# ubuntuslave/vo_single_camera_sos

Hardware: AMD Instinct MI355X
Metric: frame-pairs/sec (detect+match+triangulate+RANSAC) on 640x480 omni, 2000 kpts (higher is better)
Workload: dtype u8/f32/f64

## Files before the change

include/sosvo.h:

```cpp
#ifndef SOSVO_H
#define SOSVO_H

#include <stdint.h>

#ifdef __cplusplus
extern "C" {
#endif

typedef struct sosvo_ctx sosvo_ctx;

typedef enum {
  SOSVO_OK = 0,
  SOSVO_ERR_ARG = -1,
  SOSVO_ERR_HIP = -2,
  SOSVO_ERR_NODEVICE = -3,
  SOSVO_ERR_CAPACITY = -4
} sosvo_status;

#define SOSVO_DESC_BYTES 32
#define SOSVO_KEY_SHIFT 20
#define SOSVO_KEY_IDX_MASK 0xFFFFFu
#define SOSVO_KEY_NONE 0xFFFFFFFFu


int32_t sosvo_abi_version(void);

int32_t sosvo_orb_bit_pattern_31(int8_t* pattern_host);

int32_t sosvo_create(sosvo_ctx** out, int32_t device, void* stream);
int32_t sosvo_destroy(sosvo_ctx* ctx);
int32_t sosvo_set_stream(sosvo_ctx* ctx, void* stream);
#define SOSVO_HINT_SHARED_DEVICE 1
#define SOSVO_HINT_SCORE_FP64_ONLY 2
#define SOSVO_HINT_MATCH_UNSPLIT 3
int32_t sosvo_set_hint(sosvo_ctx* ctx, int32_t hint, int32_t value);
int32_t sosvo_synchronize(sosvo_ctx* ctx);
const char* sosvo_last_error(const sosvo_ctx* ctx);

int32_t sosvo_timer_start(sosvo_ctx* ctx);
int32_t sosvo_timer_stop(sosvo_ctx* ctx);
int32_t sosvo_timer_elapsed_ms(sosvo_ctx* ctx, float* ms);

int32_t sosvo_profile_enable(sosvo_ctx* ctx, int32_t on);
int32_t sosvo_profile_count(sosvo_ctx* ctx);
int32_t sosvo_profile_get(sosvo_ctx* ctx, int32_t i, char* name_out, int32_t name_cap, float* ms);

int32_t sosvo_debug_fill_scratch(sosvo_ctx* ctx, int32_t byte);

int32_t sosvo_unwrap(sosvo_ctx* ctx, const uint8_t* omni, const uint8_t* masks, const float* map_x,
                     const float* map_y, int32_t nframes, int32_t H, int32_t W, int32_t rows,
                     int32_t cols, uint8_t* pano);

int32_t sosvo_unwrap_prepare(sosvo_ctx* ctx, const uint8_t* masks, const float* map_x, const float* map_y,
                             int32_t H, int32_t W, int32_t rows, int32_t cols, uint32_t* table);
int32_t sosvo_unwrap_table(sosvo_ctx* ctx, const uint8_t* omni, const uint32_t* table, int32_t nframes,
                           int32_t H, int32_t W, int32_t rows, int32_t cols, uint8_t* pano);

int32_t sosvo_median_gray(sosvo_ctx* ctx, const uint8_t* img, int32_t nimg, int32_t rows,
                          int32_t cols, int32_t ksize, uint8_t* gray);
int32_t sosvo_unwrap_median_gray(sosvo_ctx* ctx, const uint8_t* omni, const uint32_t* table, int32_t nframes,
                                 int32_t H, int32_t W, int32_t rows, int32_t cols, int32_t ksize, uint8_t* gray);

int32_t sosvo_unwrap_median_gray_rows(sosvo_ctx* ctx, const uint8_t* omni, const uint32_t* table, int32_t nframes,
                                      int32_t H, int32_t W, int32_t rows, int32_t cols, int32_t ksize,
                                      const int32_t* row_range, uint8_t* gray);

int32_t sosvo_gray_rows_needed(sosvo_ctx* ctx, const uint32_t* mask_bits, int32_t nsets, int32_t rows, int32_t cols,
                               int32_t nmask, int32_t edge, const int8_t* pattern, float cos_a, float sin_a,
                               int32_t* row_range);

int32_t sosvo_detect_gft(sosvo_ctx* ctx, const uint8_t* gray, const uint32_t* mask_bits, int32_t nimg,
                         int32_t images_per_maskset, int32_t rows, int32_t cols, int32_t nmask,
                         double quality, double min_distance, int32_t max_corners, int32_t cap,
                         float* kp, int32_t* n, int32_t* status);

int32_t sosvo_describe_orb(sosvo_ctx* ctx, const uint8_t* gray, int32_t nimg, int32_t rows, int32_t cols,
                           int32_t nmask, int32_t cap, float* kp, int32_t* n, float cos_a, float sin_a,
                           const int8_t* pattern, int32_t edge, uint8_t* desc);

int32_t sosvo_describe_orb_rows(sosvo_ctx* ctx, const uint8_t* gray, int32_t nimg, int32_t rows, int32_t cols,
                                int32_t nmask, int32_t cap, float* kp, int32_t* n, float cos_a, float sin_a,
                                const int8_t* pattern, int32_t edge, const int32_t* row_range, uint8_t* desc);

int32_t sosvo_subpix_weights(sosvo_ctx* ctx, int32_t half, int32_t* w_host);
int32_t sosvo_refine_subpix(sosvo_ctx* ctx, const uint8_t* gray, int32_t nimg, int32_t rows, int32_t cols, int32_t nmask,
                            int32_t cap, float* kp, const int32_t* n, int32_t half, int32_t max_iter, double eps,
                            const int32_t* row_range);

#define SOSVO_LK_INITIAL_FLOW 1
int32_t sosvo_gray_pyramid_bytes(sosvo_ctx* ctx, int32_t nimg, int32_t rows, int32_t cols, int32_t levels, int64_t* bytes);
int32_t sosvo_gray_pyramid(sosvo_ctx* ctx, const uint8_t* gray, int32_t nimg, int32_t rows, int32_t cols, int32_t levels,
                           const int32_t* row_range, uint8_t* pyr);
int32_t sosvo_track_lk(sosvo_ctx* ctx, const uint8_t* gray, const uint8_t* pyr, int32_t nimg, int32_t rows, int32_t cols,
                       int32_t levels, const int32_t* row_range, const int32_t* prev_img, const int32_t* next_img, int32_t nprob,
                       int32_t cap, const float* prev_pts, const int32_t* n, int32_t half, int32_t max_iter, double eps,
                       double min_eig, int32_t flags, float* next_pts, uint8_t* status, float* err, float* back, double fb_max);

int64_t sosvo_orb_pyramid_pixels(int32_t rows, int32_t cols);
int32_t sosvo_orb_mask_pyramid(sosvo_ctx* ctx, const uint32_t* mask_bits, int32_t nsets, int32_t rows,
                               int32_t cols, int32_t nmask, uint32_t* mask_pyr);
int32_t sosvo_detect_orb(sosvo_ctx* ctx, const uint8_t* gray, const uint32_t* mask_pyr, int32_t nimg,
                         int32_t images_per_maskset, int32_t rows, int32_t cols, int32_t nmask,
                         int32_t nfeatures, int32_t cap, float* kp4, float* resp, int32_t* n);
int32_t sosvo_describe_orb_levels(sosvo_ctx* ctx, const uint8_t* gray, int32_t nimg, int32_t rows,
                                  int32_t cols, int32_t nmask, int32_t cap, float* kp4, int32_t* n,
                                  const int8_t* pattern, uint8_t* desc, float* kp_xy);
int32_t sosvo_detect_describe_orb(sosvo_ctx* ctx, const uint8_t* gray, const uint32_t* mask_pyr, int32_t nimg,
                                  int32_t images_per_maskset, int32_t rows, int32_t cols, int32_t nmask,
                                  int32_t nfeatures, int32_t cap, float* kp4, float* resp, int32_t* n,
                                  const int8_t* pattern, uint8_t* desc, float* kp_xy);

int32_t sosvo_detect_fast(sosvo_ctx* ctx, const uint8_t* gray, const uint32_t* mask_bits, int32_t nimg,
                          int32_t images_per_maskset, int32_t rows, int32_t cols, int32_t nmask,
                          int32_t threshold, int32_t cap, float* kp, int32_t* n, int32_t* status);

int32_t sosvo_detect_agast(sosvo_ctx* ctx, const uint8_t* gray, const uint32_t* mask_bits, int32_t nimg,
                           int32_t images_per_maskset, int32_t rows, int32_t cols, int32_t nmask,
                           int32_t threshold, int32_t cap, float* kp, int32_t* n, int32_t* status);

int32_t sosvo_match_hamming(sosvo_ctx* ctx, const uint8_t* q_desc, const uint8_t* t_desc,
                            const int32_t* nq, const int32_t* nt, const int32_t* q_slot,
                            const int32_t* t_slot, int32_t nprob, int32_t q_stride,
                            int32_t t_stride, int32_t k, uint32_t* keys);

int32_t sosvo_match_hamming_gated(sosvo_ctx* ctx, const uint8_t* q_desc, const uint8_t* t_desc, const float* q_pos,
                                  const float* t_pos, const int32_t* nq, const int32_t* nt, const int32_t* q_slot,
                                  const int32_t* t_slot, int32_t nprob, int32_t n_forward, int32_t q_stride, int32_t t_stride,
                                  double min_dv, double max_du, int32_t max_distance, uint32_t* keys);

int32_t sosvo_match_hamming_ratio(sosvo_ctx* ctx, const uint8_t* q_desc, const uint8_t* t_desc, const float* q_pos,
                                  const float* t_pos, const int32_t* nq, const int32_t* nt, const int32_t* q_slot,
                                  const int32_t* t_slot, int32_t nprob, int32_t n_forward, int32_t q_stride, int32_t t_stride,
                                  double min_dv, double max_du, int32_t max_distance, int32_t ratio_64ths,
                                  uint32_t* keys, uint32_t* rivals);

int32_t sosvo_match_l2(sosvo_ctx* ctx, const float* q_desc, const float* t_desc, const int32_t* nq, const int32_t* nt,
                       int32_t nprob, int32_t q_stride, int32_t t_stride, int32_t dim, int32_t k, uint64_t* keys);

int32_t sosvo_match_radius(sosvo_ctx* ctx, const uint8_t* q_desc, const uint8_t* t_desc, const int32_t* nq,
                           const int32_t* nt, const int32_t* q_slot, const int32_t* t_slot, int32_t nprob,
                           int32_t q_stride, int32_t t_stride, int32_t max_distance, int32_t cap,
                           uint32_t* keys, int32_t* counts);

int32_t sosvo_cross_check_matches(sosvo_ctx* ctx, const uint32_t* keys_fwd, const uint32_t* keys_rev, const int32_t* nq,
                                  const int32_t* nt, const int32_t* q_slot, const int32_t* t_slot, int32_t nprob,
                                  int32_t q_stride, int32_t t_stride, uint32_t* keys_out, int32_t* n_kept);

int32_t sosvo_sort_matches(sosvo_ctx* ctx, const uint32_t* keys, const int32_t* nq,
                           const int32_t* q_slot, int32_t nprob, int32_t q_stride, int32_t* order);

#define SOSVO_FLAG_CAM_ROT_IDENTITY 1
#define SOSVO_FLAG_EPNP 2
#define SOSVO_FLAG_GP3P 4
#define SOSVO_FLAG_TWOPT 8
int32_t sosvo_ransac_abs_pose(sosvo_ctx* ctx, const double* f, const double* p, const int32_t* cam,
                              const double* cam_off, const double* cam_rot, int32_t ncam, int32_t flags,
                              const int32_t* n, int32_t nprob, int32_t stride, double thr,
                              int32_t max_iter, int32_t adaptive, uint64_t seed, double* T_out,
                              uint8_t* inlier_mask, int32_t* inlier_idx, int32_t* n_inliers,
                              int32_t* info, int32_t* hyp_counts);
int32_t sosvo_ransac_abs_pose_seeds(sosvo_ctx* ctx, const double* f, const double* p, const int32_t* cam,
                                    const double* cam_off, const double* cam_rot, int32_t ncam, int32_t flags,
                                    const int32_t* n, int32_t nprob, int32_t stride, double thr,
                                    int32_t max_iter, int32_t adaptive, const uint64_t* seeds, double* T_out,
                                    uint8_t* inlier_mask, int32_t* inlier_idx, int32_t* n_inliers,
                                    int32_t* info, int32_t* hyp_counts);

int32_t sosvo_refine_abs_pose(sosvo_ctx* ctx, const double* f, const double* p, const int32_t* cam,
                              const double* cam_off, const double* cam_rot, int32_t ncam,
                              const int32_t* n, int32_t nprob, int32_t stride, const int32_t* idx,
                              const int32_t* m, int32_t max_lm_iter, double* T_io, double* cost_out,
                              int32_t* iters_out);

#define SOSVO_REL_FIVEPT 5
#define SOSVO_REL_SEVENPT 7
#define SOSVO_REL_EIGHTPT 8
int32_t sosvo_ransac_rel_pose(sosvo_ctx* ctx, const double* f1, const double* f2, const int32_t* n, int32_t nprob,
                              int32_t stride, int32_t algorithm, double thr, int32_t max_iter, int32_t adaptive,
                              uint64_t seed, double* T_out, uint8_t* inlier_mask, int32_t* inlier_idx,
                              int32_t* n_inliers, int32_t* info, int32_t* hyp_counts);

int32_t sosvo_pano_to_bearing(sosvo_ctx* ctx, const double* uv, int32_t n, double cols, double rows,
                              double pixel_size, double cyl_height_max, double* az, double* el,
                              double* bearing);
int32_t sosvo_triangulate_midpoint(sosvo_ctx* ctx, const double* az_top, const double* el_top,
                                   const double* az_bot, const double* el_bot, int32_t n,
                                   const double* F_top_host, const double* F_bot_host, double* X);
int32_t sosvo_triangulate2(sosvo_ctx* ctx, const double* b1, const double* b2, int32_t n, const double* t12_host,
                           const double* R12_host, double* X);
int32_t sosvo_range_filter(sosvo_ctx* ctx, const double* X, int32_t n, double min_range,
                           double max_range, uint8_t* ok);
int32_t sosvo_rgbd_backproject(sosvo_ctx* ctx, const float* depth, int32_t rows, int32_t cols,
                               const int32_t* u, const int32_t* v, int32_t n, double fx, double fy,
                               double cx, double cy, double focal_length_m, int32_t depth_is_Z,
                               double* xyz, double* bearing);

typedef struct sosvo_rig {
  double pano_top[4];
  double pano_bot[4];
  double F_top[3];
  double F_bot[3];
  double min_range;
  double max_range;
  double stereo_min_disp;
  double stereo_max_hdiff;
  double f2f_max_hdiff;
  double pct_good_matches;
} sosvo_rig;

int32_t sosvo_stereo_assemble(sosvo_ctx* ctx, const sosvo_rig* rig_host, const float* kp_top,
                              const float* kp_bot, const uint8_t* desc_top, const uint8_t* desc_bot,
                              const int32_t* n_top, const int32_t* n_bot, const uint32_t* keys,
                              const int32_t* order, int32_t nframes, int32_t nmask, int32_t cap,
                              int32_t out_cap, float* m_top, float* m_bot, uint8_t* d_top,
                              uint8_t* d_bot, double* X, double* b_top, double* b_bot, int32_t* M,
                              int32_t* n_cand);

int32_t sosvo_f2f_assemble(sosvo_ctx* ctx, const sosvo_rig* rig_host, const float* m_top,
                           const float* m_bot, const double* X, const double* b_top,
                           const double* b_bot, const int32_t* M, int32_t frame_cap,
                           const int32_t* ref_frame, const int32_t* cur_frame, const uint32_t* keys_top,
                           const int32_t* order_top, const uint32_t* keys_bot, const int32_t* order_bot,
                           int32_t npairs, int32_t corr_cap, double* f, double* p, int32_t* cam,
                           int32_t* corr_q, int32_t* corr_t, int32_t* n, int32_t* n_topview);

int32_t sosvo_f2f_assemble_tracked(sosvo_ctx* ctx, const sosvo_rig* rig_host, const float* m_top, const float* m_bot,
                                   const double* X, const int32_t* M, int32_t frame_cap, const int32_t* ref_frame,
// ... 193 lines not shown
```

vo_single_camera_sos_amd/_lib.py:

```python
import ctypes
import os
import re
from collections import namedtuple

_HERE = os.path.dirname(os.path.abspath(__file__))
LIB_PATH = os.path.join(_HERE, "libsosvo.so")
HEADER_PATH = os.path.join(os.path.dirname(_HERE), "include", "sosvo.h")

c_i32 = ctypes.c_int32
c_f64 = ctypes.c_double
c_f32 = ctypes.c_float
c_u64 = ctypes.c_uint64
c_p = ctypes.c_void_p

SOSVO_OK = 0
STATUS_NAMES = {0: "SOSVO_OK", -1: "SOSVO_ERR_ARG", -2: "SOSVO_ERR_HIP", -3: "SOSVO_ERR_NODEVICE",
                -4: "SOSVO_ERR_CAPACITY"}

KEY_SHIFT = 20
KEY_IDX_MASK = 0xFFFFF
KEY_NONE = 0xFFFFFFFF
DESC_BYTES = 32


class SosvoError(RuntimeError):
    pass


SIGNATURES = {
    "sosvo_abi_version": (c_i32, []),
    "sosvo_orb_bit_pattern_31": (c_i32, [c_p]),
    "sosvo_create": (c_i32, [ctypes.POINTER(c_p), c_i32, c_p]),
    "sosvo_destroy": (c_i32, [c_p]),
    "sosvo_set_stream": (c_i32, [c_p, c_p]),
    "sosvo_set_hint": (c_i32, [c_p, c_i32, c_i32]),
    "sosvo_set_lk_options": (c_i32, [c_p, c_p]),
    "sosvo_set_stereo_lk_options": (c_i32, [c_p, c_p]),
    "sosvo_synchronize": (c_i32, [c_p]),
    "sosvo_last_error": (ctypes.c_char_p, [c_p]),
    "sosvo_timer_start": (c_i32, [c_p]),
    "sosvo_timer_stop": (c_i32, [c_p]),
    "sosvo_timer_elapsed_ms": (c_i32, [c_p, ctypes.POINTER(c_f32)]),
    "sosvo_profile_enable": (c_i32, [c_p, c_i32]),
    "sosvo_profile_count": (c_i32, [c_p]),
    "sosvo_debug_fill_scratch": (c_i32, [c_p, c_i32]),
    "sosvo_profile_get": (c_i32, [c_p, c_i32, ctypes.c_char_p, c_i32, ctypes.POINTER(c_f32)]),
    "sosvo_unwrap": (c_i32, [c_p, c_p, c_p, c_p, c_p, c_i32, c_i32, c_i32, c_i32, c_i32, c_p]),
    "sosvo_unwrap_prepare": (c_i32, [c_p, c_p, c_p, c_p, c_i32, c_i32, c_i32, c_i32, c_p]),
    "sosvo_unwrap_table": (c_i32, [c_p, c_p, c_p, c_i32, c_i32, c_i32, c_i32, c_i32, c_p]),
    "sosvo_median_gray": (c_i32, [c_p, c_p, c_i32, c_i32, c_i32, c_i32, c_p]),
    "sosvo_unwrap_median_gray": (c_i32, [c_p, c_p, c_p, c_i32, c_i32, c_i32, c_i32, c_i32, c_i32, c_p]),
    "sosvo_unwrap_median_gray_rows": (c_i32, [c_p, c_p, c_p, c_i32, c_i32, c_i32, c_i32, c_i32, c_i32, c_p, c_p]),
    "sosvo_gray_rows_needed": (c_i32, [c_p, c_p, c_i32, c_i32, c_i32, c_i32, c_i32, c_p, c_f32, c_f32, c_p]),
    "sosvo_detect_gft": (c_i32, [c_p, c_p, c_p, c_i32, c_i32, c_i32, c_i32, c_i32, c_f64, c_f64, c_i32, c_i32, c_p,
                                 c_p, c_p]),
    "sosvo_describe_orb": (c_i32, [c_p, c_p, c_i32, c_i32, c_i32, c_i32, c_i32, c_p, c_p, c_f32, c_f32, c_p, c_i32,
                                   c_p]),
    "sosvo_describe_orb_rows": (c_i32, [c_p, c_p, c_i32, c_i32, c_i32, c_i32, c_i32, c_p, c_p, c_f32, c_f32, c_p, c_i32,
                                        c_p, c_p]),
    "sosvo_subpix_weights": (c_i32, [c_p, c_i32, c_p]),
    "sosvo_refine_subpix": (c_i32, [c_p, c_p, c_i32, c_i32, c_i32, c_i32, c_i32, c_p, c_p, c_i32, c_i32, c_f64, c_p]),
    "sosvo_gray_pyramid_bytes": (c_i32, [c_p, c_i32, c_i32, c_i32, c_i32, ctypes.POINTER(ctypes.c_int64)]),
    "sosvo_gray_pyramid": (c_i32, [c_p, c_p, c_i32, c_i32, c_i32, c_i32, c_p, c_p]),
    "sosvo_track_lk": (c_i32, [c_p, c_p, c_p, c_i32, c_i32, c_i32, c_i32, c_p, c_p, c_p, c_i32, c_i32, c_p, c_p, c_i32, c_i32,
                               c_f64, c_f64, c_i32, c_p, c_p, c_p, c_p, c_f64]),
    "sosvo_refine_stereo_lk": (c_i32, [c_p, c_p, c_i32, c_i32, c_i32, c_p, c_i32, c_i32, c_p, c_p, c_p, c_p, c_p, c_f64, c_f64,
                                       c_p, c_p]),
    "sosvo_orb_pyramid_pixels": (ctypes.c_int64, [c_i32, c_i32]),
    "sosvo_orb_mask_pyramid": (c_i32, [c_p, c_p, c_i32, c_i32, c_i32, c_i32, c_p]),
    "sosvo_detect_orb": (c_i32, [c_p, c_p, c_p, c_i32, c_i32, c_i32, c_i32, c_i32, c_i32, c_i32, c_p, c_p, c_p]),
    "sosvo_describe_orb_levels": (c_i32, [c_p, c_p, c_i32, c_i32, c_i32, c_i32, c_i32, c_p, c_p, c_p, c_p, c_p]),
    "sosvo_detect_describe_orb": (c_i32, [c_p, c_p, c_p, c_i32, c_i32, c_i32, c_i32, c_i32, c_i32, c_i32, c_p, c_p, c_p, c_p,
                                          c_p, c_p]),
    "sosvo_detect_fast": (c_i32, [c_p, c_p, c_p, c_i32, c_i32, c_i32, c_i32, c_i32, c_i32, c_i32, c_p, c_p, c_p]),
    "sosvo_detect_agast": (c_i32, [c_p, c_p, c_p, c_i32, c_i32, c_i32, c_i32, c_i32, c_i32, c_i32, c_p, c_p, c_p]),
    "sosvo_match_hamming": (c_i32, [c_p, c_p, c_p, c_p, c_p, c_p, c_p, c_i32, c_i32, c_i32, c_i32, c_p]),
    "sosvo_match_hamming_gated": (c_i32, [c_p, c_p, c_p, c_p, c_p, c_p, c_p, c_p, c_p, c_i32, c_i32, c_i32, c_i32, c_f64, c_f64,
                                          c_i32, c_p]),
    "sosvo_match_hamming_ratio": (c_i32, [c_p, c_p, c_p, c_p, c_p, c_p, c_p, c_p, c_p, c_i32, c_i32, c_i32, c_i32, c_f64, c_f64,
                                          c_i32, c_i32, c_p, c_p]),
    "sosvo_match_radius": (c_i32, [c_p, c_p, c_p, c_p, c_p, c_p, c_p, c_i32, c_i32, c_i32, c_i32, c_i32, c_p, c_p]),
    "sosvo_cross_check_matches": (c_i32, [c_p, c_p, c_p, c_p, c_p, c_p, c_p, c_i32, c_i32, c_i32, c_p, c_p]),
    "sosvo_sort_matches": (c_i32, [c_p, c_p, c_p, c_p, c_i32, c_i32, c_p]),
    "sosvo_pano_to_bearing": (c_i32, [c_p, c_p, c_i32, c_f64, c_f64, c_f64, c_f64, c_p, c_p, c_p]),
    "sosvo_triangulate_midpoint": (c_i32, [c_p, c_p, c_p, c_p, c_p, c_i32, c_p, c_p, c_p]),
    "sosvo_triangulate2": (c_i32, [c_p, c_p, c_p, c_i32, c_p, c_p, c_p]),
    "sosvo_range_filter": (c_i32, [c_p, c_p, c_i32, c_f64, c_f64, c_p]),
    "sosvo_rgbd_backproject": (c_i32, [c_p, c_p, c_i32, c_i32, c_p, c_p, c_i32, c_f64, c_f64, c_f64, c_f64, c_f64,
                                       c_i32, c_p, c_p]),
    "sosvo_stereo_assemble": (c_i32, [c_p] + [c_p] * 9 + [c_i32] * 4 + [c_p] * 9),
    "sosvo_f2f_assemble": (c_i32, [c_p] + [c_p] * 7 + [c_i32] + [c_p] * 6 + [c_i32, c_i32] + [c_p] * 7),
    "sosvo_f2f_assemble_tracked": (c_i32, [c_p] + [c_p] * 5 + [c_i32] + [c_p] * 5 + [c_i32, c_i32] + [c_p] * 7),
    "sosvo_ransac_abs_pose": (c_i32, [c_p, c_p, c_p, c_p, c_p, c_p, c_i32, c_i32, c_p, c_i32, c_i32, c_f64,
                                      c_i32, c_i32, c_u64, c_p, c_p, c_p, c_p, c_p, c_p]),
    "sosvo_ransac_abs_pose_seeds": (c_i32, [c_p, c_p, c_p, c_p, c_p, c_p, c_i32, c_i32, c_p, c_i32, c_i32, c_f64,
                                            c_i32, c_i32, c_p, c_p, c_p, c_p, c_p, c_p, c_p]),
    "sosvo_match_l2": (c_i32, [c_p, c_p, c_p, c_p, c_p, c_i32, c_i32, c_i32, c_i32, c_i32, c_p]),
    "sosvo_ransac_rel_pose": (c_i32, [c_p, c_p, c_p, c_p, c_i32, c_i32, c_i32, c_f64, c_i32, c_i32, c_u64, c_p, c_p, c_p, c_p,
                                      c_p, c_p]),
    "sosvo_refine_abs_pose": (c_i32, [c_p, c_p, c_p, c_p, c_p, c_p, c_i32, c_p, c_i32, c_i32, c_p, c_p, c_i32,
                                      c_p, c_p, c_p]),
    "sosvo_rgbd_assemble": (c_i32, [c_p, c_p, c_p, c_p, c_p, c_p, c_i32, c_i32, c_i32, c_i32, c_i32, c_p, c_p, c_p, c_p, c_p]),
    "sosvo_f2f_assemble_central": (c_i32, [c_p, c_f64, c_f64, c_p, c_p, c_p, c_p, c_i32, c_p, c_p, c_p, c_p, c_i32, c_i32,
                                           c_p, c_p, c_p, c_p, c_p]),
    "sosvo_frame_pair_batch_workspace": (ctypes.c_size_t, [c_p]),
    "sosvo_frame_pair_batch": (c_i32, [c_p, c_p, c_p, c_p, c_p, c_p, c_p, c_p, ctypes.c_size_t, c_p]),
    "sosvo_frame_pair_batch_streams_workspace": (ctypes.c_size_t, [c_p, c_i32]),
    "sosvo_frame_pair_batch_streams": (c_i32, [c_p, c_p, c_p, c_i32, c_p, c_p, c_p, c_p, c_p, ctypes.c_size_t, c_p]),
    "sosvo_frame_pair_batch_streams_enqueue": (c_i32, [c_p, c_p, c_p, c_i32, c_p, c_p, c_p, c_p, c_p, ctypes.c_size_t, c_p]),
    "sosvo_frame_pair_batch_streams_join": (c_i32, [c_p]),
    "sosvo_sequence_workspace": (ctypes.c_size_t, [c_p, c_i32, c_i32]),
    "sosvo_sequence_front_end": (c_i32, [c_p, c_p, c_p, c_i32, c_i32, c_p, c_i32, c_i32, c_p, c_p, c_p, c_p, ctypes.c_size_t]),
    "sosvo_sequence_track": (c_i32, [c_p, c_p, c_p, c_i32, c_i32, c_p, c_p, c_i32, c_u64, c_p, ctypes.c_size_t, c_p]),
    "sosvo_sequence_copy_slot": (c_i32, [c_p, c_p, c_i32, c_i32, c_i32, c_i32, c_p, ctypes.c_size_t]),
    "sosvo_sequence_frame_counts": (c_i32, [c_p, c_p, c_i32, c_i32, c_i32, c_i32, c_p, ctypes.c_size_t, c_p]),
    "sosvo_sequence_front_end_slots": (c_i32, [c_p, c_p, c_p, c_i32, c_i32, c_p, c_i32, c_p, c_p, c_p, c_p, c_p, ctypes.c_size_t]),
    "sosvo_sequence_track_seeds": (c_i32, [c_p, c_p, c_p, c_i32, c_i32, c_p, c_p, c_p, c_i32, c_p, ctypes.c_size_t, c_p]),
    "sosvo_sequence_copy_slots": (c_i32, [c_p, c_p, c_i32, c_i32, c_p, c_p, c_i32, c_p, ctypes.c_size_t]),
    "sosvo_rgbd_sequence_workspace": (ctypes.c_size_t, [c_p, c_i32, c_i32]),
    "sosvo_rgbd_sequence_front_end": (c_i32, [c_p, c_p, c_p, c_i32, c_i32, c_p, c_p, c_i32, c_i32, c_p, c_p, c_p, ctypes.c_size_t]),
    "sosvo_rgbd_sequence_track": (c_i32, [c_p, c_p, c_i32, c_i32, c_p, c_p, c_i32, c_u64, c_p, ctypes.c_size_t, c_p]),
    "sosvo_rgbd_sequence_copy_slot": (c_i32, [c_p, c_p, c_i32, c_i32, c_i32, c_i32, c_p, ctypes.c_size_t]),
    "sosvo_rgbd_sequence_frame_counts": (c_i32, [c_p, c_p, c_i32, c_i32, c_i32, c_i32, c_p, ctypes.c_size_t, c_p]),
    "sosvo_rgbd_sequence_front_end_slots": (c_i32, [c_p, c_p, c_p, c_i32, c_i32, c_p, c_p, c_i32, c_p, c_p, c_p, c_p,
                                                    ctypes.c_size_t]),
    "sosvo_rgbd_sequence_track_seeds": (c_i32, [c_p, c_p, c_i32, c_i32, c_p, c_p, c_p, c_i32, c_p, ctypes.c_size_t, c_p]),
    "sosvo_rgbd_sequence_copy_slots": (c_i32, [c_p, c_p, c_i32, c_i32, c_p, c_p, c_i32, c_p, ctypes.c_size_t]),
    "sosvo_rgbd_pair_batch_workspace": (ctypes.c_size_t, [c_p]),
    "sosvo_rgbd_pair_batch": (c_i32, [c_p, c_p, c_p, c_p, c_p, c_p, c_p, c_p, ctypes.c_size_t, c_p]),
}

HINT_SHARED_DEVICE = 1
HINT_SCORE_FP64_ONLY = 2
HINT_MATCH_UNSPLIT = 3
FLAG_CAM_ROT_IDENTITY = 1
FLAG_EPNP = 2
FLAG_GP3P = 4
FLAG_TWOPT = 8
FLAG_CROSS_CHECK_STEREO = 0x1000
FLAG_CROSS_CHECK_F2F = 0x2000
FLAG_GATED_STEREO = 0x4000
FLAG_GATED_F2F = 0x8000
GATED_MAX_DIST_SHIFT = 16
GATED_MAX_DIST_MASK = 0x1FF << GATED_MAX_DIST_SHIFT
FLAG_RATIO_STEREO = 0x10
FLAG_RATIO_F2F = 0x20
RATIO_64THS_SHIFT = 25
RATIO_64THS_MASK = 0x3F << RATIO_64THS_SHIFT
FLAG_SUBPIX = 0x40
SUBPIX_HALF_SHIFT = 10
SUBPIX_HALF_MASK = 3 << SUBPIX_HALF_SHIFT
SUBPIX_MAX_ITER = 10
SUBPIX_EPS = 0.01
FLAG_LK_F2F = 0x80
FLAG_LK_STEREO = 0x100
LK_INITIAL_FLOW = 1
LK_MAX_HALF, LK_MAX_LEVELS, LK_MAX_ITER, LK_MAX_CAP = 10, 4, 30, 4096
DETECTOR_GFT = 0
DETECTOR_ORB = 1
DETECTOR_FAST = 2
DETECTOR_AGAST = 3
DETECTORS = {"GFT": DETECTOR_GFT, "ORB": DETECTOR_ORB, "FAST": DETECTOR_FAST, "AGAST": DETECTOR_AGAST}
RGBD_DETECTOR_SHIFT = 8
RGBD_DETECTOR_MASK = 3 << RGBD_DETECTOR_SHIFT
REL_FIVEPT = 5
REL_SEVENPT = 7
REL_EIGHTPT = 8


class Rig(ctypes.Structure):
    _fields_ = [("pano_top", c_f64 * 4), ("pano_bot", c_f64 * 4), ("F_top", c_f64 * 3), ("F_bot", c_f64 * 3),
                ("min_range", c_f64), ("max_range", c_f64), ("stereo_min_disp", c_f64),
                ("stereo_max_hdiff", c_f64), ("f2f_max_hdiff", c_f64), ("pct_good_matches", c_f64)]



class RgbdCam(ctypes.Structure):
    _fields_ = [("fx", c_f64), ("fy", c_f64), ("cx", c_f64), ("cy", c_f64), ("focal_length_m", c_f64),
                ("depth_is_Z", c_i32), ("reserved", c_i32), ("min_range", c_f64), ("max_range", c_f64)]


class BatchCfg(ctypes.Structure):
    _fields_ = [("n_pairs", c_i32), ("H", c_i32), ("W", c_i32), ("rows", c_i32), ("cols", c_i32), ("nmask", c_i32),
                ("kp_cap", c_i32), ("frame_cap", c_i32), ("median_ksize", c_i32), ("max_corners", c_i32), ("edge", c_i32),
                ("ransac_max_iter", c_i32), ("ransac_adaptive", c_i32), ("lm_max_iter", c_i32), ("quality", c_f64),
                ("min_distance", c_f64), ("ransac_threshold", c_f64), ("seed", c_u64), ("cos_a", c_f32), ("sin_a", c_f32),
                ("ransac_flags", c_i32), ("detector", c_i32)]


class RgbdBatchCfg(ctypes.Structure):
    _fields_ = [("n_pairs", c_i32), ("rows", c_i32), ("cols", c_i32), ("kp_cap", c_i32), ("frame_cap", c_i32),
                ("median_ksize", c_i32), ("max_corners", c_i32), ("edge", c_i32), ("ransac_max_iter", c_i32),
                ("ransac_adaptive", c_i32), ("lm_max_iter", c_i32), ("flags", c_i32), ("quality", c_f64),
                ("min_distance", c_f64), ("ransac_threshold", c_f64), ("pct_good_matches", c_f64), ("f2f_max_hdiff", c_f64),
                ("seed", c_u64), ("cos_a", c_f32), ("sin_a", c_f32)]


def detector_code(method):
    name = str(method).upper()
    if name not in DETECTORS:
        raise NotImplementedError("detection method %r: the batched paths run %s" % (method, ", ".join(DETECTORS)))
    return DETECTORS[name]


def rgbd_detector_flags(method):
    return detector_code(method) << RGBD_DETECTOR_SHIFT


def cross_check_flags(stereo=False, f2f=False):
    return (FLAG_CROSS_CHECK_STEREO if stereo else 0) | (FLAG_CROSS_CHECK_F2F if f2f else 0)


def gated_flags(stereo=False, f2f=False, max_distance=None):
    if max_distance is not None and (int(max_distance) != max_distance or not 1 <= max_distance <= 256):
        raise ValueError("gated_max_distance must be None or an integer in 1 .. 256, got %r" % (max_distance,))
    flags = (FLAG_GATED_STEREO if stereo else 0) | (FLAG_GATED_F2F if f2f else 0)
    if flags and max_distance is not None:
        flags |= int(max_distance) << GATED_MAX_DIST_SHIFT
    return flags


def ratio_64ths(ratio):
    try:
        x = float(ratio) * 64.0
    except (TypeError, ValueError):
        raise ValueError("ratio must be a float in (0, 1) with ratio * 64 an integer, got %r" % (ratio,))
    if not (x == x and 1.0 <= x <= 63.0 and x == int(x)):
        if x != x:
            raise ValueError("ratio must be a float in (0, 1) with ratio * 64 an integer, got %r" % (ratio,))
        lo, hi = sorted(sorted(range(1, 64), key=lambda c: abs(c - x))[:2])
        raise ValueError("ratio must be a float in (0, 1) with ratio * 64 an integer, got %r; the nearest admissible values "
                         "are %r (%d/64) and %r (%d/64)" % (ratio, lo / 64.0, lo, hi / 64.0, hi))
    return int(x)


def ratio_flags(stereo=False, f2f=False, ratio=None):
    r = None if ratio is None else ratio_64ths(ratio)
    flags = (FLAG_RATIO_STEREO if stereo else 0) | (FLAG_RATIO_F2F if f2f else 0)
    if flags and r is None:
        raise ValueError("the ratio test needs a ratio (a float in (0, 1) with ratio * 64 an integer, e.g. 0.75)")
    if flags:
        flags |= r << RATIO_64THS_SHIFT
    return flags


def subpix_half(subpix):
    if subpix is None or subpix is False:
        return None
    if subpix is True:
        return 5
    if int(subpix) != subpix or not 2 <= subpix <= 5:
        raise ValueError("subpix must be None or a window half-size in 2 .. 5, got %r" % (subpix,))
    return int(subpix)


def subpix_flags(subpix=None):
    half = subpix_half(subpix)
    return 0 if half is None else FLAG_SUBPIX | ((half - 2) << SUBPIX_HALF_SHIFT)


def subpix_half_of(flags):
    flags = int(flags)
    return ((flags & SUBPIX_HALF_MASK) >> SUBPIX_HALF_SHIFT) + 2 if flags & FLAG_SUBPIX else None


def subpix_weights(half):
    w = (c_i32 * 11)()
    rc = load().sosvo_subpix_weights(None, int(half), w)
    if rc != 0:
        raise SosvoError("sosvo_subpix_weights(%r) -> %s" % (half, STATUS_NAMES.get(rc, rc)))
    return list(w)[:2 * int(half) + 1]


class LKOptions(namedtuple("LKOptions", "half levels max_iter eps min_eig fb_max")):
    __slots__ = ()

    def __new__(cls, half=10, levels=3, max_iter=30, eps=0.01, min_eig=1e-4, fb_max=None):
        for name, v, lo, hi in (("half", half, 2, LK_MAX_HALF), ("levels", levels, 1, LK_MAX_LEVELS),
                                ("max_iter", max_iter, 1, LK_MAX_ITER)):
            if isinstance(v, bool) or not isinstance(v, (int, float)) or int(v) != v or not lo <= v <= hi:
                raise ValueError("lk %s must be an integer in %d .. %d, got %r" % (name, lo, hi, v))
        for name, v in (("eps", eps), ("min_eig", min_eig)):
            if isinstance(v, bool) or not isinstance(v, (int, float)) or not 0.0 <= v < float("inf"):
                raise ValueError("lk %s must be a finite number >= 0, got %r" % (name, v))
        if fb_max is not None and (isinstance(fb_max, bool) or not isinstance(fb_max, (int, float))
                                   or not 0.0 < fb_max < float("inf")):
            raise ValueError("lk fb_max must be None or a finite number > 0 (pixels), got %r" % (fb_max,))
# ... 181 lines not shown
```

vo_single_camera_sos_amd/csrc/common.h:

```cpp
#pragma once
#include <hip/hip_runtime.h>
#include <stdint.h>
#include <stdio.h>
#include <string.h>

#include "sosvo.h"

struct sosvo_prof_entry {
  const char* name;
  hipEvent_t a, b;
};

constexpr int kSosvoProfMax = 16384;

constexpr int kSosvoMaxSubStreams = 4;

struct sosvo_ctx {
  int32_t device;
  hipStream_t stream;
  hipEvent_t ev_start, ev_stop;
  char err[512];
  void* ws;
  size_t ws_bytes;
  int32_t prof_on;
  int32_t prof_n;
  int32_t prof_created;
  sosvo_prof_entry* prof;
  sosvo_ctx* sub[kSosvoMaxSubStreams];
  hipEvent_t sub_done[kSosvoMaxSubStreams], sub_median[kSosvoMaxSubStreams], sub_begin;
  int32_t n_sub;
  int32_t hint_score_fp64_only;
  int32_t hint_shared_device;
  int32_t hint_match_unsplit;
  sosvo_lk_options lk;
  sosvo_stereo_lk_options stereo_lk;
  int32_t sub_last;
  int32_t sub_pending;
  const void* sub_last_ws;
  size_t sub_last_bytes[kSosvoMaxSubStreams];
};

struct SosvoProfScope {
  sosvo_ctx* ctx;
  bool active;
  SosvoProfScope(sosvo_ctx* c, const char* name) : ctx(c), active(false) {
    if (!c->prof_on || !c->prof || c->prof_n >= kSosvoProfMax) return;
    sosvo_prof_entry& e = c->prof[c->prof_n];
    if (c->prof_n >= c->prof_created) {
      if (hipEventCreate(&e.a) != hipSuccess || hipEventCreate(&e.b) != hipSuccess) return;
      c->prof_created = c->prof_n + 1;
    }
    e.name = name;
    if (hipEventRecord(e.a, c->stream) != hipSuccess) return;
    active = true;
  }
  ~SosvoProfScope() {
    if (!active) return;
    (void)hipEventRecord(ctx->prof[ctx->prof_n].b, ctx->stream);
    ctx->prof_n++;
  }
};
#define SOSVO_PROFILE(ctx, name) SosvoProfScope sosvo_prof_scope_(ctx, name)

#define SOSVO_LAUNCH(ctx, kernel, ...)            \
  do {                                            \
    SOSVO_PROFILE(ctx, #kernel);                  \
    hipLaunchKernelGGL(kernel, __VA_ARGS__);      \
  } while (0)

#define SOSVO_WAVE 64

static inline int32_t sosvo_fail(sosvo_ctx* ctx, int32_t code, const char* what, const char* detail) {
  if (ctx) snprintf(ctx->err, sizeof(ctx->err), "%s: %s", what, detail ? detail : "");
  return code;
}

#define SOSVO_REQUIRE(ctx, cond, msg)                                   \
  do {                                                                  \
    if (!(cond)) return sosvo_fail((ctx), SOSVO_ERR_ARG, __func__, msg); \
  } while (0)

static inline bool sosvo_table_frame_ok(int64_t H, int64_t W) {
  return H > 0 && W > 0 && H <= 16384 && W <= 16384 && 3 * W * (H - 1) >= 8;
}
#define SOSVO_TABLE_FRAME_MSG \
  "frame size out of range for the unwrap table: 1 <= H, W <= 16384 and 3 * W * (H - 1) >= 8 (8 bytes must follow the start of the second row)"

#define SOSVO_HIP(ctx, call)                                                          \
  do {                                                                                \
    hipError_t e_ = (call);                                                           \
    if (e_ != hipSuccess) return sosvo_fail((ctx), SOSVO_ERR_HIP, #call, hipGetErrorString(e_)); \
  } while (0)

#define SOSVO_ENTER(ctx)                                   \
  do {                                                     \
    if (!(ctx)) return SOSVO_ERR_ARG;                      \
    SOSVO_HIP((ctx), hipSetDevice((ctx)->device));         \
  } while (0)

#define SOSVO_LATENCY_BOUND_PRIO() __builtin_amdgcn_s_setprio(3)
#define SOSVO_STREAMING_PRIO() __builtin_amdgcn_s_setprio(2)

#define SOSVO_LAUNCH_CHECK(ctx) SOSVO_HIP((ctx), hipGetLastError())

static inline int32_t sosvo_ws_reserve(sosvo_ctx* ctx, size_t bytes) {
  if (bytes <= ctx->ws_bytes) return SOSVO_OK;
  if (ctx->ws) {
    SOSVO_HIP(ctx, hipStreamSynchronize(ctx->stream));
    SOSVO_HIP(ctx, hipFree(ctx->ws));
    ctx->ws = nullptr;
    ctx->ws_bytes = 0;
  }
  SOSVO_HIP(ctx, hipMalloc(&ctx->ws, bytes));
  ctx->ws_bytes = bytes;
  return SOSVO_OK;
}

static inline int cdiv(int a, int b) { return (a + b - 1) / b; }

__host__ __device__ static inline uint32_t sosvo_float_ordered(float f) {
  uint32_t u;
  memcpy(&u, &f, 4);
  return (u & 0x80000000u) ? ~u : (u | 0x80000000u);
}
__host__ __device__ static inline float sosvo_ordered_float(uint32_t u) {
  u = (u & 0x80000000u) ? (u & 0x7FFFFFFFu) : ~u;
  float f;
  memcpy(&f, &u, 4);
  return f;
}

#ifdef __HIPCC__
__device__ __forceinline__ int refl101(int i, int n) {
  if (n == 1) return 0;
  while (i < 0 || i >= n) i = i < 0 ? -i : 2 * (n - 1) - i;
  return i;
}

__device__ __forceinline__ int clampi(int v, int lo, int hi) { return v < lo ? lo : (v > hi ? hi : v); }

__device__ __forceinline__ void sosvo_copy_bytes(uint8_t* __restrict__ d, const uint8_t* __restrict__ s, size_t nbytes, int i0, int stride) {
  size_t done = 0;
  if ((((uintptr_t)d | (uintptr_t)s) & 15) == 0) {
    const size_t nv = nbytes / 16;
    for (size_t i = i0; i < nv; i += stride) reinterpret_cast<uint4*>(d)[i] = reinterpret_cast<const uint4*>(s)[i];
    done = nv * 16;
  }
  for (size_t i = done + i0; i < nbytes; i += stride) d[i] = s[i];
}

__device__ __forceinline__ int lane_from_left(int v) { return __builtin_amdgcn_update_dpp(0, v, 0x138, 0xF, 0xF, true); }
__device__ __forceinline__ int lane_from_right(int v) { return __builtin_amdgcn_update_dpp(0, v, 0x130, 0xF, 0xF, true); }
__device__ __forceinline__ float lane_from_left(float v) { return __int_as_float(lane_from_left(__float_as_int(v))); }
__device__ __forceinline__ float lane_from_right(float v) { return __int_as_float(lane_from_right(__float_as_int(v))); }

__device__ __forceinline__ uint32_t vmad24(uint32_t k, uint32_t x, uint32_t acc) {
  uint32_t r;
  asm("v_mad_u32_u24 %0, %1, %2, %3" : "=v"(r) : "v"(x), "v"(k), "v"(acc));
  return r;
}

template <int NW = 4>
__device__ __forceinline__ int sosvo_block_compact_pos(bool valid, int* wave_off, int* s_running, int tid) {
  const int lane = tid & 63, wid = tid >> 6;
  const unsigned long long bal = __ballot(valid);
  __syncthreads();
  if (lane == 0) wave_off[wid + 1] = __popcll(bal);
  __syncthreads();
  if (tid == 0) {
    wave_off[0] = *s_running;
    for (int w = 0; w < NW; ++w) wave_off[w + 1] += wave_off[w];
    *s_running = wave_off[NW];
  }
  __syncthreads();
  return wave_off[wid] + __popcll(bal & ((1ULL << lane) - 1ULL));
}

__device__ __forceinline__ int xcd_problem(int nimg, int nmask) {
  const int xcd = (int)(blockIdx.x & 7), slot = (int)(blockIdx.x >> 3);
  const int img = (slot / nmask) * 8 + xcd, m = slot - (slot / nmask) * nmask;
  return img < nimg ? img * nmask + m : -1;
}
static inline unsigned xcd_grid(int nimg, int nmask) { return (unsigned)(8 * cdiv(nimg, 8) * nmask); }

__device__ __forceinline__ int sosvo_block_count_matches(const uint32_t* __restrict__ keys, int nq, int tid, int threads) {
  int kept = 0;
// ... 41 lines not shown
```

vo_single_camera_sos_amd/csrc/ctx.hip:

```cpp
#include "common.h"
#include "orb_bit_pattern_31.h"

#include <stdlib.h>

static const sosvo_lk_options kLkDefaults = SOSVO_LK_OPTIONS_DEFAULT;
static const sosvo_stereo_lk_options kStereoLkDefaults = SOSVO_STEREO_LK_OPTIONS_DEFAULT;

extern "C" {

int32_t sosvo_abi_version(void) { return 1; }

int32_t sosvo_orb_bit_pattern_31(int8_t* pattern_host) {
  if (!pattern_host) return SOSVO_ERR_ARG;
  memcpy(pattern_host, sosvo_orb_bit_pattern_31_table, 1024);
  return SOSVO_OK;
}

int32_t sosvo_create(sosvo_ctx** out, int32_t device, void* stream) {
  if (!out) return SOSVO_ERR_ARG;
  *out = nullptr;
  int n = 0;
  if (hipGetDeviceCount(&n) != hipSuccess || n <= 0) return SOSVO_ERR_NODEVICE;
  if (device < 0 || device >= n) return SOSVO_ERR_NODEVICE;
  hipDeviceProp_t prop;
  if (hipGetDeviceProperties(&prop, device) != hipSuccess) return SOSVO_ERR_HIP;
  if (strncmp(prop.gcnArchName, "gfx950", 6) != 0) return SOSVO_ERR_NODEVICE;
  sosvo_ctx* ctx = (sosvo_ctx*)calloc(1, sizeof(sosvo_ctx));
  if (!ctx) return SOSVO_ERR_HIP;
  ctx->device = device;
  ctx->stream = (hipStream_t)stream;
  if (hipSetDevice(device) != hipSuccess || hipEventCreate(&ctx->ev_start) != hipSuccess ||
      hipEventCreate(&ctx->ev_stop) != hipSuccess) {
    free(ctx);
    return SOSVO_ERR_HIP;
  }
  ctx->lk = kLkDefaults;
  ctx->stereo_lk = kStereoLkDefaults;
  *out = ctx;
  return SOSVO_OK;
}

int32_t sosvo_set_lk_options(sosvo_ctx* ctx, const sosvo_lk_options* options) {
  if (!ctx) return SOSVO_ERR_ARG;
  if (!options) return sosvo_fail(ctx, SOSVO_ERR_ARG, __func__, "null pointer (SOSVO_LK_OPTIONS_DEFAULT gives the defaults)");
  const sosvo_lk_options o = *options;
  if (!sosvo_lk_options_ok(o))
    return sosvo_fail(ctx, SOSVO_ERR_ARG, __func__,
                      "out of range: half 2..10, levels 1..4, max_iter 1..30, eps and min_eig finite and >= 0, fb_max finite");
  ctx->lk = o;
  ctx->lk.reserved = 0;
  return SOSVO_OK;
}

int32_t sosvo_set_stereo_lk_options(sosvo_ctx* ctx, const sosvo_stereo_lk_options* options) {
  if (!ctx) return SOSVO_ERR_ARG;
  if (!options)
    return sosvo_fail(ctx, SOSVO_ERR_ARG, __func__, "null pointer (SOSVO_STEREO_LK_OPTIONS_DEFAULT gives the defaults)");
  const sosvo_stereo_lk_options o = *options;
  if (!sosvo_stereo_lk_options_ok(o))
    return sosvo_fail(ctx, SOSVO_ERR_ARG, __func__,
                      "out of range: half 2..10, max_iter 1..30, eps and min_eig finite and >= 0, max_shift finite and >= 0");
  ctx->stereo_lk = o;
  return SOSVO_OK;
}

int32_t sosvo_set_hint(sosvo_ctx* ctx, int32_t hint, int32_t value) {
  if (!ctx) return SOSVO_ERR_ARG;
  if (hint == SOSVO_HINT_SHARED_DEVICE) {
    ctx->hint_shared_device = value != 0;
  } else if (hint == SOSVO_HINT_SCORE_FP64_ONLY) {
    ctx->hint_score_fp64_only = value != 0;
    for (int i = 0; i < ctx->n_sub; ++i)
      if (ctx->sub[i]) ctx->sub[i]->hint_score_fp64_only = value != 0;
  } else if (hint == SOSVO_HINT_MATCH_UNSPLIT) {
    ctx->hint_match_unsplit = value != 0;
  } else {
    return sosvo_fail(ctx, SOSVO_ERR_ARG, __func__, "unknown hint");
  }
  return SOSVO_OK;
}

int32_t sosvo_destroy(sosvo_ctx* ctx) {
  if (!ctx) return SOSVO_OK;
  (void)hipSetDevice(ctx->device);
  for (int i = 0; i < ctx->n_sub; ++i) {
    if (ctx->sub[i]) {
      hipStream_t st = ctx->sub[i]->stream;
      (void)hipStreamSynchronize(st);
      (void)sosvo_destroy(ctx->sub[i]);
      (void)hipStreamDestroy(st);
    }
    (void)hipEventDestroy(ctx->sub_done[i]);
    (void)hipEventDestroy(ctx->sub_median[i]);
  }
  if (ctx->n_sub) (void)hipEventDestroy(ctx->sub_begin);
  if (ctx->ws) (void)hipFree(ctx->ws);
  if (ctx->prof) {
    for (int i = 0; i < ctx->prof_created; ++i) {
      (void)hipEventDestroy(ctx->prof[i].a);
      (void)hipEventDestroy(ctx->prof[i].b);
    }
    free(ctx->prof);
  }
  (void)hipEventDestroy(ctx->ev_start);
  (void)hipEventDestroy(ctx->ev_stop);
  free(ctx);
  return SOSVO_OK;
}

int32_t sosvo_set_stream(sosvo_ctx* ctx, void* stream) {
  SOSVO_ENTER(ctx);
  ctx->stream = (hipStream_t)stream;
  return SOSVO_OK;
}

int32_t sosvo_synchronize(sosvo_ctx* ctx) {
  SOSVO_ENTER(ctx);
  SOSVO_HIP(ctx, hipStreamSynchronize(ctx->stream));
  return SOSVO_OK;
}

const char* sosvo_last_error(const sosvo_ctx* ctx) { return ctx ? ctx->err : "null context"; }

int32_t sosvo_timer_start(sosvo_ctx* ctx) {
  SOSVO_ENTER(ctx);
  SOSVO_HIP(ctx, hipEventRecord(ctx->ev_start, ctx->stream));
  return SOSVO_OK;
}

int32_t sosvo_timer_stop(sosvo_ctx* ctx) {
  SOSVO_ENTER(ctx);
  SOSVO_HIP(ctx, hipEventRecord(ctx->ev_stop, ctx->stream));
  return SOSVO_OK;
}

int32_t sosvo_profile_enable(sosvo_ctx* ctx, int32_t on) {
  SOSVO_ENTER(ctx);
  if (on && !ctx->prof) {
    ctx->prof = (sosvo_prof_entry*)calloc(kSosvoProfMax, sizeof(sosvo_prof_entry));
    if (!ctx->prof) return sosvo_fail(ctx, SOSVO_ERR_HIP, __func__, "out of host memory");
  }
  ctx->prof_on = on ? 1 : 0;
  ctx->prof_n = 0;
  return SOSVO_OK;
}

int32_t sosvo_profile_count(sosvo_ctx* ctx) { return ctx ? ctx->prof_n : 0; }

int32_t sosvo_profile_get(sosvo_ctx* ctx, int32_t i, char* name_out, int32_t name_cap, float* ms) {
  SOSVO_ENTER(ctx);
  SOSVO_REQUIRE(ctx, ctx->prof && i >= 0 && i < ctx->prof_n && name_out && name_cap > 0 && ms, "bad arguments");
  const sosvo_prof_entry& e = ctx->prof[i];
  SOSVO_HIP(ctx, hipEventSynchronize(e.b));
  SOSVO_HIP(ctx, hipEventElapsedTime(ms, e.a, e.b));
  snprintf(name_out, (size_t)name_cap, "%s", e.name ? e.name : "");
  return SOSVO_OK;
}

int32_t sosvo_debug_fill_scratch(sosvo_ctx* ctx, int32_t byte) {
  SOSVO_ENTER(ctx);
  if (ctx->ws && ctx->ws_bytes) SOSVO_HIP(ctx, hipMemsetAsync(ctx->ws, byte & 0xFF, ctx->ws_bytes, ctx->stream));
  for (int i = 0; i < ctx->n_sub; ++i) {
    if (!ctx->sub[i]) continue;
    const int32_t rc = sosvo_debug_fill_scratch(ctx->sub[i], byte);
    if (rc != SOSVO_OK) return sosvo_fail(ctx, rc, __func__, ctx->sub[i]->err);
  }
  return SOSVO_OK;
}

int32_t sosvo_timer_elapsed_ms(sosvo_ctx* ctx, float* ms) {
  SOSVO_ENTER(ctx);
  SOSVO_REQUIRE(ctx, ms != nullptr, "ms is null");
  SOSVO_HIP(ctx, hipEventSynchronize(ctx->ev_stop));
  SOSVO_HIP(ctx, hipEventElapsedTime(ms, ctx->ev_start, ctx->ev_stop));
  return SOSVO_OK;
}

}
```

vo_single_camera_sos_amd/csrc/detect.hip:

```cpp
#include "common.h"

#include <type_traits>

namespace {

constexpr int kThreads = 256;
constexpr int kCandCap = 4096;
constexpr int kCandCapSmall = 2048;
constexpr int kCandCapLarge = 16384;
constexpr int kMaxMasks = 32;

__device__ __forceinline__ float sqrt_rn_normal(float x) {
  const float s = __builtin_amdgcn_sqrtf(x);
  const float s_dn = __int_as_float(__float_as_int(s) - 1), s_up = __int_as_float(__float_as_int(s) + 1);
  const float r_dn = __builtin_fmaf(-s_dn, s, x), r_up = __builtin_fmaf(-s_up, s, x);
  float r = (r_dn <= 0.0f) ? s_dn : s;
  r = (r_up > 0.0f) ? s_up : r;
  return r;
}

constexpr int kEigHalo = 3;
constexpr int kEigStripW = 64 - 2 * kEigHalo;

__device__ __forceinline__ void eig_flush(uint32_t* __restrict__ mstat_img, uint32_t bits, uint32_t omax) {
  while (bits) {
    const int m = __ffs(bits) - 1;
    bits &= bits - 1;
    atomicMax(&mstat_img[m * 5], omax);
  }
}

__global__ __launch_bounds__(kThreads) void min_eigen_kernel(const uint8_t* __restrict__ gray,
                                                             const uint32_t* __restrict__ mask_bits, int nimg,
                                                             int images_per_maskset, int rows, int cols, int nmask,
                                                             int strips, int nchunks, int chunk_rows, int wcap,
                                                             uint2* __restrict__ cand, uint32_t* __restrict__ wcnt,
                                                             uint32_t* __restrict__ mstat) {
  SOSVO_STREAMING_PRIO();
  const int lane = threadIdx.x & 63;
  const int wave = __builtin_amdgcn_readfirstlane((int)((blockIdx.x * kThreads + threadIdx.x) >> 6));
  if (wave >= nimg * strips * nchunks) return;
  const int img = wave / (strips * nchunks);
  const int rem = wave - img * strips * nchunks;
  const int chunk = rem / strips, strip = rem - chunk * strips;
  const int xb = strip * kEigStripW - kEigHalo;
  const int xc = xb + lane;
  const int xs = clampi(xc, 0, cols - 1);
  const int ll = clampi(refl101(xs - 1, cols) - xb, 0, 63);
  const int lr = clampi(refl101(xs + 1, cols) - xb, 0, 63);
  const bool out_lane = lane >= kEigHalo && lane < 64 - kEigHalo && xc < cols;
  uint32_t* mstat_img = mstat + (size_t)img * nmask * 5;
  int r_lo = rows, r_hi = 0;
  {
    const uint32_t* sbb = mstat + (size_t)(img / images_per_maskset) * images_per_maskset * nmask * 5;
    for (int m = 0; m < nmask; ++m) {
      const uint32_t y1 = sbb[m * 5 + 4];
      if (y1) {
        r_lo = min(r_lo, (int)(0xFFFFFFFFu - sbb[m * 5 + 2]));
        r_hi = max(r_hi, (int)y1);
      }
    }
  }
  const int ys = max(chunk * chunk_rows, r_lo), ye = min(min(rows, chunk * chunk_rows + chunk_rows), r_hi);
  if (ys >= ye) {
    if (lane == 0) wcnt[wave] = 0u;
    return;
  }
  const int e_lo = max(ys - 1, 0), e_hi = min(ye, rows - 1);
  const int f_lo = max(ys, 1), f_hi = min(ye, rows - 1) - 1;
  const uint8_t* g = gray + (size_t)img * rows * cols;
  uint2* region = cand + (size_t)wave * wcap;
  int wpos = 0;
  uint32_t mb_prev = 0u;
  const uint32_t* mb = mask_bits + (size_t)(img / images_per_maskset) * rows * cols;
  const uint32_t mask_all = nmask < 32 ? (1u << nmask) - 1u : 0xFFFFFFFFu;
  const float scale = (float)(1.0 / 3060.0);

  int hd[3] = {0, 0, 0}, hs[3] = {0, 0, 0};
  float pxx[3] = {0.f, 0.f, 0.f}, pxy[3] = {0.f, 0.f, 0.f}, pyy[3] = {0.f, 0.f, 0.f};
  float hm[3] = {0.f, 0.f, 0.f}, ec[3] = {0.f, 0.f, 0.f};
  uint32_t cur_bits = 0u, cur_max = 0u;
  const int t_first = e_lo - 2, t_last = e_hi + 2;

  const bool edge_strip = xb < 1 || xb + 64 > cols - 1;
  int c_cur[3] = {0, 0, 0}, c_pre[3] = {0, 0, 0};
  auto request = [&](int t0) __attribute__((always_inline)) {
#pragma unroll
    for (int k = 0; k < 3; ++k) c_pre[k] = (int)g[(uint32_t)(refl101(min(t0 + k, t_last), rows) * cols) + (uint32_t)xs];
  };
  auto step = [&](auto phase_tag, auto edge_tag, const int t) __attribute__((always_inline)) {
    constexpr int P = decltype(phase_tag)::value;
    constexpr bool EDGE = decltype(edge_tag)::value;
    auto left = [&](auto v) { return EDGE ? __shfl(v, ll) : lane_from_left(v); };
    auto right = [&](auto v) { return EDGE ? __shfl(v, lr) : lane_from_right(v); };
    constexpr int i0 = (P + 1) % 3, i1 = (P + 2) % 3, i2 = P;
    if (t > t_last) return;
    const int y_pre = t - 2;
    const bool y_out = y_pre >= ys && y_pre < ye && y_pre >= e_lo && out_lane;
    const uint32_t o_pre = (uint32_t)(max(y_pre, 0) * cols) + (uint32_t)xc;
    const uint32_t mb_pre = y_out ? mb[o_pre] : 0u;
    {
      const int c = c_cur[P];
      const int l = left(c), r = right(c);
      hd[i2] = r - l;
      hs[i2] = (l + 2 * c) + r;
    }
    const int v = t - 1;
    if (v < e_lo - 1) return;
    {
      const int dxi = (hd[i0] + 2 * hd[i1]) + hd[i2], dyi = hs[i2] - hs[i0];
      const float dx = (float)dxi * scale, dy = (float)dyi * scale;
      const float xx = dx * dx, yy = dy * dy;
      float xy = dx * dy;
      if (v < 0 || v >= rows) xy = -xy;
      pxx[i2] = (left(xx) + xx) + right(xx);
      pxy[i2] = (left(xy) + xy) + right(xy);
      pyy[i2] = (left(yy) + yy) + right(yy);
    }
    const int y = v - 1;
    if (y < e_lo) return;
    {
      const float a = ((pxx[i0] + pxx[i1]) + pxx[i2]) * 0.5f, b = (pxy[i0] + pxy[i1]) + pxy[i2];
      const float c = ((pyy[i0] + pyy[i1]) + pyy[i2]) * 0.5f;
      const float e = (a + c) - sqrt_rn_normal(((a - c) * (a - c)) + (b * b));
      if (y_out) {
        const uint32_t bits = mb_pre & mask_all;
        if (bits != cur_bits) {
          eig_flush(mstat_img, cur_bits, cur_max);
          cur_bits = bits;
          cur_max = 0u;
        }
        cur_max = max(cur_max, sosvo_float_ordered(e));
      }
      const float el = left(e), er = right(e);
      hm[i2] = fmaxf(fmaxf(el, e), er);
      ec[i2] = e;
    }
    const int f = y - 1;
    const uint32_t mb_f = mb_prev & mask_all;
    mb_prev = mb_pre;
    if (f < f_lo || f > f_hi) return;
    {
      const float ev = ec[i1];
      const bool is_cand = out_lane && xc >= 1 && xc <= cols - 2 && ev == fmaxf(fmaxf(hm[i0], hm[i1]), hm[i2]) && ev > 0.0f &&
                           mb_f != 0u;
      const unsigned long long bal = __ballot(is_cand);
      if (bal) {
        const int pos = wpos + (int)__builtin_amdgcn_mbcnt_hi((uint32_t)(bal >> 32), __builtin_amdgcn_mbcnt_lo((uint32_t)bal, 0u));
        if (is_cand && pos < wcap) region[pos] = make_uint2(__float_as_uint(ev), ((uint32_t)f << 16) | (uint32_t)xc);
        wpos += __popcll(bal);
      }
    }
  };
  auto run = [&](auto edge_tag) __attribute__((always_inline)) {
    request(t_first);
    for (int t = t_first; t <= t_last; t += 3) {
#pragma unroll
      for (int k = 0; k < 3; ++k) c_cur[k] = c_pre[k];
      request(t + 3);
      step(std::integral_constant<int, 0>{}, edge_tag, t);
      step(std::integral_constant<int, 1>{}, edge_tag, t + 1);
      step(std::integral_constant<int, 2>{}, edge_tag, t + 2);
    }
  };
  if (edge_strip) run(std::true_type{}); else run(std::false_type{});
  if (lane == 0) wcnt[wave] = (uint32_t)wpos;
  const unsigned long long act = __ballot(out_lane && cur_bits != 0u);
  if (act) {
    const int first = __ffsll((long long)act) - 1;
    const uint32_t b0 = __shfl(cur_bits, first);
    if (__ballot(out_lane && cur_bits != 0u && cur_bits != b0) == 0ULL) {
      uint32_t om = (out_lane && cur_bits != 0u) ? cur_max : 0u;
      for (int s = 32; s > 0; s >>= 1) om = max(om, (uint32_t)__shfl_down((int)om, s));
      if (lane == 0) eig_flush(mstat_img, b0, om);
    } else {
      eig_flush(mstat_img, cur_bits, cur_max);
    }
  }
}

__global__ __launch_bounds__(kThreads) void mask_bbox_kernel(const uint32_t* __restrict__ mask_bits, int images_per_maskset,
                                                             int rows, int cols, int nmask, uint32_t* __restrict__ mstat) {
  __shared__ uint32_t sb[2][kMaxMasks];
  const int tid = threadIdx.x, y = blockIdx.x, set = blockIdx.y;
  if (tid < 2 * kMaxMasks) (&sb[0][0])[tid] = 0u;
  __syncthreads();
  const uint32_t* mb = mask_bits + ((size_t)set * rows + y) * cols;
  const uint32_t mask_all = nmask < 32 ? (1u << nmask) - 1u : 0xFFFFFFFFu;
  for (int x = tid; x < cols; x += kThreads) {
    uint32_t b = mb[x] & mask_all;
    while (b) {
      const int m = __ffs(b) - 1;
      b &= b - 1;
      atomicMax(&sb[0][m], 0xFFFFFFFFu - (uint32_t)x);
      atomicMax(&sb[1][m], (uint32_t)x + 1u);
    }
  }
  __syncthreads();
  if (tid < nmask && sb[1][tid]) {
    uint32_t* st = mstat + ((size_t)set * images_per_maskset * nmask + tid) * 5;
    atomicMax(&st[1], sb[0][tid]);
    atomicMax(&st[2], 0xFFFFFFFFu - (uint32_t)y);
    atomicMax(&st[3], sb[1][tid]);
    atomicMax(&st[4], (uint32_t)y + 1u);
  }
}

template <int LOGR, int NT>
__device__ __forceinline__ void bitonic_pass(unsigned long long* keys, int N, int k, int jtop, int tid) {
  constexpr int R = 1 << LOGR;
  const int jl = jtop >> (LOGR - 1);
  for (int t = tid; t < (N >> LOGR); t += NT) {
    const int i = ((t & ~(jl - 1)) << LOGR) | (t & (jl - 1));
    const bool desc = (i & k) == 0;
    unsigned long long v[R];
#pragma unroll
    for (int m = 0; m < R; ++m) v[m] = keys[i + m * jl];
#pragma unroll
    for (int sb = LOGR - 1; sb >= 0; --sb) {
#pragma unroll
      for (int m = 0; m < R; ++m) {
        if (m & (1 << sb)) continue;
        const unsigned long long a = v[m], b = v[m | (1 << sb)];
        const bool sw = (a < b) == desc;
        v[m] = sw ? b : a;
        v[m | (1 << sb)] = sw ? a : b;
      }
    }
#pragma unroll
    for (int m = 0; m < R; ++m) keys[i + m * jl] = v[m];
  }
}

__device__ __forceinline__ uint32_t dist2_packed(uint32_t a, uint32_t b) {
  typedef short short2v __attribute__((ext_vector_type(2)));
  const short2v d = __builtin_bit_cast(short2v, a) - __builtin_bit_cast(short2v, b);
  return (uint32_t)__builtin_amdgcn_sdot2(d, d, 0, false);
}

constexpr uint32_t kGridEmpty = 0xFFFFFFFFu;
struct gft_igrid {
  uint32_t thr_i;
  uint32_t magic;
  int cell, cx0, cy0, gwp;
  __device__ __forceinline__ gft_igrid(float md2, int cell_, int cx0_, int cy0_, int gwp_)
      : thr_i((uint32_t)__builtin_amdgcn_readfirstlane((int)(uint32_t)ceilf(md2))),
        magic((uint32_t)__builtin_amdgcn_readfirstlane((int)(cell_ > 1 ? 0xFFFFFFFFu / (uint32_t)cell_ + 1u : 0u))), cell(cell_),
        cx0(cx0_), cy0(cy0_), gwp(gwp_) {}
  __device__ __forceinline__ int cell_index(uint32_t xy, bool active) const {
    const uint32_t x = xy & 0xFFFFu, y = xy >> 16;
    const int xc = active ? (int)(cell > 1 ? __umulhi(x, magic) : x) - cx0 + 1 : 1;
    const int yc = active ? (int)(cell > 1 ? __umulhi(y, magic) : y) - cy0 + 1 : 1;
    return (yc * gwp + xc) * 2;
  }
  __device__ __forceinline__ uint32_t cell_hit(const uint32_t* grid, int cidx, int dxc, int dyc, uint32_t xy) const {
    const uint2 q2 = *reinterpret_cast<const uint2*>(&grid[cidx + dyc * gwp * 2 + dxc * 2]);
    return ((uint32_t)(q2.x != kGridEmpty) & (uint32_t)(dist2_packed(xy, q2.x) < thr_i)) |
           ((uint32_t)(q2.y != kGridEmpty) & (uint32_t)(dist2_packed(xy, q2.y) < thr_i));
  }
  __device__ __forceinline__ bool near(uint32_t a, uint32_t b) const { return dist2_packed(a, b) < thr_i; }
  __device__ __forceinline__ void insert(uint32_t* grid, int cidx, uint32_t xy, int* s_ovf, uint32_t* acc_list, int limit_list) const {
    if (atomicCAS(&grid[cidx], kGridEmpty, xy) != kGridEmpty && atomicCAS(&grid[cidx + 1], kGridEmpty, xy) != kGridEmpty) {
      const int o = atomicAdd(s_ovf, 1);
      if (o < limit_list) acc_list[o] = xy;
    }
  }
};

struct gft_regions {
  const uint2* cand;
  const uint32_t* wcnt;
  const uint32_t* mb;
  int img, m, cols, strips, nchunks, wcap, s0, c0, ns, R;
  float thr;
};

template <int NT, class F>
__device__ __forceinline__ void gft_walk_keys(const gft_regions& g, int* s_region, int tid, F&& f) {
  const int wave = __builtin_amdgcn_readfirstlane(tid >> 6), lane = tid & 63;
  for (int rb = 0; rb < g.R; rb += NT) {
    if (rb + tid < g.R) {
      const int rg = rb + tid, c = g.c0 + rg / g.ns, sidx = g.s0 + rg % g.ns;
      s_region[tid] = min((int)g.wcnt[(g.img * g.nchunks + c) * g.strips + sidx], g.wcap);
    }
    __syncthreads();
    const int rend = min(NT, g.R - rb);
    for (int rr = wave; rr < rend; rr += NT / 64) {
      const int have = s_region[rr];
      const int rg = rb + rr, c = g.c0 + rg / g.ns, sidx = g.s0 + rg % g.ns;
      const uint2* region = g.cand + (size_t)((g.img * g.nchunks + c) * g.strips + sidx) * g.wcap;
      for (int i = lane; i < have; i += 64) {
        const uint2 r = region[i];
        if (__uint_as_float(r.x) > g.thr && ((g.mb[(r.y >> 16) * (uint32_t)g.cols + (r.y & 0xFFFFu)] >> g.m) & 1u))
          f(((unsigned long long)sosvo_float_ordered(__uint_as_float(r.x)) << 32) | r.y);
      }
    }
    __syncthreads();
  }
}

template <int CAND, int NT>
__device__ __forceinline__ void gft_keep_largest(const gft_regions g, unsigned long long* keys, int* s_region, int* s_count,
                                              int* s_sel, int tid) {
  constexpr int kBits = 11, kBins = 1 << kBits, kPer = kBins / 64;
  static_assert(kBins * sizeof(uint32_t) <= CAND * sizeof(unsigned long long), "the histogram lives in the key LDS");
  uint32_t* hist = reinterpret_cast<uint32_t*>(keys);
  unsigned long long prefix = 0ULL;
  int want = CAND;
  for (int shift = 64; shift > 0;) {
    const int width = min(kBits, shift);
    const unsigned long long high = shift < 64 ? ~0ULL << shift : 0ULL;
    shift -= width;
    for (int i = tid; i < kBins; i += NT) hist[i] = 0u;
    __syncthreads();
    gft_walk_keys<NT>(g, s_region, tid, [&](unsigned long long key) {
      if ((key & high) == prefix) atomicAdd(&hist[(uint32_t)(key >> shift) & ((1u << width) - 1u)], 1u);
    });
    if (tid < 64) {
      uint32_t sum = 0u;
      for (int b = 0; b < kPer; ++b) sum += hist[tid * kPer + b];
      uint32_t incl = sum;
      for (int s = 1; s < 64; s <<= 1) {
        const uint32_t o = (uint32_t)__shfl_down((int)incl, s);
        if (tid + s < 64) incl += o;
      }
      uint32_t above = incl - sum;
      if (above < (uint32_t)want && (uint32_t)want <= incl) {
        for (int b = kPer - 1; b >= 0; --b) {
          const uint32_t c = hist[tid * kPer + b];
          if (above + c >= (uint32_t)want) {
            s_sel[0] = tid * kPer + b;
            s_sel[1] = want - (int)above;
            s_sel[2] = (int)c;
            break;
          }
          above += c;
        }
      }
    }
    __syncthreads();
    prefix |= (unsigned long long)(uint32_t)s_sel[0] << shift;
    want = s_sel[1];
    const bool whole_bin = want == s_sel[2];
    __syncthreads();
    if (whole_bin) break;
  }
  if (tid == 0) *s_count = 0;
  __syncthreads();
  gft_walk_keys<NT>(g, s_region, tid, [&](unsigned long long key) {
    if (key >= prefix) {
      const int slot = atomicAdd(s_count, 1);
      if (slot < CAND) keys[slot] = key;
    }
  });
}

template <int CAND, int NT>
__global__ __launch_bounds__(NT) void gft_select_kernel(const uint2* __restrict__ cand,
                                                              const uint32_t* __restrict__ wcnt, int strips, int nchunks,
                                                              int chunk_rows, int wcap, const uint32_t* __restrict__ mask_bits,
                                                              const uint32_t* __restrict__ mstat, int images_per_maskset,
                                                              int nmask, int rows, int cols, double quality,
                                                              float min_distance, int cell, int max_corners, int cap,
                                                              uint32_t* __restrict__ sorted_g, int sorted_stride,
                                                              float* __restrict__ kp, int32_t* __restrict__ n_out,
                                                              int32_t* __restrict__ status, int32_t* __restrict__ redo,
                                                              int redo_pass, int nimg_total) {
  SOSVO_LATENCY_BOUND_PRIO();
  constexpr int kSelGridCells = (CAND * 8 - 1024 * 4) / 8;
  const int p = xcd_problem(nimg_total, nmask);
  if (p < 0) return;
  if (redo && redo_pass == 1 && redo[p] == 0) return;
  __shared__ unsigned long long lds_u64[CAND];
  __shared__ int s_count, s_accepted, s_overflow;
  __shared__ int s_region[NT];
  __shared__ int s_sel[3];
  __shared__ unsigned long long s_conf[64];
  __shared__ unsigned long long s_prior;
  __shared__ int s_ovf;
  unsigned long long* keys = lds_u64;
  uint32_t* grid = reinterpret_cast<uint32_t*>(lds_u64);
  uint32_t* acc_list = grid + 2 * kSelGridCells;
  const int tid = threadIdx.x;
  const int img = p / nmask, m = p - img * nmask;
  const uint32_t* st = mstat + (size_t)p * 5;
  const uint32_t* sb = mstat + ((size_t)(img / images_per_maskset) * images_per_maskset * nmask + m) * 5;
  uint32_t* sorted = sorted_g + (size_t)p * sorted_stride;
  if (tid == 0) {
    s_count = 0;
    s_accepted = 0;
    s_overflow = 0;
    s_prior = 0ULL;
    s_ovf = 0;
  }
  __syncthreads();
  const bool any = st[0] != 0u;
  const int bx0 = any ? max(1, (int)(0xFFFFFFFFu - sb[1])) : 0, by0 = any ? max(1, (int)(0xFFFFFFFFu - sb[2])) : 0;
  const int bx1 = any ? min(cols - 2, (int)sb[3] - 1) : -1, by1 = any ? min(rows - 2, (int)sb[4] - 1) : -1;
  const int bw = bx1 - bx0 + 1, bh = by1 - by0 + 1;
  if (any && bw > 0 && bh > 0) {
    const float thr = (float)((double)sosvo_ordered_float(st[0]) * quality);
    const uint32_t* mb = mask_bits + (size_t)(img / images_per_maskset) * rows * cols;
    const int s0 = bx0 / kEigStripW, s1 = bx1 / kEigStripW;
    const int c0 = by0 / chunk_rows, c1 = by1 / chunk_rows;
    const int ns = s1 - s0 + 1, R = (c1 - c0 + 1) * ns;
    const int wave = __builtin_amdgcn_readfirstlane(tid >> 6), lane = tid & 63;
    for (int rb = 0; rb < R; rb += NT) {
      if (rb + tid < R) {
        const int rg = rb + tid, c = c0 + rg / ns, sidx = s0 + rg % ns;
        const int have = (int)wcnt[(img * nchunks + c) * strips + sidx];
        if (have > wcap) s_overflow = 1;
        s_region[tid] = min(have, wcap);
      }
      __syncthreads();
      const int rend = min(NT, R - rb);
      for (int rr = wave; rr < rend; rr += NT / 64) {
        const int have = s_region[rr];
        const int rg = rb + rr, c = c0 + rg / ns, sidx = s0 + rg % ns;
        const uint2* region = cand + (size_t)((img * nchunks + c) * strips + sidx) * wcap;
        for (int i0 = 0; i0 < have; i0 += 64) {
          const int i = i0 + lane;
          uint2 r = make_uint2(0u, 0u);
          bool keep = false;
          if (i < have) {
            r = region[i];
            keep = __uint_as_float(r.x) > thr && ((mb[(r.y >> 16) * (uint32_t)cols + (r.y & 0xFFFFu)] >> m) & 1u);
          }
          const unsigned long long km = __ballot(keep);
          if (km) {
            const int leader = __ffsll((long long)km) - 1;
            int slot0 = 0;
            if (lane == leader) slot0 = atomicAdd(&s_count, __popcll(km));
            slot0 = __shfl(slot0, leader);
            const int slot = slot0 + __popcll(km & ((1ULL << lane) - 1ULL));
            if (keep && slot < CAND) keys[slot] = ((unsigned long long)sosvo_float_ordered(__uint_as_float(r.x)) << 32) | r.y;
          }
        }
      }
      __syncthreads();
    }
  }
  __syncthreads();
  const int total = s_count;
  if (redo && redo_pass == 0) {
    const int cx0_ = bx0 / cell, cy0_ = by0 / cell;
    const int gw_ = bw > 0 ? bx1 / cell - cx0_ + 1 : 0, gh_ = bh > 0 ? by1 / cell - cy0_ + 1 : 0;
    const bool fits = total <= CAND && (gw_ + 2) * (gh_ + 2) <= kSelGridCells;
    if (tid == 0) redo[p] = fits ? 0 : 1;
    if (!fits) return;
  }
  if (__builtin_expect(total > CAND, 0)) {
    const gft_regions g = {cand, wcnt, mask_bits + (size_t)(img / images_per_maskset) * rows * cols, img, m, cols, strips, nchunks, wcap,
                           bx0 / kEigStripW, by0 / chunk_rows, bx1 / kEigStripW - bx0 / kEigStripW + 1,
                           (by1 / chunk_rows - by0 / chunk_rows + 1) * (bx1 / kEigStripW - bx0 / kEigStripW + 1),
                           (float)((double)sosvo_ordered_float(st[0]) * quality)};
    gft_keep_largest<CAND, NT>(g, keys, s_region, &s_count, s_sel, tid);
    __syncthreads();
  }
  const int n = min(total, CAND);
  int N = 64;
  while (N < n) N <<= 1;
  for (int i = n + tid; i < N; i += NT) keys[i] = 0ULL;
  __syncthreads();
  for (int k = 2, lk = 1; k <= N; k <<= 1, ++lk) {
    for (int left = lk, j = k >> 1; left > 0;) {
      const int take = left >= 3 ? 3 : left;
      if (take == 3) bitonic_pass<3, NT>(keys, N, k, j, tid);
      else if (take == 2) bitonic_pass<2, NT>(keys, N, k, j, tid);
      else bitonic_pass<1, NT>(keys, N, k, j, tid);
      j >>= take;
      left -= take;
      __syncthreads();
    }
  }
  for (int i = tid; i < n; i += NT) sorted[i] = (uint32_t)keys[i];
  int stt = (total > CAND || s_overflow) ? 1 : 0;
  const int cx0 = bx0 / cell, cy0 = by0 / cell;
  const int gw = bw > 0 ? bx1 / cell - cx0 + 1 : 0, gh = bh > 0 ? by1 / cell - cy0 + 1 : 0;
  const bool use_grid = gw * gh <= kSelGridCells;
  const int limit_list = 1024;
  const float md2 = min_distance * min_distance;
  const bool spaced = min_distance >= 1.0f;
  int limit = cap;
  if (max_corners > 0 && max_corners < limit) limit = max_corners;
  const int gwp = gw + 2;
  const bool igrid = spaced && n > 0 && cell <= 2048 && rows <= 32768 && cols <= 32768 && gwp * (gh + 2) <= kSelGridCells;
  const bool fast = NT > 256 && igrid;
  __syncthreads();
  if (igrid) {
    for (int i = tid; i < gwp * (gh + 2) * 2; i += NT) grid[i] = kGridEmpty;
  } else {
    for (int i = tid; i < (use_grid ? gw * gh * 2 : 0); i += NT) grid[i] = 0u;
  }
  __syncthreads();
  if (fast) {
    const int wave = __builtin_amdgcn_readfirstlane(tid >> 6), lane = tid & 63;
    const gft_igrid ig(md2, cell, cx0, cy0, gwp);
    int accepted = 0;
    uint32_t xy_next = lane < n ? sorted[lane] : 0u;
    for (int k0 = 0; k0 < n && accepted < limit; k0 += 64) {
      const int kend = min(64, n - k0);
      const bool active = lane < kend;
      const uint32_t xy = xy_next;
      xy_next = k0 + 64 + lane < n ? sorted[k0 + 64 + lane] : 0u;
      const int y = (int)(xy >> 16), x = (int)(xy & 0xFFFFu);
      const int cidx = ig.cell_index(xy, active);
      constexpr int NWV = NT / 64;
      for (int c9 = wave; c9 < 9; c9 += NWV) {
        const unsigned long long hb = __ballot(active && ig.cell_hit(grid, cidx, c9 % 3 - 1, c9 / 3 - 1, xy) != 0u);
        if (hb && lane == 0) atomicOr(&s_prior, hb);
      }
      for (int a = wave, novf = min(s_ovf, limit_list); a < novf; a += NWV) {
        const unsigned long long hb = __ballot(active && ig.near(xy, acc_list[a]));
        if (hb && lane == 0) atomicOr(&s_prior, hb);
      }
      {
        const int first = (wave + NWV - 9 % NWV) % NWV;
        uint32_t glo = 0u, ghi = 0u;
        int t = 0;
        for (int jb = first; jb < kend; jb += 4 * NWV, t += 4) {
#pragma unroll
          for (int u = 0; u < 4; ++u) {
            const int j = min(jb + u * NWV, 63);
            const unsigned long long row = __ballot(active && ig.near(xy, (uint32_t)__builtin_amdgcn_readlane((int)xy, j)));
            const bool here = lane == t + u;
            glo = here ? (uint32_t)row : glo;
            ghi = here ? (uint32_t)(row >> 32) : ghi;
          }
        }
        const int jmine = first + lane * NWV;
        if (jmine < kend) s_conf[jmine] = ((unsigned long long)ghi << 32) | glo;
      }
      __syncthreads();
      if (wave == 0) {
        const unsigned long long alive0 = __ballot(active) & ~s_prior;
        const unsigned long long mine = active ? s_conf[lane] : 0ULL;
        const unsigned long long lt = (1ULL << lane) - 1ULL;
        const bool surv = (alive0 >> lane) & 1ULL;
        const unsigned long long fr = __ballot(surv && (mine & alive0 & lt) == 0ULL);
        unsigned long long pending = alive0 & ~fr, acc = fr;
        const int rlo = (int)(uint32_t)mine, rhi = (int)(uint32_t)(mine >> 32);
        while (pending) {
          const int j = __ffsll((long long)pending) - 1;
          pending &= pending - 1ULL;
          const unsigned long long row = ((unsigned long long)(uint32_t)__builtin_amdgcn_readlane(rhi, j) << 32) |
                                         (uint32_t)__builtin_amdgcn_readlane(rlo, j);
          if ((row & acc & ((1ULL << j) - 1ULL)) == 0ULL) acc |= 1ULL << j;
        }
        const int room = limit - accepted;
        acc = __ballot(((acc >> lane) & 1ULL) && __popcll(acc & lt) < room);
        if ((acc >> lane) & 1ULL) {
          const int pos = accepted + __popcll(acc & ((1ULL << lane) - 1ULL));
          kp[((size_t)p * cap + pos) * 2] = (float)x;
          kp[((size_t)p * cap + pos) * 2 + 1] = (float)y;
          ig.insert(grid, cidx, xy, &s_ovf, acc_list, limit_list);
        }
        if (lane == 0) {
          s_accepted = accepted + __popcll(acc);
          s_prior = 0ULL;
        }
      }
      __syncthreads();
      accepted = s_accepted;
    }
    if (s_ovf > limit_list) stt |= 2;
  } else if (NT <= 256 && igrid) {
    if (tid < 64) {
      const int lane = tid;
      const gft_igrid ig(md2, cell, cx0, cy0, gwp);
      int accepted = 0;
      uint32_t xy_next = lane < n ? sorted[lane] : 0u;
      for (int k0 = 0; k0 < n && accepted < limit; k0 += 64) {
        const int kend = min(64, n - k0);
        const bool active = lane < kend;
        const uint32_t xy = xy_next;
        xy_next = k0 + 64 + lane < n ? sorted[k0 + 64 + lane] : 0u;
        const int cidx = ig.cell_index(xy, active);
        uint32_t prior = 0u;
#pragma unroll 1
        for (int dyc = -1; dyc <= 1; ++dyc)
#pragma unroll
          for (int dxc = -1; dxc <= 1; ++dxc) prior |= ig.cell_hit(grid, cidx, dxc, dyc, xy);
        for (int a = 0, novf = min(s_ovf, limit_list); a < novf; ++a) prior |= (uint32_t)ig.near(xy, acc_list[a]);
        unsigned long long alive = __ballot(active && prior == 0u);
        unsigned long long acc = 0ULL;
        int room = limit - accepted;
        while (alive && room > 0) {
          const int j = __ffsll((long long)alive) - 1;
          alive &= alive - 1ULL;
          acc |= 1ULL << j;
          room--;
          alive &= ~__ballot(ig.near(xy, (uint32_t)__builtin_amdgcn_readlane((int)xy, j)));
        }
        if ((acc >> lane) & 1ULL) {
          const int pos = accepted + __popcll(acc & ((1ULL << lane) - 1ULL));
          kp[((size_t)p * cap + pos) * 2] = (float)(xy & 0xFFFFu);
          kp[((size_t)p * cap + pos) * 2 + 1] = (float)(xy >> 16);
          ig.insert(grid, cidx, xy, &s_ovf, acc_list, limit_list);
        }
        accepted += __popcll(acc);
      }
      if (lane == 0) s_accepted = accepted;
    }
  } else
  if (tid < 64) {
    const int lane = tid;
    if (!use_grid && limit_list < limit) {
// ... 4 lines not shown
    uint32_t xy_next = lane < n ? sorted[lane] : 0u;
    for (int k0 = 0; k0 < n && accepted < limit; k0 += 64) {
      const int kend = min(64, n - k0);
      const bool active = lane < kend;
      const uint32_t xy = xy_next;
      xy_next = k0 + 64 + lane < n ? sorted[k0 + 64 + lane] : 0u;
      const int y = (int)(xy >> 16), x = (int)(xy & 0xFFFFu);
      bool prior = false;
      if (active && spaced) {
        if (use_grid) {
          const int xc = x / cell - cx0, yc = y / cell - cy0;
#pragma unroll
          for (int c9 = 0; c9 < 9; ++c9) {
            const int xx = xc + (c9 % 3) - 1, yy = yc + (c9 / 3) - 1;
            if (xx < 0 || xx >= gw || yy < 0 || yy >= gh) continue;
            const uint2 q2 = *reinterpret_cast<const uint2*>(&grid[(yy * gw + xx) * 2]);
#pragma unroll
            for (int slot = 0; slot < 2; ++slot) {
              const uint32_t q = slot ? q2.y : q2.x;
              if (q) {
                const float dx = (float)(x - (int)((q - 1u) & 0xFFFFu)), dy = (float)(y - (int)((q - 1u) >> 16));
                prior = prior || (dx * dx + dy * dy < md2);
              }
            }
          }
          for (int a = 0, novf = min(s_ovf, limit_list); a < novf; ++a) {
            const uint32_t q = acc_list[a];
            const float dx = (float)(x - (int)(q & 0xFFFFu)), dy = (float)(y - (int)(q >> 16));
            prior = prior || (dx * dx + dy * dy < md2);
          }
        } else {
          for (int a = 0; a < accepted; ++a) {
            const uint32_t q = acc_list[a];
            const float dx = (float)(x - (int)(q & 0xFFFFu)), dy = (float)(y - (int)(q >> 16));
            prior = prior || (dx * dx + dy * dy < md2);
          }
        }
      }
      unsigned long long alive = __ballot(active && !prior);
      unsigned long long acc = 0ULL;
      int room = limit - accepted;
      while (alive && room > 0) {
        const int j = __ffsll((long long)alive) - 1;
        alive &= alive - 1ULL;
        acc |= 1ULL << j;
        room--;
        if (spaced) {
          const int xj = __builtin_amdgcn_readlane(x, j), yj = __builtin_amdgcn_readlane(y, j);
          const float dx = (float)(x - xj), dy = (float)(y - yj);
          alive &= ~__ballot(dx * dx + dy * dy < md2);
        }
      }
      if ((acc >> lane) & 1ULL) {
        const int pos = accepted + __popcll(acc & ((1ULL << lane) - 1ULL));
        kp[((size_t)p * cap + pos) * 2] = (float)x;
        kp[((size_t)p * cap + pos) * 2 + 1] = (float)y;
        if (spaced) {
          if (use_grid) {
            uint32_t* c = &grid[((y / cell - cy0) * gw + (x / cell - cx0)) * 2];
            if (atomicCAS(&c[0], 0u, xy + 1u) != 0u && atomicCAS(&c[1], 0u, xy + 1u) != 0u) {
              const int o = atomicAdd(&s_ovf, 1);
              if (o < limit_list) acc_list[o] = xy;
            }
          } else {
            acc_list[pos] = xy;
          }
        }
      }
      accepted += __popcll(acc);
    }
    if (lane == 0) s_accepted = accepted;
  }
  __syncthreads();
  if (tid == 0) {
    if (s_ovf > limit_list) stt |= 2;
    n_out[p] = min(s_accepted, cap);
    if (status) status[p] = stt;
  }
}

__global__ __launch_bounds__(kThreads) void gauss7_kernel(const uint8_t* __restrict__ gray, long long img_stride, int nimg,
                                                          int rows, int cols, int strips, int nchunks, int chunk_rows,
                                                          uint8_t* __restrict__ out, long long out_stride,
                                                          const int32_t* __restrict__ row_range, int imgs_per_range) {
  SOSVO_STREAMING_PRIO();
  const int lane = threadIdx.x & 63;
  const int wave = __builtin_amdgcn_readfirstlane((int)((blockIdx.x * kThreads + threadIdx.x) >> 6));
  if (wave >= nimg * strips * nchunks) return;
  const int img = wave / (strips * nchunks);
  const int rem = wave - img * strips * nchunks;
  const int chunk = rem / strips, strip = rem - chunk * strips;
  const int xb = strip * kEigStripW - kEigHalo;
  const int xc = xb + lane;
  const int xs = clampi(xc, 0, cols - 1);
  int src[7];
#pragma unroll
  for (int k = 0; k < 7; ++k) src[k] = clampi(refl101(xs + k - 3, cols) - xb, 0, 63);
  const bool out_lane = lane >= kEigHalo && lane < 64 - kEigHalo && xc < cols;
  int ys = chunk * chunk_rows, ye = min(rows, ys + chunk_rows);
  if (row_range) {
    const int v = img / imgs_per_range;
    ys = max(ys, row_range[2 * v]);
    ye = min(ye, row_range[2 * v + 1]);
    if (ys >= ye) return;
  }
  const uint8_t* g = gray + (size_t)img * img_stride;
  uint8_t* o = out + (size_t)img * out_stride;
  uint32_t h[7] = {0, 0, 0, 0, 0, 0, 0};
  const bool edge_strip = xb < 3 || xb + 64 > cols - 3;
  const int t_first = ys - 3, t_last = ye + 2;
  int c_pre[7];
  auto request = [&](int t0, int k0, int k1) __attribute__((always_inline)) {
#pragma unroll
    for (int k = 0; k < 7; ++k)
      if (k >= k0 && k < k1) c_pre[k] = (int)g[(uint32_t)(refl101(min(t0 + k, t_last), rows) * cols) + (uint32_t)xs];
  };
  request(t_first, 0, 7);
  auto step = [&](auto phase_tag, auto edge_tag, const int t) __attribute__((always_inline)) {
    constexpr int P = decltype(phase_tag)::value;
    constexpr bool EDGE = decltype(edge_tag)::value;
    if (t > t_last) return;
    const int c = c_pre[P];
    int l1, l2, l3, r1, r2, r3;
    if (EDGE) {
      l3 = __shfl(c, src[0]); l2 = __shfl(c, src[1]); l1 = __shfl(c, src[2]);
      r1 = __shfl(c, src[4]); r2 = __shfl(c, src[5]); r3 = __shfl(c, src[6]);
    } else {
      l1 = lane_from_left(c); l2 = lane_from_left(l1); l3 = lane_from_left(l2);
      r1 = lane_from_right(c); r2 = lane_from_right(r1); r3 = lane_from_right(r2);
    }
    h[P] = vmad24(18u, (uint32_t)(l3 + r3), vmad24(34u, (uint32_t)(l2 + r2), vmad24(49u, (uint32_t)(l1 + r1), 54u * (uint32_t)c)));
    const int y = t - 3;
    if (y < ys) return;
    const uint32_t vsum = vmad24(18u, h[(P + 1) % 7] + h[P], vmad24(34u, h[(P + 2) % 7] + h[(P + 6) % 7],
                                vmad24(49u, h[(P + 3) % 7] + h[(P + 5) % 7], 54u * h[(P + 4) % 7])));
    if (out_lane) o[(uint32_t)(y * cols) + (uint32_t)xc] = (uint8_t)((vsum + 32768u) >> 16);
  };
  auto run = [&](auto edge_tag) __attribute__((always_inline)) {
    for (int t = t_first; t <= t_last; t += 7) {
      step(std::integral_constant<int, 0>{}, edge_tag, t);
      step(std::integral_constant<int, 1>{}, edge_tag, t + 1);
      step(std::integral_constant<int, 2>{}, edge_tag, t + 2);
      step(std::integral_constant<int, 3>{}, edge_tag, t + 3);
      request(t + 7, 0, 4);
      step(std::integral_constant<int, 4>{}, edge_tag, t + 4);
      step(std::integral_constant<int, 5>{}, edge_tag, t + 5);
      step(std::integral_constant<int, 6>{}, edge_tag, t + 6);
      request(t + 7, 4, 7);
    }
  };
  if (edge_strip) run(std::true_type{}); else run(std::false_type{});
}

constexpr int kPatchMaxR = 23, kPatchRows = 48, kPatchStride = 64;
constexpr int kDescRegionBytesGft = 24 * 1024;
typedef uint32_t __attribute__((aligned(1))) u32_unaligned;

__host__ __device__ __forceinline__ int orb_patch_stride_dw(int R) { return ((2 * R + 1 + 3) >> 2) | 1; }
struct orb_pattern_table {
  int2 pt[256];
  int R, pad;
  uint16_t poff[512];
};
__global__ __launch_bounds__(256) void orb_pattern_table_kernel(const int8_t* __restrict__ pattern, float cos_a, float sin_a,
                                                                orb_pattern_table* __restrict__ tab) {
  __shared__ int s_R;
  const int t = threadIdx.x;
  if (t == 0) s_R = 0;
  __syncthreads();
  int d[4];
#pragma unroll
  for (int e = 0; e < 2; ++e) {
    const float px = (float)pattern[4 * t + 2 * e], py = (float)pattern[4 * t + 2 * e + 1];
    const float xr = (px * cos_a) - (py * sin_a), yr = (px * sin_a) + (py * cos_a);
    d[2 * e] = __float2int_rn(xr);
    d[2 * e + 1] = __float2int_rn(yr);
  }
  tab->pt[t] = make_int2((int)(((uint32_t)d[1] << 16) | ((uint32_t)d[0] & 0xFFFFu)), (int)(((uint32_t)d[3] << 16) | ((uint32_t)d[2] & 0xFFFFu)));
  atomicMax(&s_R, max(max(abs(d[0]), abs(d[1])), max(abs(d[2]), abs(d[3]))));
  __syncthreads();
  const int R = s_R;
  if (t == 0) tab->R = R;
  const int pitch = R <= kPatchMaxR ? 4 * orb_patch_stride_dw(R) : 0;
  tab->poff[2 * t] = (uint16_t)(R <= kPatchMaxR ? (d[1] + R) * pitch + (d[0] + R) : 0);
  tab->poff[2 * t + 1] = (uint16_t)(R <= kPatchMaxR ? (d[3] + R) * pitch + (d[2] + R) : 0);
}

template <int NT>
__global__ __launch_bounds__(NT) void orb_describe_kernel(const uint8_t* __restrict__ blurred, int rows, int cols,
                                                                int nmask, int cap, float* __restrict__ kp,
                                                                int32_t* __restrict__ n_io, const orb_pattern_table* __restrict__ ptab, int edge,
                                                                uint8_t* __restrict__ desc, int nimg_total,
                                                                const int32_t* __restrict__ row_range, int imgs_per_range) {
  SOSVO_LATENCY_BOUND_PRIO();
  extern __shared__ float lds_kp[];
  constexpr int kPatchWords = (NT / 64) * (kPatchRows * kPatchStride / 4);
  constexpr int kRegionWords = NT == 256 ? kDescRegionBytesGft / 4 : 0;
  __shared__ uint32_t patch_area[kPatchWords > kRegionWords ? kPatchWords : kRegionWords];
  __shared__ int wave_off[NT / 64 + 1];
  __shared__ int s_running;
  __shared__ int s_bb[4];
  const int tid = threadIdx.x, lane = tid & 63, wid = tid >> 6;
  const int p = xcd_problem(nimg_total, nmask);
  if (p < 0) return;
  const int img = p / nmask;
  const int n = min(n_io[p], cap);
  if (tid == 0) s_running = 0;
  __syncthreads();
  const int R = ptab->R;
  auto lane_offsets = [&](int pitch, int* a, int* b) __attribute__((always_inline)) {
    const int2* tp = ptab->pt;
    asm volatile("" : "+s"(tp));
#pragma unroll
    for (int r = 0; r < 4; ++r) {
      const int2 d = tp[64 * r + lane];
      a[r] = (d.x >> 16) * pitch + (int)(short)d.x;
      b[r] = (d.y >> 16) * pitch + (int)(short)d.y;
    }
  };
  const bool patch_ok = R <= kPatchMaxR && edge >= R + 1;
  const int PR = 2 * R + 1;
  int y_first = 0, y_last = rows - 1;
  if (row_range) {
    const int v = img / imgs_per_range;
    const int rr_lo = row_range[2 * v], rr_hi = row_range[2 * v + 1];
    y_first = (rr_lo <= 0 ? 0 : rr_lo + 3) + R;
    y_last = (rr_hi >= rows ? rows : rr_hi - 3) - 1 - R;
  }
  const int pdw = (PR + 3) >> 2;
  const int pstride = orb_patch_stride_dw(R);
  for (int i0 = 0; i0 < n; i0 += NT) {
    const int i = i0 + tid;
    float x = 0.f, y = 0.f;
    bool keep = false;
    if (i < n) {
      x = kp[((size_t)p * cap + i) * 2];
      y = kp[((size_t)p * cap + i) * 2 + 1];
      keep = x >= (float)edge && x < (float)(cols - edge) && y >= (float)edge && y < (float)(rows - edge);
      const int yi = __float2int_rn(y);
      keep = keep && yi >= y_first && yi <= y_last;
    }
    const int pos = sosvo_block_compact_pos<NT / 64>(keep, wave_off, &s_running, tid);
    if (keep) {
      lds_kp[2 * pos] = x;
      lds_kp[2 * pos + 1] = y;
    }
  }
  __syncthreads();
  const int m = s_running;
  for (int i = tid; i < 2 * m; i += NT) kp[(size_t)p * cap * 2 + i] = lds_kp[i];
  if (tid == 0) n_io[p] = m;
  const uint8_t* im = blurred + (size_t)img * rows * cols;
  if constexpr (NT == 256) {
    if (patch_ok && m > 0) {
      if (tid < 4) s_bb[tid] = tid < 2 ? 0x7FFFFFFF : -1;
      __syncthreads();
      for (int i = tid; i < m; i += NT) {
        const int cx = __float2int_rn(lds_kp[2 * i]), cy = __float2int_rn(lds_kp[2 * i + 1]);
        atomicMin(&s_bb[0], cx);
        atomicMin(&s_bb[1], cy);
        atomicMax(&s_bb[2], cx);
        atomicMax(&s_bb[3], cy);
      }
      __syncthreads();
      const int rx0 = s_bb[0] - R, ry0 = s_bb[1] - R, rw = s_bb[2] - s_bb[0] + PR, rh = s_bb[3] - s_bb[1] + PR;
      const int ldw = (rw + 3) >> 2, pitch_dw = ldw | 1, pitch_b = 4 * pitch_dw;
      if (pitch_b * rh <= kDescRegionBytesGft) {
        {
          const int step_r = NT / ldw, step_k = NT - step_r * ldw;
          int ry = tid / ldw, k = tid - ry * ldw;
          const uint8_t* org = im + (size_t)ry0 * cols + rx0;
          while (__any(ry < rh)) {
            uint32_t v[8];
            int dst[8];
#pragma unroll
            for (int u = 0; u < 8; ++u) {
              dst[u] = ry < rh ? ry * pitch_dw + k : -1;
              v[u] = *reinterpret_cast<const u32_unaligned*>(org + (uint32_t)(min(ry, rh - 1) * cols + 4 * k));
              k += step_k;
              ry += step_r;
              if (k >= ldw) {
                k -= ldw;
                ++ry;
              }
            }
#pragma unroll
            for (int u = 0; u < 8; ++u)
              if (dst[u] >= 0) patch_area[dst[u]] = v[u];
          }
        }
        int ra[4], rb[4];
        lane_offsets(pitch_b, ra, rb);
        __syncthreads();
        const uint8_t* region8 = reinterpret_cast<const uint8_t*>(patch_area);
        const int wid_s = __builtin_amdgcn_readfirstlane(wid);
        for (int j = wid_s; j < m; j += NT / 64) {
          const int cx = __builtin_amdgcn_readfirstlane(__float2int_rn(lds_kp[2 * j]));
          const int cy = __builtin_amdgcn_readfirstlane(__float2int_rn(lds_kp[2 * j + 1]));
          const int org = (cy - ry0) * pitch_b + (cx - rx0);
          unsigned long long* d = reinterpret_cast<unsigned long long*>(desc + ((size_t)p * cap + j) * 32);
          unsigned long long mine = 0ULL;
#pragma unroll
          for (int r = 0; r < 4; ++r) {
            const unsigned long long bal = __ballot(region8[org + ra[r]] < region8[org + rb[r]]);
            if (lane == r) mine = bal;
          }
          if (lane < 4) d[lane] = mine;
        }
        return;
      }
      __syncthreads();
    }
  }
  if (patch_ok) {
    uint32_t* patch32 = patch_area + wid * (kPatchRows * kPatchStride / 4);
    const uint8_t* patch = reinterpret_cast<const uint8_t*>(patch32);
    const int lsh = pdw <= 8 ? 3 : 4;
    const int prow = lane >> lsh, pk = min(lane & ((1 << lsh) - 1), pdw - 1);
    const int rpr = 64 >> lsh, nit = (PR + rpr - 1) / rpr;
    uint32_t reg[kPatchRows / 4];
    int goff[kPatchRows / 4], lidx[kPatchRows / 4];
#pragma unroll
    for (int it = 0; it < kPatchRows / 4; ++it) {
      const int r = min(rpr * it + prow, PR - 1);
      goff[it] = r * cols;
      lidx[it] = r * pstride + pk;
    }
    auto issue = [&](int j) {
      const uint8_t* base =
          im + ((size_t)__float2int_rn(lds_kp[2 * j + 1]) - R) * cols + (__float2int_rn(lds_kp[2 * j]) - R) + 4 * pk;
#pragma unroll
      for (int it = 0; it < kPatchRows / 4; ++it)
        if (it < nit) reg[it] = *reinterpret_cast<const u32_unaligned*>(base + goff[it]);
    };
    int pa[4], pb[4];
#pragma unroll
    for (int r = 0; r < 4; ++r) {
      pa[r] = ptab->poff[2 * (64 * r + lane)];
      pb[r] = ptab->poff[2 * (64 * r + lane) + 1];
    }
    int j = wid;
    if (j < m) issue(j);
    for (; j < m; j += NT / 64) {
#pragma unroll
      for (int it = 0; it < kPatchRows / 4; ++it)
        if (it < nit) patch32[lidx[it]] = reg[it];
      if (j + NT / 64 < m) issue(j + NT / 64);
      unsigned long long* d = reinterpret_cast<unsigned long long*>(desc + ((size_t)p * cap + j) * 32);
      unsigned long long mine = 0ULL;
#pragma unroll
      for (int r = 0; r < 4; ++r) {
        const unsigned long long bal = __ballot(patch[pa[r]] < patch[pb[r]]);
        if (lane == r) mine = bal;
      }
      if (lane < 4) d[lane] = mine;
    }
    return;
  }
  int ga[4], gb[4];
  lane_offsets(cols, ga, gb);
  for (int j = wid; j < m; j += NT / 64) {
    const uint8_t* c = im + (size_t)__float2int_rn(lds_kp[2 * j + 1]) * cols + __float2int_rn(lds_kp[2 * j]);
    unsigned long long* d = reinterpret_cast<unsigned long long*>(desc + ((size_t)p * cap + j) * 32);
#pragma unroll
    for (int r = 0; r < 4; ++r) {
      const unsigned long long bal = __ballot(c[ga[r]] < c[gb[r]]);
      if (lane == 0) d[r] = bal;
    }
  }
}

static void rolling_chunks(int nimg, int rows, int strips, int* nchunks, int* chunk_rows) {
  int nc = cdiv(16384, nimg * strips);
  if (nc > rows / 24) nc = rows / 24;
  if (nc < 1) nc = 1;
  *chunk_rows = cdiv(rows, nc);
  *nchunks = cdiv(rows, *chunk_rows);
}

}

static int32_t launch_gauss7_rows(sosvo_ctx* ctx, const uint8_t* in, long long in_stride, int nimg, int rows, int cols,
                                  uint8_t* out, long long out_stride, const int32_t* row_range, int imgs_per_range) {
  const int strips = cdiv(cols, kEigStripW);
  int nchunks, chunk_rows;
  rolling_chunks(nimg, rows, strips, &nchunks, &chunk_rows);
  SOSVO_LAUNCH(ctx, gauss7_kernel, dim3(cdiv(nimg * strips * nchunks, kThreads / 64)), dim3(kThreads), 0, ctx->stream, in,
               in_stride, nimg, rows, cols, strips, nchunks, chunk_rows, out, out_stride, row_range, imgs_per_range);
  SOSVO_LAUNCH_CHECK(ctx);
  return SOSVO_OK;
}
int32_t sosvo_launch_gauss7_rows(sosvo_ctx* ctx, const uint8_t* in, long long in_stride, int nimg, int rows, int cols,
                                 uint8_t* out, long long out_stride, const int32_t* row_range, int imgs_per_range) {
  return launch_gauss7_rows(ctx, in, in_stride, nimg, rows, cols, out, out_stride, row_range, imgs_per_range);
}
int32_t sosvo_launch_gauss7_to(sosvo_ctx* ctx, const uint8_t* in, long long in_stride, int nimg, int rows, int cols,
                               uint8_t* out, long long out_stride) {
  return launch_gauss7_rows(ctx, in, in_stride, nimg, rows, cols, out, out_stride, nullptr, 1);
}
int32_t sosvo_launch_gauss7(sosvo_ctx* ctx, const uint8_t* in, long long img_stride, int nimg, int rows, int cols,
                            uint8_t* out) {
  return sosvo_launch_gauss7_to(ctx, in, img_stride, nimg, rows, cols, out, img_stride);
}

extern "C" {

int32_t sosvo_detect_gft(sosvo_ctx* ctx, const uint8_t* gray, const uint32_t* mask_bits, int32_t nimg,
                         int32_t images_per_maskset, int32_t rows, int32_t cols, int32_t nmask, double quality,
                         double min_distance, int32_t max_corners, int32_t cap, float* kp, int32_t* n,
                         int32_t* status) {
  SOSVO_ENTER(ctx);
  SOSVO_REQUIRE(ctx, gray && mask_bits && kp && n, "null pointer");
  SOSVO_REQUIRE(ctx, nimg >= 0 && nimg <= 65535 && images_per_maskset > 0, "nimg out of range");
  SOSVO_REQUIRE(ctx, rows >= 3 && cols >= 3 && rows * (int64_t)cols < (1 << 28), "image sizes out of range");
  SOSVO_REQUIRE(ctx, rows <= 65535 && cols <= 65535, "image sizes out of range (the candidates are packed as y << 16 | x)");
  SOSVO_REQUIRE(ctx, nmask >= 1 && nmask <= kMaxMasks, "nmask out of range (1..32)");
  SOSVO_REQUIRE(ctx, cap > 0 && cap <= 4096 && quality > 0 && min_distance >= 0, "bad detector parameters (quality > 0)");
  if (nimg == 0) return SOSVO_OK;
  const size_t P = (size_t)nimg * nmask;
  size_t off = 0;
  auto carve = [&](size_t bytes) {
    size_t o = off;
    off += (bytes + 255) & ~(size_t)255;
    return o;
  };
  const int strips = cdiv(cols, kEigStripW);
  int nchunks, chunk_rows;
  rolling_chunks(nimg, rows, strips, &nchunks, &chunk_rows);
  const int wcap = (chunk_rows * kEigStripW + 63) & ~63;
  const size_t n_waves = (size_t)nimg * strips * nchunks;
  const size_t o_cand = carve(sizeof(uint2) * n_waves * wcap);
  const size_t o_wcnt = carve(sizeof(uint32_t) * n_waves);
  const size_t o_stat = carve(sizeof(uint32_t) * P * 5);
  const bool large = cap > 1024;
  const int sorted_stride = large ? kCandCapLarge : kCandCap;
  const size_t o_sorted = carve(sizeof(uint32_t) * P * sorted_stride);
  const size_t o_redo = carve(sizeof(int32_t) * P);
  int32_t rc = sosvo_ws_reserve(ctx, off);
  if (rc != SOSVO_OK) return rc;
  char* ws = (char*)ctx->ws;
  uint2* cand = (uint2*)(ws + o_cand);
  uint32_t* wcnt = (uint32_t*)(ws + o_wcnt);
  uint32_t* mstat = (uint32_t*)(ws + o_stat);
  uint32_t* sorted_g = (uint32_t*)(ws + o_sorted);
  SOSVO_HIP(ctx, hipMemsetAsync(mstat, 0, sizeof(uint32_t) * P * 5, ctx->stream));

  const int nsets = cdiv(nimg, images_per_maskset);
  SOSVO_LAUNCH(ctx, mask_bbox_kernel, dim3(rows, nsets), dim3(kThreads), 0, ctx->stream, mask_bits, images_per_maskset, rows,
               cols, nmask, mstat);
  SOSVO_LAUNCH_CHECK(ctx);
  const int waves = nimg * strips * nchunks;
  SOSVO_LAUNCH(ctx, min_eigen_kernel, dim3(cdiv(waves, kThreads / 64)), dim3(kThreads), 0, ctx->stream, gray, mask_bits, nimg,
               images_per_maskset, rows, cols, nmask, strips, nchunks, chunk_rows, wcap, cand, wcnt, mstat);
  SOSVO_LAUNCH_CHECK(ctx);
  const int cell = min_distance >= 1 ? (int)lrint(min_distance) : 1;
  int32_t* redo = (int32_t*)(ws + o_redo);
  if (large) {
    SOSVO_PROFILE(ctx, "gft_select_kernel");
    hipLaunchKernelGGL((gft_select_kernel<kCandCapLarge, 1024>), dim3(xcd_grid(nimg, nmask)), dim3(1024), 0, ctx->stream, cand, wcnt,
                       strips, nchunks, chunk_rows, wcap, mask_bits, mstat, images_per_maskset, nmask, rows, cols, quality, (float)min_distance, cell,
                       max_corners, cap, sorted_g, sorted_stride, kp, n, status, nullptr, 0, nimg);
  } else {
    SOSVO_PROFILE(ctx, "gft_select_kernel");
    auto launch = [&](auto small, auto full, int nt) {
      hipLaunchKernelGGL(small, dim3(xcd_grid(nimg, nmask)), dim3(nt), 0, ctx->stream, cand, wcnt, strips, nchunks, chunk_rows, wcap,
                         mask_bits, mstat, images_per_maskset, nmask, rows, cols, quality, (float)min_distance, cell, max_corners, cap,
                         sorted_g, sorted_stride, kp, n, status, redo, 0, nimg);
      hipLaunchKernelGGL(full, dim3(xcd_grid(nimg, nmask)), dim3(nt), 0, ctx->stream, cand, wcnt, strips, nchunks, chunk_rows, wcap,
                         mask_bits, mstat, images_per_maskset, nmask, rows, cols, quality, (float)min_distance, cell, max_corners, cap,
                         sorted_g, sorted_stride, kp, n, status, redo, 1, nimg);
    };
    if (P <= 1024)
      launch(gft_select_kernel<kCandCapSmall, 512>, gft_select_kernel<kCandCap, 512>, 512);
    else
      launch(gft_select_kernel<kCandCapSmall, kThreads>, gft_select_kernel<kCandCap, kThreads>, kThreads);
  }
  SOSVO_LAUNCH_CHECK(ctx);
  return SOSVO_OK;
}

int32_t sosvo_describe_orb(sosvo_ctx* ctx, const uint8_t* gray, int32_t nimg, int32_t rows, int32_t cols,
                           int32_t nmask, int32_t cap, float* kp, int32_t* n, float cos_a, float sin_a,
                           const int8_t* pattern, int32_t edge, uint8_t* desc) {
  return sosvo_describe_orb_rows(ctx, gray, nimg, rows, cols, nmask, cap, kp, n, cos_a, sin_a, pattern, edge, nullptr, desc);
}

int32_t sosvo_describe_orb_rows(sosvo_ctx* ctx, const uint8_t* gray, int32_t nimg, int32_t rows, int32_t cols,
                                int32_t nmask, int32_t cap, float* kp, int32_t* n, float cos_a, float sin_a,
                                const int8_t* pattern, int32_t edge, const int32_t* row_range, uint8_t* desc) {
  SOSVO_ENTER(ctx);
  SOSVO_REQUIRE(ctx, row_range == nullptr || nimg % 2 == 0, "row_range needs the two views' images (nimg even, view-major)");
  SOSVO_REQUIRE(ctx, gray && kp && n && pattern && desc, "null pointer");
  SOSVO_REQUIRE(ctx, nimg >= 0 && nimg <= 65535 && nmask >= 1, "nimg / nmask out of range");
  SOSVO_REQUIRE(ctx, rows >= 1 && cols >= 1 && rows * (int64_t)cols < (1 << 28), "image sizes out of range");
  SOSVO_REQUIRE(ctx, cap > 0 && cap <= 4096, "cap out of range");
  SOSVO_REQUIRE(ctx, edge >= 19, "edge must cover the rotated 31x31 patch (>= 19)");
  SOSVO_REQUIRE(ctx, ((uintptr_t)desc & 7) == 0, "desc must be 8-byte aligned");
  if (nimg == 0) return SOSVO_OK;
  const size_t bytes = (size_t)nimg * rows * cols;
  const size_t o_tab = (bytes + 255) & ~(size_t)255;
  int32_t rc = sosvo_ws_reserve(ctx, o_tab + sizeof(orb_pattern_table));
  if (rc != SOSVO_OK) return rc;
  uint8_t* blurred = (uint8_t*)ctx->ws;
  orb_pattern_table* ptab = (orb_pattern_table*)((char*)ctx->ws + o_tab);
  SOSVO_LAUNCH(ctx, orb_pattern_table_kernel, dim3(1), dim3(256), 0, ctx->stream, pattern, cos_a, sin_a, ptab);
  SOSVO_LAUNCH_CHECK(ctx);
  rc = launch_gauss7_rows(ctx, gray, (long long)rows * cols, nimg, rows, cols, blurred, (long long)rows * cols, row_range,
                          nimg > 1 ? nimg / 2 : 1);
  if (rc != SOSVO_OK) return rc;
  const size_t lds_kp_bytes = (size_t)cap * 2 * sizeof(float);
  const int irange = nimg > 1 ? nimg / 2 : 1;
  SOSVO_PROFILE(ctx, "orb_describe_kernel");
  auto launch = [&](auto kernel, int nt) {
    hipLaunchKernelGGL(kernel, dim3(xcd_grid(nimg, nmask)), dim3(nt), lds_kp_bytes, ctx->stream, blurred, rows, cols, nmask, cap, kp,
                       n, ptab, edge, desc, nimg, row_range, irange);
  };
  if (cap > 1024)
    launch(orb_describe_kernel<1024>, 1024);
  else if ((size_t)nimg * nmask <= 1024)
    launch(orb_describe_kernel<512>, 512);
  else
    launch(orb_describe_kernel<kThreads>, kThreads);
  SOSVO_LAUNCH_CHECK(ctx);
  return SOSVO_OK;
}

}
```

vo_single_camera_sos_amd/csrc/pipeline.hip:

```cpp
#include <vector>

#include "common.h"

namespace {

struct Carver {
  char* base;
  size_t off = 0;
  template <typename T>
  T* take(size_t count) {
    T* p = base ? reinterpret_cast<T*>(base + off) : nullptr;
    off += (count * sizeof(T) + 255) & ~(size_t)255;
    return p;
  }
};

struct OrbBufs {
  float *kp4 = nullptr, *resp = nullptr;
  uint32_t* mask_pyr = nullptr;
};
OrbBufs carve_orb(Carver& cv, int detector, size_t P, size_t cap, size_t nsets, int rows, int cols) {
  OrbBufs o;
  if (detector != SOSVO_DETECTOR_ORB) return o;
  o.kp4 = cv.take<float>(P * cap * 4);
// ... 644 lines not shown
                                 t.kp + (size_t)h * cap * 2, n_bot, t.s_keys, rig->stereo_min_disp, rig->stereo_max_hdiff, nullptr,
                                 t.lk_status));
  if (slot_of_frame)
    STAGE(sosvo_stereo_assemble_slots(ctx, rig, kp_top, kp_bot, desc_top, desc_bot, n_top, n_bot, t.s_keys, t.s_order, F,
                                      slot_of_frame, NM, cap, Fc, o.m_top, o.m_bot, o.d_top, o.d_bot, o.X, o.b_top, o.b_bot, o.M,
                                      t.n_cand));
  else
    STAGE(sosvo_stereo_assemble(ctx, rig, kp_top, kp_bot, desc_top, desc_bot, n_top, n_bot, t.s_keys, t.s_order, F, NM, cap,
                                Fc, o.m_top, o.m_bot, o.d_top, o.d_bot, o.X, o.b_top, o.b_bot, o.M, t.n_cand));
  return SOSVO_OK;
}

static int32_t correspondences_matched(sosvo_ctx* ctx, const sosvo_rig* rig, const sosvo_batch_cfg* cfg, int B, const FrameStore& s,
                                       const TrackTmp& b) {
  const int Fc = cfg->frame_cap, Cc = 2 * Fc;
  int32_t rc;
  const bool mutual = cross_f2f(*cfg);
  const Gate gate = gate_f2f(*cfg, *rig);
  if (mutual) {
    STAGE(mutual_tabs(ctx, b.cur_frame, b.ref_frame, B, b.mutual));
    STAGE(match_mutual(ctx, gate, b.ratio, s.d_top, s.m_top, s.M, B, Fc, b.mutual, b.k_top));
  } else
    STAGE(match_1nn(ctx, gate, b.ratio, s.d_top, s.d_top, s.m_top, s.m_top, s.M, s.M, b.cur_frame, b.ref_frame, B, B, Fc, b.k_top));
  STAGE(sosvo_sort_matches(ctx, b.k_top, s.M, b.cur_frame, B, Fc, b.o_top));
  if (mutual)
    STAGE(match_mutual(ctx, gate, b.ratio, s.d_bot, s.m_bot, s.M, B, Fc, b.mutual, b.k_bot));
  else
    STAGE(match_1nn(ctx, gate, b.ratio, s.d_bot, s.d_bot, s.m_bot, s.m_bot, s.M, s.M, b.cur_frame, b.ref_frame, B, B, Fc, b.k_bot));
  STAGE(sosvo_sort_matches(ctx, b.k_bot, s.M, b.cur_frame, B, Fc, b.o_bot));
  return sosvo_f2f_assemble(ctx, rig, s.m_top, s.m_bot, s.X, s.b_top, s.b_bot, s.M, Fc, b.ref_frame, b.cur_frame, b.k_top, b.o_top,
                            b.k_bot, b.o_bot, B, Cc, b.f, b.p, b.cam, b.cq, b.ct, b.cn, b.cn_top);
}

static int32_t correspondences_tracked(sosvo_ctx* ctx, const sosvo_rig* rig, const sosvo_batch_cfg* cfg, int B, const FrameStore& s,
                                       const TrackTmp& b, const sosvo_lk_images& im, const int32_t* img_rows) {
  const int Fc = cfg->frame_cap, Cc = 2 * Fc;
  int32_t rc;
  const LkTmp& k = b.lk;
  SOSVO_REQUIRE(ctx, im.level[0] && k.next, "SOSVO_FLAG_LK_F2F without the store's images");
  SOSVO_LAUNCH(ctx, lk_setup_kernel, dim3(cdiv(2 * B, 256)), dim3(256), 0, ctx->stream, B, im.slots, Fc, b.ref_frame, b.cur_frame, s.M,
               (int64_t)((s.m_bot - s.m_top) / 2), k.from, k.to, k.n, k.pt);
  SOSVO_LAUNCH_CHECK(ctx);
  STAGE(sosvo_lk_images_track(ctx, im, ctx->lk, img_rows, k.from, k.to, 2 * B, Fc, s.m_top, k.pt, k.n, k.next, k.status, k.err, k.back));
  return sosvo_f2f_assemble_tracked(ctx, rig, s.m_top, s.m_bot, s.X, s.M, Fc, b.ref_frame, k.next, k.next + (size_t)B * Fc * 2, k.status,
                                    k.status + (size_t)B * Fc, B, Cc, b.f, b.p, b.cam, b.cq, b.ct, b.cn, b.cn_top);
}

static int32_t run_tracking(sosvo_ctx* ctx, const sosvo_rig* rig, const sosvo_batch_cfg* cfg, int B, uint64_t seed,
                            const FrameStore& s, const TrackTmp& b, double* results, const uint64_t* seeds = nullptr,
                            const Workspace* images = nullptr) {
  const int Fc = cfg->frame_cap, Cc = 2 * Fc;
  int32_t rc;
  SOSVO_REQUIRE(ctx, !lk_f2f(*cfg) || images, "SOSVO_FLAG_LK_F2F without the store's images");
  if (lk_f2f(*cfg))
    STAGE(correspondences_tracked(ctx, rig, cfg, B, s, b, images->img, images->img_rows));
  else
    STAGE(correspondences_matched(ctx, rig, cfg, B, s, b));
  const int32_t rflags = SOSVO_FLAG_CAM_ROT_IDENTITY | (cfg->ransac_flags & SOSVO_FLAG_GP3P);
  if (seeds)
    STAGE(sosvo_ransac_abs_pose_seeds(ctx, b.f, b.p, b.cam, b.cam_off, b.cam_rot, 2, rflags, b.cn, B, Cc, cfg->ransac_threshold,
                                      cfg->ransac_max_iter, cfg->ransac_adaptive, seeds, b.T_ransac, b.mask, b.idx, b.n_inl,
                                      b.info, nullptr));
  else
    STAGE(sosvo_ransac_abs_pose(ctx, b.f, b.p, b.cam, b.cam_off, b.cam_rot, 2, rflags, b.cn, B, Cc, cfg->ransac_threshold,
                                cfg->ransac_max_iter, cfg->ransac_adaptive, seed, b.T_ransac, b.mask, b.idx, b.n_inl, b.info,
                                nullptr));
  SOSVO_HIP(ctx, hipMemcpyAsync(b.T, b.T_ransac, sizeof(double) * 12 * B, hipMemcpyDeviceToDevice, ctx->stream));
  STAGE(sosvo_refine_abs_pose(ctx, b.f, b.p, b.cam, b.cam_off, b.cam_rot, 2, b.cn, B, Cc, b.idx, b.n_inl, cfg->lm_max_iter,
                              b.T, b.lm_cost, b.lm_iters));
  SOSVO_LAUNCH(ctx, batch_results_kernel, dim3(cdiv(B, 256)), dim3(256), 0, ctx->stream, B, b.T, b.n_inl, b.cn, b.info,
               results);
  SOSVO_LAUNCH_CHECK(ctx);
  return SOSVO_OK;
}

static int32_t run_frame_pairs(sosvo_ctx* ctx, const sosvo_rig* rig, const sosvo_batch_cfg* cfg, const uint8_t* omni,
                               const uint32_t* unwrap_table, const uint32_t* mask_bits, const int8_t* pattern,
                               void* workspace, size_t workspace_bytes, double* results, hipEvent_t median_wait,
                               hipEvent_t median_done) {
  SOSVO_ENTER(ctx);
  SOSVO_REQUIRE(ctx, rig && cfg && omni && unwrap_table && mask_bits && pattern && workspace && results, "null pointer");
  SOSVO_REQUIRE(ctx, cfg->n_pairs > 0 && cfg->n_pairs <= 8192, "n_pairs out of range (1..8192)");
  SOSVO_REQUIRE(ctx, cfg->nmask >= 1 && cfg->nmask <= 32 && cfg->kp_cap > 0 && cfg->kp_cap <= 4096, "nmask / kp_cap out of range");
  SOSVO_REQUIRE(ctx, cfg->frame_cap > 0 && cfg->frame_cap <= 16384, "frame_cap out of range (max 16384)");
  SOSVO_REQUIRE(ctx, detector_ok(cfg->detector, cfg->kp_cap), "unknown detector, or ORB with kp_cap > 2048");
  if (omni_flags_msg(cfg->ransac_flags)) return sosvo_fail(ctx, SOSVO_ERR_ARG, __func__, omni_flags_msg(cfg->ransac_flags));
  SOSVO_REQUIRE(ctx, !lk_f2f(*cfg) || sosvo_lk_options_ok(ctx->lk), "LK settings out of range (sosvo_set_lk_options)");
  SOSVO_REQUIRE(ctx, ((uintptr_t)workspace & 255) == 0, "workspace must be 256-byte aligned");
  const int B = cfg->n_pairs, F = 2 * B;
  const Workspace ws = carve(*cfg, F, F, workspace, true);
  SOSVO_REQUIRE(ctx, workspace_bytes >= ws.bytes, "workspace too small (see sosvo_frame_pair_batch_workspace)");
  int32_t rc;
  SOSVO_LAUNCH(ctx, batch_setup_kernel, dim3(cdiv(B > 18 ? B : 18, 256)), dim3(256), 0, ctx->stream, B, foci_of(rig),
               ws.tt.ref_frame, ws.tt.cur_frame, ws.tt.cam_off, ws.tt.cam_rot);
  SOSVO_LAUNCH_CHECK(ctx);
  STAGE(run_front_end(ctx, rig, cfg, F, omni, unwrap_table, mask_bits, pattern, ws.fe, ws.store, median_wait, median_done, nullptr,
                      &ws));
  return run_tracking(ctx, rig, cfg, B, cfg->seed, ws.store, ws.tt, results, nullptr, &ws);
}

int32_t sosvo_frame_pair_batch(sosvo_ctx* ctx, const sosvo_rig* rig, const sosvo_batch_cfg* cfg, const uint8_t* omni,
                               const uint32_t* unwrap_table, const uint32_t* mask_bits, const int8_t* pattern,
                               void* workspace, size_t workspace_bytes, double* results) {
  SOSVO_ENTER(ctx);
  SOSVO_REQUIRE(ctx, rig && cfg && omni && unwrap_table && mask_bits && pattern && workspace && results, "null pointer");
  SOSVO_REQUIRE(ctx, sosvo_table_frame_ok(cfg->H, cfg->W), SOSVO_TABLE_FRAME_MSG);
  return run_frame_pairs(ctx, rig, cfg, omni, unwrap_table, mask_bits, pattern, workspace, workspace_bytes, results, nullptr,
                         nullptr);
}

static void part_range(int n, int part, int parts, int* lo, int* hi) {
  const int base = n / parts, extra = n % parts;
  *lo = part * base + (part < extra ? part : extra);
  *hi = *lo + base + (part < extra ? 1 : 0);
}

size_t sosvo_frame_pair_batch_streams_workspace(const sosvo_batch_cfg* cfg, int32_t n_streams) {
  if (!cfg || n_streams < 1 || n_streams > kSosvoMaxSubStreams || cfg->n_pairs < n_streams) return 0;
  size_t total = 0;
  for (int s = 0; s < n_streams; ++s) {
    int lo, hi;
    part_range(cfg->n_pairs, s, n_streams, &lo, &hi);
    sosvo_batch_cfg c = *cfg;
    c.n_pairs = hi - lo;
    const size_t bytes = sosvo_frame_pair_batch_workspace(&c);
    if (bytes == 0) return 0;
    total += (bytes + 255) & ~(size_t)255;
  }
  return total;
}

static int32_t sosvo_frame_pair_batch_streams_impl(sosvo_ctx* ctx, const sosvo_rig* rig, const sosvo_batch_cfg* cfg, int32_t n_streams,
                             const uint8_t* omni, const uint32_t* unwrap_table, const uint32_t* mask_bits,
                             const int8_t* pattern, void* workspace, size_t workspace_bytes, double* results, bool join) {
  SOSVO_REQUIRE(ctx, n_streams >= 1 && n_streams <= kSosvoMaxSubStreams, "n_streams out of range (1..4)");
  SOSVO_REQUIRE(ctx, cfg->n_pairs >= n_streams && cfg->n_pairs <= 8192, "n_pairs out of range (n_streams..8192)");
  SOSVO_REQUIRE(ctx, detector_ok(cfg->detector, cfg->kp_cap), "unknown detector, or ORB with kp_cap > 2048");
  if (omni_flags_msg(cfg->ransac_flags)) return sosvo_fail(ctx, SOSVO_ERR_ARG, __func__, omni_flags_msg(cfg->ransac_flags));
  SOSVO_REQUIRE(ctx, ((uintptr_t)workspace & 255) == 0, "workspace must be 256-byte aligned");
  const size_t need = sosvo_frame_pair_batch_streams_workspace(cfg, n_streams);
  SOSVO_REQUIRE(ctx, need > 0 && workspace_bytes >= need, "workspace too small (see sosvo_frame_pair_batch_streams_workspace)");
  while (ctx->n_sub < n_streams) {
    const int i = ctx->n_sub;
    if (i == 0) SOSVO_HIP(ctx, hipEventCreateWithFlags(&ctx->sub_begin, hipEventDisableTiming));
    hipStream_t st;
    SOSVO_HIP(ctx, hipStreamCreateWithFlags(&st, hipStreamNonBlocking));
    const int32_t rc = sosvo_create(&ctx->sub[i], ctx->device, st);
    if (rc != SOSVO_OK) {
      (void)hipStreamDestroy(st);
      return sosvo_fail(ctx, rc, __func__, "cannot create an internal stream context");
    }
    ctx->sub[i]->hint_shared_device = 1;
    ctx->sub[i]->hint_score_fp64_only = ctx->hint_score_fp64_only;
    SOSVO_HIP(ctx, hipEventCreateWithFlags(&ctx->sub_done[i], hipEventDisableTiming));
    SOSVO_HIP(ctx, hipEventCreateWithFlags(&ctx->sub_median[i], hipEventDisableTiming));
    ctx->n_sub = i + 1;
  }
  size_t bytes[kSosvoMaxSubStreams];
  for (int s = 0; s < n_streams; ++s) {
    int lo, hi;
    part_range(cfg->n_pairs, s, n_streams, &lo, &hi);
    sosvo_batch_cfg c = *cfg;
    c.n_pairs = hi - lo;
    bytes[s] = (sosvo_frame_pair_batch_workspace(&c) + 255) & ~(size_t)255;
  }
  if (ctx->sub_pending) {
    hipStreamCaptureStatus cap = hipStreamCaptureStatusNone;
    SOSVO_HIP(ctx, hipStreamIsCapturing(ctx->stream, &cap));
    SOSVO_REQUIRE(ctx, cap == hipStreamCaptureStatusNone,
                  "un-joined sosvo_frame_pair_batch_streams_enqueue work is pending: call ..._join before capturing");
    bool same = ctx->sub_last == n_streams && ctx->sub_last_ws == workspace;
    for (int s = 0; same && s < n_streams; ++s) same = ctx->sub_last_bytes[s] == bytes[s];
    if (!same) {
      for (int s = 0; s < ctx->sub_last; ++s) SOSVO_HIP(ctx, hipStreamWaitEvent(ctx->stream, ctx->sub_done[s], 0));
      ctx->sub_pending = 0;
    }
  }
  SOSVO_HIP(ctx, hipEventRecord(ctx->sub_begin, ctx->stream));
  char* ws = reinterpret_cast<char*>(workspace);
  hipEvent_t token = (ctx->sub_pending && ctx->sub_last > 0) ? ctx->sub_median[ctx->sub_last - 1] : nullptr;
  for (int s = 0; s < n_streams; ++s) {
    int lo, hi;
    part_range(cfg->n_pairs, s, n_streams, &lo, &hi);
    sosvo_batch_cfg c = *cfg;
    c.n_pairs = hi - lo;
    c.seed = cfg->seed + (uint64_t)lo;
    sosvo_ctx* sc = ctx->sub[s];
    sc->lk = ctx->lk;
    sc->stereo_lk = ctx->stereo_lk;
    SOSVO_HIP(ctx, hipStreamWaitEvent(sc->stream, ctx->sub_begin, 0));
    const int32_t rc = run_frame_pairs(sc, rig, &c, omni + (size_t)2 * lo * cfg->H * cfg->W * 3, unwrap_table, mask_bits, pattern,
                                       ws, bytes[s], results + (size_t)16 * lo, token, ctx->sub_median[s]);
    if (rc != SOSVO_OK) {
      (void)hipEventRecord(ctx->sub_done[s], sc->stream);
      for (int k = 0; k <= s; ++k) (void)hipStreamWaitEvent(ctx->stream, ctx->sub_done[k], 0);
      if (ctx->sub_pending)
        for (int k = s + 1; k < ctx->sub_last; ++k) (void)hipStreamWaitEvent(ctx->stream, ctx->sub_done[k], 0);
      ctx->sub_pending = 0;
      return sosvo_fail(ctx, rc, __func__, sc->err);
    }
    token = ctx->sub_median[s];
    SOSVO_HIP(ctx, hipEventRecord(ctx->sub_done[s], sc->stream));
    ws += bytes[s];
  }
  ctx->sub_last = n_streams;
  ctx->sub_last_ws = workspace;
  for (int s = 0; s < n_streams; ++s) ctx->sub_last_bytes[s] = bytes[s];
  ctx->sub_pending = join ? 0 : 1;
  if (join)
    for (int s = 0; s < n_streams; ++s) SOSVO_HIP(ctx, hipStreamWaitEvent(ctx->stream, ctx->sub_done[s], 0));
  return SOSVO_OK;
}

int32_t sosvo_frame_pair_batch_streams(sosvo_ctx* ctx, const sosvo_rig* rig, const sosvo_batch_cfg* cfg, int32_t n_streams,
                                       const uint8_t* omni, const uint32_t* unwrap_table, const uint32_t* mask_bits,
                                       const int8_t* pattern, void* workspace, size_t workspace_bytes, double* results) {
  SOSVO_ENTER(ctx);
  SOSVO_REQUIRE(ctx, rig && cfg && omni && unwrap_table && mask_bits && pattern && workspace && results, "null pointer");
  SOSVO_REQUIRE(ctx, sosvo_table_frame_ok(cfg->H, cfg->W), SOSVO_TABLE_FRAME_MSG);
  return sosvo_frame_pair_batch_streams_impl(ctx, rig, cfg, n_streams, omni, unwrap_table, mask_bits, pattern, workspace, workspace_bytes, results, true);
}

int32_t sosvo_frame_pair_batch_streams_enqueue(sosvo_ctx* ctx, const sosvo_rig* rig, const sosvo_batch_cfg* cfg,
                                               int32_t n_streams, const uint8_t* omni, const uint32_t* unwrap_table,
                                               const uint32_t* mask_bits, const int8_t* pattern, void* workspace,
                                               size_t workspace_bytes, double* results) {
  SOSVO_ENTER(ctx);
  SOSVO_REQUIRE(ctx, rig && cfg && omni && unwrap_table && mask_bits && pattern && workspace && results, "null pointer");
  SOSVO_REQUIRE(ctx, sosvo_table_frame_ok(cfg->H, cfg->W), SOSVO_TABLE_FRAME_MSG);
  return sosvo_frame_pair_batch_streams_impl(ctx, rig, cfg, n_streams, omni, unwrap_table, mask_bits, pattern, workspace, workspace_bytes, results, false);
}

int32_t sosvo_frame_pair_batch_streams_join(sosvo_ctx* ctx) {
  SOSVO_ENTER(ctx);
  for (int s = 0; s < ctx->sub_last; ++s) SOSVO_HIP(ctx, hipStreamWaitEvent(ctx->stream, ctx->sub_done[s], 0));
  ctx->sub_pending = 0;
  return SOSVO_OK;
}

size_t sosvo_rgbd_pair_batch_workspace(const sosvo_rgbd_batch_cfg* cfg) {
  if (!cfg || cfg->n_pairs <= 0 || cfg->rows <= 0 || cfg->cols <= 0 || cfg->kp_cap <= 0 || cfg->frame_cap <= 0 ||
      !detector_ok(rgbd_detector(*cfg), cfg->kp_cap) || !rgbd_flags_ok(*cfg))
    return 0;
  const size_t F = 2 * (size_t)cfg->n_pairs;
  return carve_rgbd(*cfg, F, F, nullptr).bytes;
}

static int32_t run_rgbd_front_end(sosvo_ctx* ctx, const sosvo_rgbd_cam* cam, const sosvo_rgbd_batch_cfg* cfg, int F,
                                  const uint8_t* bgr, const float* depth, const uint32_t* mask_bits, const int8_t* pattern,
                                  const RgbdFrontTmp& t, const RgbdStore& o, const int32_t* slot_of_frame = nullptr) {
  const int cap = cfg->kp_cap, Fc = cfg->frame_cap;
  int32_t rc;
  const int det = rgbd_detector(*cfg);
  STAGE(sosvo_median_gray(ctx, bgr, F, cfg->rows, cfg->cols, cfg->median_ksize, t.gray));
  if (det == SOSVO_DETECTOR_ORB) {
    STAGE(sosvo_orb_mask_pyramid(ctx, mask_bits, 1, cfg->rows, cfg->cols, 1, t.orb.mask_pyr));
    STAGE(sosvo_detect_describe_orb(ctx, t.gray, t.orb.mask_pyr, F, F, cfg->rows, cfg->cols, 1, cfg->max_corners, cap, t.orb.kp4,
                                    t.orb.resp, t.n, pattern, t.desc, t.kp));
  } else {
    if (det == SOSVO_DETECTOR_FAST || det == SOSVO_DETECTOR_AGAST)
      STAGE((det == SOSVO_DETECTOR_FAST ? sosvo_detect_fast : sosvo_detect_agast)(ctx, t.gray, mask_bits, F, F, cfg->rows, cfg->cols,
                                                                                  1, 10, cap, t.kp, t.n, t.status));
    else
      STAGE(sosvo_detect_gft(ctx, t.gray, mask_bits, F, F, cfg->rows, cfg->cols, 1, cfg->quality, cfg->min_distance,
                             cfg->max_corners, cap, t.kp, t.n, t.status));
    STAGE(sosvo_describe_orb(ctx, t.gray, F, cfg->rows, cfg->cols, 1, cap, t.kp, t.n, cfg->cos_a, cfg->sin_a, pattern, cfg->edge,
                             t.desc));
  }
  if (slot_of_frame)
    STAGE(sosvo_rgbd_assemble_slots(ctx, cam, t.kp, t.desc, t.n, depth, F, slot_of_frame, cfg->rows, cfg->cols, cap, Fc, o.m, o.d,
                                    o.X, o.b, o.M));
  else
    STAGE(sosvo_rgbd_assemble(ctx, cam, t.kp, t.desc, t.n, depth, F, cfg->rows, cfg->cols, cap, Fc, o.m, o.d, o.X, o.b, o.M));
  return SOSVO_OK;
}

static int32_t run_rgbd_tracking(sosvo_ctx* ctx, const sosvo_rgbd_batch_cfg* cfg, int B, uint64_t seed, const RgbdStore& s,
                                 const RgbdTrackTmp& b, double* results, const uint64_t* seeds = nullptr) {
  const int Fc = cfg->frame_cap;
  int32_t rc;
  const Gate gate = gate_f2f(*cfg);
  if (cross_f2f(*cfg)) {
    STAGE(mutual_tabs(ctx, b.cur_frame, b.ref_frame, B, b.mutual));
    STAGE(match_mutual(ctx, gate, b.ratio, s.d, s.m, s.M, B, Fc, b.mutual, b.keys));
  } else
    STAGE(match_1nn(ctx, gate, b.ratio, s.d, s.d, s.m, s.m, s.M, s.M, b.cur_frame, b.ref_frame, B, B, Fc, b.keys));
  STAGE(sosvo_sort_matches(ctx, b.keys, s.M, b.cur_frame, B, Fc, b.order));
  STAGE(sosvo_f2f_assemble_central(ctx, cfg->pct_good_matches, cfg->f2f_max_hdiff, s.m, s.X, s.b, s.M, Fc, b.ref_frame,
                                   b.cur_frame, b.keys, b.order, B, Fc, b.f, b.p, b.cq, b.ct, b.cn));
  const int32_t rflags = cfg->flags & (SOSVO_FLAG_EPNP | SOSVO_FLAG_GP3P | SOSVO_FLAG_TWOPT);
  if (seeds)
    STAGE(sosvo_ransac_abs_pose_seeds(ctx, b.f, b.p, nullptr, nullptr, nullptr, 1, rflags, b.cn, B, Fc, cfg->ransac_threshold,
                                      cfg->ransac_max_iter, cfg->ransac_adaptive, seeds, b.T_ransac, b.mask, b.idx, b.n_inl,
                                      b.info, nullptr));
  else
    STAGE(sosvo_ransac_abs_pose(ctx, b.f, b.p, nullptr, nullptr, nullptr, 1, rflags, b.cn, B, Fc, cfg->ransac_threshold,
                                cfg->ransac_max_iter, cfg->ransac_adaptive, seed, b.T_ransac, b.mask, b.idx, b.n_inl, b.info,
                                nullptr));
  SOSVO_HIP(ctx, hipMemcpyAsync(b.T, b.T_ransac, sizeof(double) * 12 * B, hipMemcpyDeviceToDevice, ctx->stream));
  STAGE(sosvo_refine_abs_pose(ctx, b.f, b.p, nullptr, nullptr, nullptr, 1, b.cn, B, Fc, b.idx, b.n_inl, cfg->lm_max_iter, b.T,
                              b.lm_cost, b.lm_iters));
  SOSVO_LAUNCH(ctx, batch_results_kernel, dim3(cdiv(B, 256)), dim3(256), 0, ctx->stream, B, b.T, b.n_inl, b.cn, b.info,
               results);
  SOSVO_LAUNCH_CHECK(ctx);
  return SOSVO_OK;
}
// ... 356 lines not shown
```

vo_single_camera_sos_amd/device.py:

```python
import ctypes

import torch

from . import _lib
from ._lib import SosvoError, c_f32, c_p

NULL = c_p(0)


def _ptr(t):
    return c_p(t.data_ptr()) if t is not None else NULL


def _check(t, dtype, name, shape=None, ndim=None):
    if not isinstance(t, torch.Tensor):
        raise SosvoError("%s: expected a torch tensor, got %r" % (name, type(t)))
    if not t.is_cuda:
        raise SosvoError("%s: must live on the GPU" % name)
    if t.dtype != dtype:
        raise SosvoError("%s: dtype %s, expected %s" % (name, t.dtype, dtype))
    if not t.is_contiguous():
        raise SosvoError("%s: must be contiguous" % name)
    if ndim is not None and t.dim() != ndim:
        raise SosvoError("%s: ndim %d, expected %d" % (name, t.dim(), ndim))
    if shape is not None:
        if len(shape) != t.dim() or any(s is not None and s != d for s, d in zip(shape, t.shape)):
            raise SosvoError("%s: shape %s, expected %s" % (name, tuple(t.shape), tuple(shape)))
    return t


def make_rig(pano_top, pano_bot, F_top, F_bot, min_range, max_range, stereo_min_disp=1.0, stereo_max_hdiff=2.5,
             f2f_max_hdiff=-1.0, pct_good_matches=1.0):
    r = _lib.Rig()
    for k in range(4):
        r.pano_top[k] = float(pano_top[k])
        r.pano_bot[k] = float(pano_bot[k])
    for k in range(3):
        r.F_top[k] = float(F_top[k])
        r.F_bot[k] = float(F_bot[k])
    r.min_range, r.max_range = float(min_range), float(max_range)
    r.stereo_min_disp, r.stereo_max_hdiff = float(stereo_min_disp), float(stereo_max_hdiff)
    r.f2f_max_hdiff, r.pct_good_matches = float(f2f_max_hdiff), float(pct_good_matches)
    return r


class GrayPyramid(object):

    def __init__(self, gray, upper, levels, row_range):
        self.gray, self.upper, self.levels, self.row_range = gray, upper, levels, row_range

    def level(self, l):
        NI, rows, cols = self.gray.shape
        if l == 0:
            return self.gray
        off = 0
        for k in range(1, l + 1):
            rows, cols = (rows + 1) // 2, (cols + 1) // 2
            if k < l:
                off += NI * rows * cols
        return self.upper[off:off + NI * rows * cols].view(NI, rows, cols)


class Context(object):

    def __init__(self, device=0, stream=None):
        self._lib = _lib.load()
        if not torch.cuda.is_available():
            raise SosvoError("no GPU visible: libsosvo needs an MI355X (gfx950); there is no CPU fallback")
        self.device = torch.device("cuda", device)
        torch.cuda.set_device(self.device)
        if stream is None:
            stream = torch.cuda.current_stream(self.device)
        self.stream = stream
        h = c_p()
        rc = self._lib.sosvo_create(ctypes.byref(h), int(device), c_p(stream.cuda_stream))
        if rc != 0:
            raise SosvoError("sosvo_create failed: %s" % _lib.STATUS_NAMES.get(rc, rc))
        self._h = h
        self.lk_options = _lib.LKOptions()
        self.stereo_lk_options = _lib.StereoLKOptions()

    def close(self):
        if getattr(self, "_h", None) is not None:
            self._lib.sosvo_destroy(self._h)
            self._h = None

    def __del__(self):
        try:
            self.close()
        except Exception:
            pass

    def _call(self, fn, *args):
        rc = fn(self._h, *args)
        if rc != 0:
            msg = self._lib.sosvo_last_error(self._h)
            raise SosvoError("%s -> %s: %s" % (fn.__name__, _lib.STATUS_NAMES.get(rc, rc),
                                               msg.decode() if msg else ""))

    def set_hint_shared_device(self, on=True):
        self._call(self._lib.sosvo_set_hint, _lib.HINT_SHARED_DEVICE, 1 if on else 0)

    def set_hint_match_unsplit(self, on=True):
        self._call(self._lib.sosvo_set_hint, _lib.HINT_MATCH_UNSPLIT, 1 if on else 0)

    def set_hint_score_fp64_only(self, on=True):
        self._call(self._lib.sosvo_set_hint, _lib.HINT_SCORE_FP64_ONLY, 1 if on else 0)

    def set_lk_options(self, lk=None):
        lk = _lib.LKOptions.of(lk)
        self._call(self._lib.sosvo_set_lk_options, ctypes.byref(_lib.LkOptionsStruct.of(lk)))
        self.lk_options = lk

    def set_stereo_lk_options(self, stereo_lk=None):
        o = _lib.StereoLKOptions.of(stereo_lk)
        self._call(self._lib.sosvo_set_stereo_lk_options, ctypes.byref(_lib.StereoLkOptionsStruct.of(o)))
        self.stereo_lk_options = o

    def set_stream(self, stream):
        self._call(self._lib.sosvo_set_stream, c_p(stream.cuda_stream))
        self.stream = stream

    def synchronize(self):
        self._call(self._lib.sosvo_synchronize)

    def timer_start(self):
        self._call(self._lib.sosvo_timer_start)

    def timer_stop(self):
        self._call(self._lib.sosvo_timer_stop)

    def timer_elapsed_ms(self):
        ms = c_f32()
        self._call(self._lib.sosvo_timer_elapsed_ms, ctypes.byref(ms))
        return float(ms.value)

    def debug_fill_scratch(self, byte=0xFF):
        self._call(self._lib.sosvo_debug_fill_scratch, int(byte))

    def profile_enable(self, on=True):
        self._call(self._lib.sosvo_profile_enable, 1 if on else 0)

    def profile_read(self):
        n = self._lib.sosvo_profile_count(self._h)
        buf = ctypes.create_string_buffer(128)
        ms = c_f32()
        out = []
        for i in range(n):
            self._call(self._lib.sosvo_profile_get, i, buf, 128, ctypes.byref(ms))
            out.append((buf.value.decode(), float(ms.value)))
        return out

    def unwrap(self, omni, masks, map_x, map_y, pano=None):
        _check(omni, torch.uint8, "omni", (None, None, None, 3))
        F, H, W = omni.shape[0], omni.shape[1], omni.shape[2]
        if masks is not None:
            _check(masks, torch.uint8, "masks", (2, H, W))
        _check(map_x, torch.float32, "map_x", (2, None, None))
        rows, cols = map_x.shape[1], map_x.shape[2]
        _check(map_y, torch.float32, "map_y", (2, rows, cols))
        if pano is None:
            pano = torch.empty((2, F, rows, cols, 3), dtype=torch.uint8, device=omni.device)
        _check(pano, torch.uint8, "pano", (2, F, rows, cols, 3))
        self._call(self._lib.sosvo_unwrap, _ptr(omni), _ptr(masks), _ptr(map_x), _ptr(map_y), F, H, W, rows, cols,
                   _ptr(pano))
        return pano

    def unwrap_prepare(self, masks, map_x, map_y, omni_shape):
        H, W = omni_shape
        if masks is not None:
            _check(masks, torch.uint8, "masks", (2, H, W))
        _check(map_x, torch.float32, "map_x", (2, None, None))
        rows, cols = map_x.shape[1], map_x.shape[2]
        _check(map_y, torch.float32, "map_y", (2, rows, cols))
        table = torch.empty((2, rows, cols, 2), dtype=torch.uint32, device=map_x.device)
        self._call(self._lib.sosvo_unwrap_prepare, _ptr(masks), _ptr(map_x), _ptr(map_y), H, W, rows, cols, _ptr(table))
        return table

    def unwrap_table(self, omni, table, pano=None):
        _check(omni, torch.uint8, "omni", (None, None, None, 3))
        F, H, W = omni.shape[0], omni.shape[1], omni.shape[2]
        _check(table, torch.uint32, "table", (2, None, None, 2))
        rows, cols = table.shape[1], table.shape[2]
        if pano is None:
            pano = torch.empty((2, F, rows, cols, 3), dtype=torch.uint8, device=omni.device)
        _check(pano, torch.uint8, "pano", (2, F, rows, cols, 3))
        self._call(self._lib.sosvo_unwrap_table, _ptr(omni), _ptr(table), F, H, W, rows, cols, _ptr(pano))
        return pano

    def median_gray(self, img, ksize, gray=None):
        _check(img, torch.uint8, "img")
        if img.dim() < 3 or img.shape[-1] != 3:
            raise SosvoError("img: expected [..., rows, cols, 3]")
        rows, cols = img.shape[-3], img.shape[-2]
        nimg = int(img.numel() // (rows * cols * 3))
        if gray is None:
            gray = torch.empty(tuple(img.shape[:-1]), dtype=torch.uint8, device=img.device)
        _check(gray, torch.uint8, "gray", tuple(img.shape[:-1]))
        self._call(self._lib.sosvo_median_gray, _ptr(img), nimg, rows, cols, int(ksize), _ptr(gray))
        return gray

    def gray_rows_needed(self, mask_bits, nmask, edge, pattern, cos_a, sin_a):
        _check(mask_bits, torch.uint32, "mask_bits", (None, None, None))
        _check(pattern, torch.int8, "pattern")
        nsets, rows, cols = mask_bits.shape
        out = torch.zeros((nsets, 2), dtype=torch.int32, device=mask_bits.device)
        self._call(self._lib.sosvo_gray_rows_needed, _ptr(mask_bits), nsets, rows, cols, int(nmask), int(edge), _ptr(pattern),
                   float(cos_a), float(sin_a), _ptr(out))
        return out

    def unwrap_median_gray(self, omni, table, ksize, gray=None, row_range=None):
        _check(omni, torch.uint8, "omni", (None, None, None, 3))
        F, H, W = omni.shape[0], omni.shape[1], omni.shape[2]
        _check(table, torch.uint32, "table", (2, None, None, 2))
        rows, cols = table.shape[1], table.shape[2]
        if gray is None:
            gray = torch.empty((2 * F, rows, cols), dtype=torch.uint8, device=omni.device)
        _check(gray, torch.uint8, "gray", (2 * F, rows, cols))
        if row_range is None:
            self._call(self._lib.sosvo_unwrap_median_gray, _ptr(omni), _ptr(table), F, H, W, rows, cols, int(ksize), _ptr(gray))
        else:
            _check(row_range, torch.int32, "row_range", (2, 2))
            self._call(self._lib.sosvo_unwrap_median_gray_rows, _ptr(omni), _ptr(table), F, H, W, rows, cols, int(ksize),
                       _ptr(row_range), _ptr(gray))
        return gray

    def detect_agast(self, gray, mask_bits, images_per_maskset, nmask, cap, threshold=10, kp=None, n=None, status=None):
        return self.detect_fast(gray, mask_bits, images_per_maskset, nmask, cap, threshold, kp, n, status, _agast=True)

    def detect_fast(self, gray, mask_bits, images_per_maskset, nmask, cap, threshold=10, kp=None, n=None, status=None,
                    _agast=False):
        _check(gray, torch.uint8, "gray", ndim=3)
        NI, rows, cols = gray.shape
        _check(mask_bits, torch.uint32, "mask_bits", (None, rows, cols))
        if mask_bits.shape[0] * images_per_maskset < NI:
            raise SosvoError("mask_bits has too few sets for %d images" % NI)
        P, dev = NI * nmask, gray.device
        if kp is None:
            kp = torch.zeros((P, cap, 2), dtype=torch.float32, device=dev)
        if n is None:
            n = torch.zeros((P,), dtype=torch.int32, device=dev)
        if status is None:
            status = torch.zeros((P,), dtype=torch.int32, device=dev)
        _check(kp, torch.float32, "kp", (P, cap, 2))
        _check(n, torch.int32, "n", (P,))
        _check(status, torch.int32, "status", (P,))
        self._call(self._lib.sosvo_detect_agast if _agast else self._lib.sosvo_detect_fast, _ptr(gray), _ptr(mask_bits), NI,
                   int(images_per_maskset), rows, cols, int(nmask), int(threshold), int(cap), _ptr(kp), _ptr(n), _ptr(status))
        return kp, n, status

    def detect_gft(self, gray, mask_bits, images_per_maskset, nmask, cap, quality=0.01, min_distance=5.0,
                   max_corners=1000, kp=None, n=None, status=None):
        _check(gray, torch.uint8, "gray", ndim=3)
        NI, rows, cols = gray.shape
        _check(mask_bits, torch.uint32, "mask_bits", (None, rows, cols))
        if mask_bits.shape[0] * images_per_maskset < NI:
            raise SosvoError("mask_bits has too few sets for %d images" % NI)
        P = NI * nmask
        dev = gray.device
        if kp is None:
            kp = torch.zeros((P, cap, 2), dtype=torch.float32, device=dev)
        if n is None:
            n = torch.zeros((P,), dtype=torch.int32, device=dev)
        if status is None:
            status = torch.zeros((P,), dtype=torch.int32, device=dev)
        _check(kp, torch.float32, "kp", (P, cap, 2))
        _check(n, torch.int32, "n", (P,))
        _check(status, torch.int32, "status", (P,))
        self._call(self._lib.sosvo_detect_gft, _ptr(gray), _ptr(mask_bits), NI, int(images_per_maskset), rows, cols,
                   int(nmask), float(quality), float(min_distance), int(max_corners), int(cap), _ptr(kp), _ptr(n),
                   _ptr(status))
        return kp, n, status

    def describe_orb(self, gray, kp, n, nmask, pattern, cos_a, sin_a, edge=31, desc=None, row_range=None):
        _check(gray, torch.uint8, "gray", ndim=3)
        NI, rows, cols = gray.shape
        P = NI * nmask
        _check(kp, torch.float32, "kp", (P, None, 2))
        cap = kp.shape[1]
        _check(n, torch.int32, "n", (P,))
        _check(pattern, torch.int8, "pattern", (512, 2))
        if desc is None:
            desc = torch.zeros((P, cap, 32), dtype=torch.uint8, device=gray.device)
        _check(desc, torch.uint8, "desc", (P, cap, 32))
        if row_range is not None:
            _check(row_range, torch.int32, "row_range", (2, 2))
        self._call(self._lib.sosvo_describe_orb_rows, _ptr(gray), NI, rows, cols, int(nmask), cap, _ptr(kp), _ptr(n),
                   float(cos_a), float(sin_a), _ptr(pattern), int(edge), _ptr(row_range), _ptr(desc))
        return desc

    def refine_subpix(self, gray, kp, n, nmask, half=5, max_iter=_lib.SUBPIX_MAX_ITER, eps=_lib.SUBPIX_EPS, row_range=None):
        _check(gray, torch.uint8, "gray", ndim=3)
        NI, rows, cols = gray.shape
        P = NI * nmask
        _check(kp, torch.float32, "kp", (P, None, 2))
        _check(n, torch.int32, "n", (P,))
        if row_range is not None:
            _check(row_range, torch.int32, "row_range", (2, 2))
        self._call(self._lib.sosvo_refine_subpix, _ptr(gray), NI, rows, cols, int(nmask), kp.shape[1], _ptr(kp), _ptr(n),
                   int(half), int(max_iter), float(eps), _ptr(row_range))
        return kp

    def gray_pyramid(self, gray, levels, row_range=None, out=None):
        _check(gray, torch.uint8, "gray", ndim=3)
        NI, rows, cols = gray.shape
        nbytes = _lib.gray_pyramid_bytes(NI, rows, cols, levels)
        if row_range is not None:
            _check(row_range, torch.int32, "row_range", (2, 2))
        upper = out.upper if out is not None else torch.zeros((nbytes,), dtype=torch.uint8, device=gray.device)
        _check(upper, torch.uint8, "out.upper", (nbytes,))
        self._call(self._lib.sosvo_gray_pyramid, _ptr(gray), NI, rows, cols, int(levels), _ptr(row_range),
                   _ptr(upper) if nbytes else NULL)
        return GrayPyramid(gray, upper, int(levels), row_range)

    def track_lk(self, pyr, prev_img, next_img, prev_pts, n, half=10, max_iter=30, eps=0.01, min_eig=1e-4, next_pts=None,
                 fb_max=None, out=None):
        if not isinstance(pyr, GrayPyramid):
            raise SosvoError("pyr: expected the result of gray_pyramid")
        NI, rows, cols = pyr.gray.shape
        _check(prev_pts, torch.float32, "prev_pts", (None, None, 2))
        NP, cap = prev_pts.shape[:2]
        _check(prev_img, torch.int32, "prev_img", (NP,))
        _check(next_img, torch.int32, "next_img", (NP,))
        _check(n, torch.int32, "n", (NP,))
        flags = 0
        if next_pts is not None:
            flags = _lib.LK_INITIAL_FLOW
        else:
            next_pts = out[0] if out is not None else torch.zeros_like(prev_pts)
        _check(next_pts, torch.float32, "next_pts", (NP, cap, 2))
        dev = prev_pts.device
        status = out[1] if out is not None else torch.zeros((NP, cap), dtype=torch.uint8, device=dev)
        err = out[2] if out is not None else torch.zeros((NP, cap), dtype=torch.float32, device=dev)
        _check(status, torch.uint8, "status", (NP, cap))
        _check(err, torch.float32, "err", (NP, cap))
        back = None
        if fb_max is not None:
            back = out[3] if out is not None and len(out) > 3 else torch.zeros_like(prev_pts)
            _check(back, torch.float32, "back", (NP, cap, 2))
        self._call(self._lib.sosvo_track_lk, _ptr(pyr.gray), _ptr(pyr.upper) if pyr.upper.numel() else NULL, NI, rows, cols,
                   pyr.levels, _ptr(pyr.row_range), _ptr(prev_img), _ptr(next_img), NP, cap, _ptr(prev_pts), _ptr(n), int(half),
                   int(max_iter), float(eps), float(min_eig), flags, _ptr(next_pts), _ptr(status), _ptr(err), _ptr(back),
                   0.0 if fb_max is None else float(fb_max))
        return (next_pts, status, err) if fb_max is None else (next_pts, status, err, back)

    def refine_stereo_lk(self, gray, kp_top, n_top, kp_bot, n_bot, keys, nmask, stereo_min_disp=-1.0, stereo_max_hdiff=0.0,
                         stereo_lk=None, row_range=None, status=None):
        o = _lib.StereoLKOptions.of(stereo_lk)
        _check(gray, torch.uint8, "gray", ndim=3)
        NI, rows, cols = gray.shape
        if NI % 2:
            raise SosvoError("gray: expected the top and bottom views' images, view-major (an even count)")
        P = (NI // 2) * int(nmask)
        _check(kp_bot, torch.float32, "kp_bot", (P, None, 2))
        cap = kp_bot.shape[1]
        _check(kp_top, torch.float32, "kp_top", (P, cap, 2))
        _check(n_top, torch.int32, "n_top", (P,))
        _check(n_bot, torch.int32, "n_bot", (P,))
        _check(keys, torch.uint32, "keys")
        if tuple(keys.shape) not in ((P, cap), (P, cap, 1)):
            raise SosvoError("keys: expected shape %r (k = 1), got %r" % ((P, cap), tuple(keys.shape)))
        if row_range is not None:
            _check(row_range, torch.int32, "row_range", (2, 2))
        if status is None:
            status = torch.zeros((P, cap), dtype=torch.uint8, device=gray.device)
        _check(status, torch.uint8, "status", (P, cap))
        opt = _lib.StereoLkOptionsStruct.of(o)
        self._call(self._lib.sosvo_refine_stereo_lk, _ptr(gray), NI, rows, cols, _ptr(row_range), int(nmask), cap, _ptr(kp_top),
                   _ptr(n_top), _ptr(kp_bot), _ptr(n_bot), _ptr(keys), float(stereo_min_disp), float(stereo_max_hdiff),
                   ctypes.cast(ctypes.pointer(opt), c_p), _ptr(status))
        return kp_bot, status

    def f2f_assemble_tracked(self, rig, frames, ref_frame, trk_top, trk_bot, st_top, st_bot, corr_cap, out=None):
        F, frame_cap = frames["m_top"].shape[0], frames["m_top"].shape[1]
        NP = ref_frame.shape[0]
        _check(ref_frame, torch.int32, "ref_frame", (NP,))
        _check(frames["m_top"], torch.float32, "m_top", (F, frame_cap, 2))
        _check(frames["m_bot"], torch.float32, "m_bot", (F, frame_cap, 2))
        _check(frames["X"], torch.float64, "X", (F, frame_cap, 3))
        _check(frames["M"], torch.int32, "M", (F,))
        for name, t in (("trk_top", trk_top), ("trk_bot", trk_bot)):
            _check(t, torch.float32, name, (NP, frame_cap, 2))
        for name, t in (("st_top", st_top), ("st_bot", st_bot)):
            _check(t, torch.uint8, name, (NP, frame_cap))
        dev = ref_frame.device
        if out is None:
            out = dict(f=torch.zeros((NP, corr_cap, 3), dtype=torch.float64, device=dev),
                       p=torch.zeros((NP, corr_cap, 3), dtype=torch.float64, device=dev),
                       cam=torch.zeros((NP, corr_cap), dtype=torch.int32, device=dev),
                       q=torch.zeros((NP, corr_cap), dtype=torch.int32, device=dev),
                       t=torch.zeros((NP, corr_cap), dtype=torch.int32, device=dev),
                       n=torch.zeros((NP,), dtype=torch.int32, device=dev),
                       n_top=torch.zeros((NP,), dtype=torch.int32, device=dev))
        _check(out["f"], torch.float64, "f", (NP, corr_cap, 3))
        _check(out["p"], torch.float64, "p", (NP, corr_cap, 3))
        for k in ("cam", "q", "t"):
            _check(out[k], torch.int32, k, (NP, corr_cap))
        _check(out["n"], torch.int32, "n", (NP,))
        _check(out["n_top"], torch.int32, "n_top", (NP,))
        self._call(self._lib.sosvo_f2f_assemble_tracked, ctypes.cast(ctypes.pointer(rig), c_p), _ptr(frames["m_top"]),
                   _ptr(frames["m_bot"]), _ptr(frames["X"]), _ptr(frames["M"]), frame_cap, _ptr(ref_frame), _ptr(trk_top),
                   _ptr(trk_bot), _ptr(st_top), _ptr(st_bot), NP, corr_cap, _ptr(out["f"]), _ptr(out["p"]), _ptr(out["cam"]),
                   _ptr(out["q"]), _ptr(out["t"]), _ptr(out["n"]), _ptr(out["n_top"]))
        return out

    def orb_pyramid_pixels(self, rows, cols):
        return int(self._lib.sosvo_orb_pyramid_pixels(int(rows), int(cols)))

    def orb_mask_pyramid(self, mask_bits, nmask):
        _check(mask_bits, torch.uint32, "mask_bits", ndim=3)
        nsets, rows, cols = mask_bits.shape
        out = torch.zeros((nsets, self.orb_pyramid_pixels(rows, cols)), dtype=torch.uint32, device=mask_bits.device)
        self._call(self._lib.sosvo_orb_mask_pyramid, _ptr(mask_bits), nsets, rows, cols, int(nmask), _ptr(out))
        return out

    def detect_orb(self, gray, mask_pyr, images_per_maskset, nmask, nfeatures, cap, kp4=None, resp=None, n=None):
        _check(gray, torch.uint8, "gray", ndim=3)
        NI, rows, cols = gray.shape
        _check(mask_pyr, torch.uint32, "mask_pyr", (None, self.orb_pyramid_pixels(rows, cols)))
        if mask_pyr.shape[0] * images_per_maskset < NI:
            raise SosvoError("mask_pyr has too few sets for %d images" % NI)
        P = NI * nmask
        dev = gray.device
        if kp4 is None:
            kp4 = torch.zeros((P, cap, 4), dtype=torch.float32, device=dev)
        if resp is None:
            resp = torch.zeros((P, cap), dtype=torch.float32, device=dev)
        if n is None:
            n = torch.zeros((P,), dtype=torch.int32, device=dev)
        _check(kp4, torch.float32, "kp4", (P, cap, 4))
        _check(resp, torch.float32, "resp", (P, cap))
        _check(n, torch.int32, "n", (P,))
        self._call(self._lib.sosvo_detect_orb, _ptr(gray), _ptr(mask_pyr), NI, int(images_per_maskset), rows, cols,
                   int(nmask), int(nfeatures), int(cap), _ptr(kp4), _ptr(resp), _ptr(n))
        return kp4, resp, n

    def describe_orb_levels(self, gray, kp4, n, nmask, pattern, desc=None, kp_xy=None):
        _check(gray, torch.uint8, "gray", ndim=3)
        NI, rows, cols = gray.shape
        P = NI * nmask
        _check(kp4, torch.float32, "kp4", (P, None, 4))
        cap = kp4.shape[1]
# ... 620 lines not shown
```

Baseline: 66780.

## Add wide two-columns-per-lane min-eigen and blur kernels with rolling narrow hint

Adds a wide min-eigenvalue detection kernel in which each lane handles two adjacent columns, so one wave covers two candidate strips. Rows are loaded as 4-byte unaligned words and the next row's loads are prefetched in a rotating three-slot pipeline. A matching wide blur layout (4 columns per lane) and a new gauss7 entry point are added, and the select kernel now takes a variable strip width. A new hint flag, default off, appears to choose the old narrow path, so the wide path likely becomes the default; this trades more registers and edge-case complexity for fewer waves and more work per load.

```diff
diff --git a/include/sosvo.h b/include/sosvo.h
--- a/include/sosvo.h
+++ b/include/sosvo.h
@@ -33,6 +33,7 @@
 #define SOSVO_HINT_SHARED_DEVICE 1
 #define SOSVO_HINT_SCORE_FP64_ONLY 2
 #define SOSVO_HINT_MATCH_UNSPLIT 3
+#define SOSVO_HINT_ROLLING_NARROW 4
 int32_t sosvo_set_hint(sosvo_ctx* ctx, int32_t hint, int32_t value);
 int32_t sosvo_synchronize(sosvo_ctx* ctx);
 const char* sosvo_last_error(const sosvo_ctx* ctx);
@@ -73,6 +74,13 @@
                          int32_t images_per_maskset, int32_t rows, int32_t cols, int32_t nmask,
                          double quality, double min_distance, int32_t max_corners, int32_t cap,
                          float* kp, int32_t* n, int32_t* status);
+
+int32_t sosvo_detect_gft_candidates(sosvo_ctx* ctx, const uint8_t* gray, const uint32_t* mask_bits, int32_t nimg,
+                                    int32_t images_per_maskset, int32_t rows, int32_t cols, int32_t nmask, int32_t* geometry,
+                                    uint32_t* cand_out, uint32_t* wcnt_out, uint32_t* mstat_out);
+
+int32_t sosvo_gauss7(sosvo_ctx* ctx, const uint8_t* gray, int32_t nimg, int32_t rows, int32_t cols, int64_t img_stride,
+                     uint8_t* out, int64_t out_stride, const int32_t* row_range);
 
 int32_t sosvo_describe_orb(sosvo_ctx* ctx, const uint8_t* gray, int32_t nimg, int32_t rows, int32_t cols,
                            int32_t nmask, int32_t cap, float* kp, int32_t* n, float cos_a, float sin_a,
diff --git a/vo_single_camera_sos_amd/_lib.py b/vo_single_camera_sos_amd/_lib.py
--- a/vo_single_camera_sos_amd/_lib.py
+++ b/vo_single_camera_sos_amd/_lib.py
@@ -54,6 +54,9 @@
     "sosvo_gray_rows_needed": (c_i32, [c_p, c_p, c_i32, c_i32, c_i32, c_i32, c_i32, c_p, c_f32, c_f32, c_p]),
     "sosvo_detect_gft": (c_i32, [c_p, c_p, c_p, c_i32, c_i32, c_i32, c_i32, c_i32, c_f64, c_f64, c_i32, c_i32, c_p,
                                  c_p, c_p]),
+    "sosvo_detect_gft_candidates": (c_i32, [c_p, c_p, c_p, c_i32, c_i32, c_i32, c_i32, c_i32, ctypes.POINTER(c_i32), c_p, c_p,
+                                            c_p]),
+    "sosvo_gauss7": (c_i32, [c_p, c_p, c_i32, c_i32, c_i32, ctypes.c_int64, c_p, ctypes.c_int64, c_p]),
     "sosvo_describe_orb": (c_i32, [c_p, c_p, c_i32, c_i32, c_i32, c_i32, c_i32, c_p, c_p, c_f32, c_f32, c_p, c_i32,
                                    c_p]),
     "sosvo_describe_orb_rows": (c_i32, [c_p, c_p, c_i32, c_i32, c_i32, c_i32, c_i32, c_p, c_p, c_f32, c_f32, c_p, c_i32,
@@ -133,6 +136,7 @@
 HINT_SHARED_DEVICE = 1
 HINT_SCORE_FP64_ONLY = 2
 HINT_MATCH_UNSPLIT = 3
+HINT_ROLLING_NARROW = 4
 FLAG_CAM_ROT_IDENTITY = 1
 FLAG_EPNP = 2
 FLAG_GP3P = 4
diff --git a/vo_single_camera_sos_amd/csrc/common.h b/vo_single_camera_sos_amd/csrc/common.h
--- a/vo_single_camera_sos_amd/csrc/common.h
+++ b/vo_single_camera_sos_amd/csrc/common.h
@@ -32,6 +32,7 @@
   int32_t hint_score_fp64_only;
   int32_t hint_shared_device;
   int32_t hint_match_unsplit;
+  int32_t hint_rolling_narrow;
   sosvo_lk_options lk;
   sosvo_stereo_lk_options stereo_lk;
   int32_t sub_last;
diff --git a/vo_single_camera_sos_amd/csrc/ctx.hip b/vo_single_camera_sos_amd/csrc/ctx.hip
--- a/vo_single_camera_sos_amd/csrc/ctx.hip
+++ b/vo_single_camera_sos_amd/csrc/ctx.hip
@@ -74,6 +74,10 @@
       if (ctx->sub[i]) ctx->sub[i]->hint_score_fp64_only = value != 0;
   } else if (hint == SOSVO_HINT_MATCH_UNSPLIT) {
     ctx->hint_match_unsplit = value != 0;
+  } else if (hint == SOSVO_HINT_ROLLING_NARROW) {
+    ctx->hint_rolling_narrow = value != 0;
+    for (int i = 0; i < ctx->n_sub; ++i)
+      if (ctx->sub[i]) ctx->sub[i]->hint_rolling_narrow = value != 0;
   } else {
     return sosvo_fail(ctx, SOSVO_ERR_ARG, __func__, "unknown hint");
   }
diff --git a/vo_single_camera_sos_amd/csrc/detect.hip b/vo_single_camera_sos_amd/csrc/detect.hip
--- a/vo_single_camera_sos_amd/csrc/detect.hip
+++ b/vo_single_camera_sos_amd/csrc/detect.hip
@@ -1,4 +1,5 @@
 #include "common.h"
+#include "rolling_layout.h"
 
 #include <type_traits>
 
@@ -9,6 +10,8 @@
 constexpr int kCandCapSmall = 2048;
 constexpr int kCandCapLarge = 16384;
 constexpr int kMaxMasks = 32;
+typedef uint32_t __attribute__((aligned(1))) u32_unaligned;
+typedef uint16_t __attribute__((aligned(1))) u16_unaligned;
 
 __device__ __forceinline__ float sqrt_rn_normal(float x) {
   const float s = __builtin_amdgcn_sqrtf(x);
@@ -179,6 +182,213 @@
   }
 }
 
+constexpr int kEigWideStripW = 61;
+constexpr int kEigWideMinCols = 8;
+
+__global__ __launch_bounds__(kThreads) void min_eigen_wide_kernel(const uint8_t* __restrict__ gray,
+                                                                  const uint32_t* __restrict__ mask_bits, int nimg,
+                                                                  int images_per_maskset, int rows, int cols, int nmask,
+                                                                  int strips, int nchunks, int chunk_rows, int wcap,
+                                                                  uint2* __restrict__ cand, uint32_t* __restrict__ wcnt,
+                                                                  uint32_t* __restrict__ mstat) {
+  SOSVO_STREAMING_PRIO();
+  const int lane = threadIdx.x & 63;
+  const int spairs = (strips + 1) >> 1;
+  const int wave = __builtin_amdgcn_readfirstlane((int)((blockIdx.x * kThreads + threadIdx.x) >> 6));
+  if (wave >= nimg * spairs * nchunks) return;
+  const int img = wave / (spairs * nchunks);
+  const int rem = wave - img * spairs * nchunks;
+  const int chunk = rem / spairs, sp = rem - chunk * spairs;
+  const int reg_a = (img * nchunks + chunk) * strips + 2 * sp;
+  const bool has_b = 2 * sp + 1 < strips;
+  const int xb = sp * (2 * kEigWideStripW) - kEigHalo;
+  const int x_lo = xb + 2 * lane, x_hi = x_lo + 1;
+  const bool own_lo = lane >= 2 && lane <= 62 && x_lo < cols, own_hi = lane >= 1 && lane <= 61 && x_hi < cols;
+  const bool cd_lo = own_lo && x_lo >= 1 && x_lo <= cols - 2, cd_hi = own_hi && x_hi >= 1 && x_hi <= cols - 2;
+  const uint32_t mask_all = nmask < 32 ? (1u << nmask) - 1u : 0xFFFFFFFFu;
+  const uint32_t am_lo = own_lo ? mask_all : 0u, am_hi = own_hi ? mask_all : 0u;
+  auto mirror = [&](int x) { return clampi(x < 0 ? -x : (x >= cols ? 2 * (cols - 1) - x : x), 0, cols - 1); };
+  const int m_lo = mirror(x_lo), m_hi = mirror(x_hi);
+  const int ld_col = clampi(min(m_lo, m_hi), 0, cols - 4);
+  const uint32_t src_col = (uint32_t)ld_col;
+  const uint32_t sh_lo = 8u * (uint32_t)clampi(m_lo - ld_col, 0, 3), sh_hi = 8u * (uint32_t)clampi(m_hi - ld_col, 0, 3);
+  const uint32_t neg_lo = (x_lo < 0 || x_lo >= cols) ? 0x80000000u : 0u, neg_hi = (x_hi < 0 || x_hi >= cols) ? 0x80000000u : 0u;
+  uint32_t* mstat_img = mstat + (size_t)img * nmask * 5;
+  int r_lo = rows, r_hi = 0;
+  {
+    const uint32_t* sbb = mstat + (size_t)(img / images_per_maskset) * images_per_maskset * nmask * 5;
+    for (int m = 0; m < nmask; ++m) {
+      const uint32_t y1 = sbb[m * 5 + 4];
+      if (y1) {
+        r_lo = min(r_lo, (int)(0xFFFFFFFFu - sbb[m * 5 + 2]));
+        r_hi = max(r_hi, (int)y1);
+      }
+    }
+  }
+  const int ys = max(chunk * chunk_rows, r_lo), ye = min(min(rows, chunk * chunk_rows + chunk_rows), r_hi);
+  if (ys >= ye) {
+    if (lane == 0) {
+      wcnt[reg_a] = 0u;
+      if (has_b) wcnt[reg_a + 1] = 0u;
+    }
+    return;
+  }
+  const int e_lo = max(ys - 1, 0), e_hi = min(ye, rows - 1);
+  const int f_lo = max(ys, 1), f_hi = min(ye, rows - 1) - 1;
+  const uint8_t* g = gray + (size_t)img * rows * cols;
+  uint2* region = cand + (size_t)(reg_a + (lane >> 5)) * wcap;
+  int wpos_a = 0, wpos_b = 0;
+  const uint32_t* mb = mask_bits + (size_t)(img / images_per_maskset) * rows * cols;
+  const float scale = (float)(1.0 / 3060.0);
+
+  int hd_l[3] = {0, 0, 0}, hs_l[3] = {0, 0, 0}, hd_h[3] = {0, 0, 0}, hs_h[3] = {0, 0, 0};
+  float pxx_l[3] = {0.f, 0.f, 0.f}, pxy_l[3] = {0.f, 0.f, 0.f}, pyy_l[3] = {0.f, 0.f, 0.f};
+  float pxx_h[3] = {0.f, 0.f, 0.f}, pxy_h[3] = {0.f, 0.f, 0.f}, pyy_h[3] = {0.f, 0.f, 0.f};
+  float hm_l[3] = {0.f, 0.f, 0.f}, ec_l[3] = {0.f, 0.f, 0.f}, hm_h[3] = {0.f, 0.f, 0.f}, ec_h[3] = {0.f, 0.f, 0.f};
+  uint32_t bits_l = 0u, max_l = 0u, bits_h = 0u, max_h = 0u;
+  uint32_t mprev_l = 0u, mprev_h = 0u;
+  const int t_first = e_lo - 2, t_last = e_hi + 2;
+  const bool edge_strip = xb < 0 || xb + 128 > cols;
+  uint32_t c_pre[3] = {0u, 0u, 0u}, mw_l[3] = {0u, 0u, 0u}, mw_h[3] = {0u, 0u, 0u};
+  auto request = [&](auto slot_tag, auto edge_tag, const int t) __attribute__((always_inline)) {
+    constexpr int P = decltype(slot_tag)::value;
+    constexpr bool EDGE = decltype(edge_tag)::value;
+    c_pre[P] = *reinterpret_cast<const u32_unaligned*>(g + ((uint32_t)(refl101(min(t, t_last), rows) * cols) + src_col));
+    const int y = t - 2;
+    mw_l[P] = 0u;
+    mw_h[P] = 0u;
+    if (y >= ys && y < ye) {
+      if (EDGE) {
+        if (own_lo) mw_l[P] = mb[(uint32_t)(y * cols) + (uint32_t)x_lo];
+        if (own_hi) mw_h[P] = mb[(uint32_t)(y * cols) + (uint32_t)x_hi];
+      } else {
+        uint32_t w[2];
+        __builtin_memcpy(w, mb + ((uint32_t)(y * cols) + (uint32_t)x_lo), 8);
+        mw_l[P] = w[0];
+        mw_h[P] = w[1];
+      }
+    }
+  };
+  auto eig = [&](float xx0, float xx1, float xx2, float xy0, float xy1, float xy2, float yy0, float yy1, float yy2) {
+    const float a = ((xx0 + xx1) + xx2) * 0.5f, b = (xy0 + xy1) + xy2;
+    const float c = ((yy0 + yy1) + yy2) * 0.5f;
+    return (a + c) - sqrt_rn_normal(((a - c) * (a - c)) + (b * b));
+  };
+  auto step = [&](auto phase_tag, auto edge_tag, const int t) __attribute__((always_inline)) {
+    constexpr int P = decltype(phase_tag)::value;
+    constexpr bool EDGE = decltype(edge_tag)::value;
+    constexpr int i0 = (P + 1) % 3, i1 = (P + 2) % 3, i2 = P;
+    if (t > t_last) return;
+    const uint32_t c = c_pre[P];
+    const uint32_t mb_l = mw_l[P] & am_lo, mb_h = mw_h[P] & am_hi;
+    request(phase_tag, edge_tag, t + 3);
+    {
+      const int cl = (int)((c >> sh_lo) & 0xFFu), ch = (int)((c >> sh_hi) & 0xFFu);
+      const int l = lane_from_left(ch), r = lane_from_right(cl);
+      hd_l[i2] = ch - l;
+      hs_l[i2] = (l + 2 * cl) + ch;
+      hd_h[i2] = r - cl;
+      hs_h[i2] = (cl + 2 * ch) + r;
+    }
+    const int v = t - 1;
+    if (v < e_lo - 1) return;
+    {
+      const float dx_l = (float)((hd_l[i0] + 2 * hd_l[i1]) + hd_l[i2]) * scale, dy_l = (float)(hs_l[i2] - hs_l[i0]) * scale;
+      const float dx_h = (float)((hd_h[i0] + 2 * hd_h[i1]) + hd_h[i2]) * scale, dy_h = (float)(hs_h[i2] - hs_h[i0]) * scale;
+      const float xx_l = dx_l * dx_l, yy_l = dy_l * dy_l, xx_h = dx_h * dx_h, yy_h = dy_h * dy_h;
+      float xy_l = dx_l * dy_l, xy_h = dx_h * dy_h;
+      if (v < 0 || v >= rows) {
+        xy_l = -xy_l;
+        xy_h = -xy_h;
+      }
+      if (EDGE) {
+        xy_l = __uint_as_float(__float_as_uint(xy_l) ^ neg_lo);
+        xy_h = __uint_as_float(__float_as_uint(xy_h) ^ neg_hi);
+      }
+      pxx_l[i2] = (lane_from_left(xx_h) + xx_l) + xx_h;
+      pxx_h[i2] = (xx_l + xx_h) + lane_from_right(xx_l);
+      pxy_l[i2] = (lane_from_left(xy_h) + xy_l) + xy_h;
+      pxy_h[i2] = (xy_l + xy_h) + lane_from_right(xy_l);
+      pyy_l[i2] = (lane_from_left(yy_h) + yy_l) + yy_h;
+      pyy_h[i2] = (yy_l + yy_h) + lane_from_right(yy_l);
+    }
+    const int y = v - 1;
+    if (y < e_lo) return;
+    {
+      const float e_l = eig(pxx_l[i0], pxx_l[i1], pxx_l[i2], pxy_l[i0], pxy_l[i1], pxy_l[i2], pyy_l[i0], pyy_l[i1], pyy_l[i2]);
+      const float e_h = eig(pxx_h[i0], pxx_h[i1], pxx_h[i2], pxy_h[i0], pxy_h[i1], pxy_h[i2], pyy_h[i0], pyy_h[i1], pyy_h[i2]);
+      if (mb_l != bits_l) {
+        eig_flush(mstat_img, bits_l, max_l);
+        bits_l = mb_l;
+        max_l = 0u;
+      }
+      max_l = max(max_l, sosvo_float_ordered(e_l));
+      if (mb_h != bits_h) {
+        eig_flush(mstat_img, bits_h, max_h);
+        bits_h = mb_h;
+        max_h = 0u;
+      }
+      max_h = max(max_h, sosvo_float_ordered(e_h));
+      hm_l[i2] = fmaxf(fmaxf(lane_from_left(e_h), e_l), e_h);
+      hm_h[i2] = fmaxf(fmaxf(e_l, e_h), lane_from_right(e_l));
+      ec_l[i2] = e_l;
+      ec_h[i2] = e_h;
+    }
+    const int f = y - 1;
+    const uint32_t mf_l = mprev_l, mf_h = mprev_h;
+    mprev_l = mb_l;
+    mprev_h = mb_h;
+    if (f < f_lo || f > f_hi) return;
+    {
+      const float ev_l = ec_l[i1], ev_h = ec_h[i1];
+      const bool is_l = cd_lo && ev_l == fmaxf(fmaxf(hm_l[i0], hm_l[i1]), hm_l[i2]) && ev_l > 0.0f && mf_l != 0u;
+      const bool is_h = cd_hi && ev_h == fmaxf(fmaxf(hm_h[i0], hm_h[i1]), hm_h[i2]) && ev_h > 0.0f && mf_h != 0u;
+      const unsigned long long bal_l = __ballot(is_l), bal_h = __ballot(is_h);
+      if (bal_l | bal_h) {
+        const uint32_t al = (uint32_t)bal_l, ah = (uint32_t)bal_h, bl = (uint32_t)(bal_l >> 32), bh = (uint32_t)(bal_h >> 32);
+        const int below_a = (int)__builtin_amdgcn_mbcnt_lo(al, __builtin_amdgcn_mbcnt_lo(ah, 0u));
+        const int below_b = (int)__builtin_amdgcn_mbcnt_hi(bl, __builtin_amdgcn_mbcnt_hi(bh, 0u));
+        const int pos_l = lane < 32 ? wpos_a + below_a : wpos_b + below_b, pos_h = pos_l + (is_l ? 1 : 0);
+        if (is_l && pos_l < wcap) region[pos_l] = make_uint2(__float_as_uint(ev_l), ((uint32_t)f << 16) | (uint32_t)x_lo);
+        if (is_h && pos_h < wcap) region[pos_h] = make_uint2(__float_as_uint(ev_h), ((uint32_t)f << 16) | (uint32_t)x_hi);
+        wpos_a += __popc(al) + __popc(ah);
+        wpos_b += __popc(bl) + __popc(bh);
+      }
+    }
+  };
+  auto run = [&](auto edge_tag) __attribute__((always_inline)) {
+    request(std::integral_constant<int, 0>{}, edge_tag, t_first);
+    request(std::integral_constant<int, 1>{}, edge_tag, t_first + 1);
+    request(std::integral_constant<int, 2>{}, edge_tag, t_first + 2);
+    for (int t = t_first; t <= t_last; t += 3) {
+      step(std::integral_constant<int, 0>{}, edge_tag, t);
+      step(std::integral_constant<int, 1>{}, edge_tag, t + 1);
+      step(std::integral_constant<int, 2>{}, edge_tag, t + 2);
+    }
+  };
+  if (edge_strip) run(std::true_type{}); else run(std::false_type{});
+  if (lane == 0) {
+    wcnt[reg_a] = (uint32_t)wpos_a;
+    if (has_b) wcnt[reg_a + 1] = (uint32_t)wpos_b;
+  }
+  auto finish = [&](uint32_t cur_bits, uint32_t cur_max) __attribute__((always_inline)) {
+    const unsigned long long act = __ballot(cur_bits != 0u);
+    if (act) {
+      const int first = __ffsll((long long)act) - 1;
+      const uint32_t b0 = __shfl(cur_bits, first);
+      if (__ballot(cur_bits != 0u && cur_bits != b0) == 0ULL) {
+        uint32_t om = cur_bits != 0u ? cur_max : 0u;
+        for (int s = 32; s > 0; s >>= 1) om = max(om, (uint32_t)__shfl_down((int)om, s));
+        if (lane == 0) eig_flush(mstat_img, b0, om);
+      } else {
+        eig_flush(mstat_img, cur_bits, cur_max);
+      }
+    }
+  };
+  finish(bits_l, max_l);
+  finish(bits_h, max_h);
+}
+
 __global__ __launch_bounds__(kThreads) void mask_bbox_kernel(const uint32_t* __restrict__ mask_bits, int images_per_maskset,
                                                              int rows, int cols, int nmask, uint32_t* __restrict__ mstat) {
   __shared__ uint32_t sb[2][kMaxMasks];
@@ -357,7 +567,7 @@
 
 template <int CAND, int NT>
 __global__ __launch_bounds__(NT) void gft_select_kernel(const uint2* __restrict__ cand,
-                                                              const uint32_t* __restrict__ wcnt, int strips, int nchunks,
+                                                              const uint32_t* __restrict__ wcnt, int strip_w, int strips, int nchunks,
                                                               int chunk_rows, int wcap, const uint32_t* __restrict__ mask_bits,
                                                               const uint32_t* __restrict__ mstat, int images_per_maskset,
                                                               int nmask, int rows, int cols, double quality,
@@ -401,7 +611,7 @@
   if (any && bw > 0 && bh > 0) {
     const float thr = (float)((double)sosvo_ordered_float(st[0]) * quality);
     const uint32_t* mb = mask_bits + (size_t)(img / images_per_maskset) * rows * cols;
-    const int s0 = bx0 / kEigStripW, s1 = bx1 / kEigStripW;
+    const int s0 = bx0 / strip_w, s1 = bx1 / strip_w;
     const int c0 = by0 / chunk_rows, c1 = by1 / chunk_rows;
     const int ns = s1 - s0 + 1, R = (c1 - c0 + 1) * ns;
     const int wave = __builtin_amdgcn_readfirstlane(tid >> 6), lane = tid & 63;
@@ -451,8 +661,8 @@
   }
   if (__builtin_expect(total > CAND, 0)) {
     const gft_regions g = {cand, wcnt, mask_bits + (size_t)(img / images_per_maskset) * rows * cols, img, m, cols, strips, nchunks, wcap,
-                           bx0 / kEigStripW, by0 / chunk_rows, bx1 / kEigStripW - bx0 / kEigStripW + 1,
-                           (by1 / chunk_rows - by0 / chunk_rows + 1) * (bx1 / kEigStripW - bx0 / kEigStripW + 1),
+                           bx0 / strip_w, by0 / chunk_rows, bx1 / strip_w - bx0 / strip_w + 1,
+                           (by1 / chunk_rows - by0 / chunk_rows + 1) * (bx1 / strip_w - bx0 / strip_w + 1),
                            (float)((double)sosvo_ordered_float(st[0]) * quality)};
     gft_keep_largest<CAND, NT>(g, keys, s_region, &s_count, s_sel, tid);
     __syncthreads();
@@ -763,9 +973,91 @@
   if (edge_strip) run(std::true_type{}); else run(std::false_type{});
 }
 
+__global__ __launch_bounds__(kThreads) void gauss7_wide_kernel(const uint8_t* __restrict__ gray, long long img_stride, int nimg,
+                                                               int rows, int cols, int strips, int nchunks, int chunk_rows,
+                                                               uint8_t* __restrict__ out, long long out_stride,
+                                                               const int32_t* __restrict__ row_range, int imgs_per_range) {
+  SOSVO_STREAMING_PRIO();
+  const int lane = threadIdx.x & 63;
+  const int wave = __builtin_amdgcn_readfirstlane((int)((blockIdx.x * kThreads + threadIdx.x) >> 6));
+  if (wave >= nimg * strips * nchunks) return;
+  const int img = wave / (strips * nchunks);
+  const int rem = wave - img * strips * nchunks;
+  const int chunk = rem / strips, strip = rem - chunk * strips;
+  const sosvo_blur_wide_lane lay = sosvo_blur_wide_layout(cols, strip, lane);
+  const int x0 = strip * SOSVO_BLUR_WIDE_STRIP_W - 3 + 4 * lane;
+  int ys = chunk * chunk_rows, ye = min(rows, ys + chunk_rows);
+  if (row_range) {
+    const int v = img / imgs_per_range;
+    ys = max(ys, row_range[2 * v]);
+    ye = min(ye, row_range[2 * v + 1]);
+    if (ys >= ye) return;
+  }
+  const uint8_t* g = gray + (size_t)img * img_stride;
+  uint8_t* o = out + (size_t)img * out_stride;
+  const int jb = lay.own ? __builtin_ctz(lay.own) : 0, nb = __builtin_popcount(lay.own);
+  const bool st_dword = nb == 4, st_short = nb == 2 || nb == 3, st_byte = nb == 1 || nb == 3;
+  const uint32_t st_x = (uint32_t)(x0 + jb), st_shift = 8u * (uint32_t)jb;
+  const uint32_t st_xb = (uint32_t)(x0 + jb + nb - 1), st_shiftb = 8u * (uint32_t)(st_byte ? jb + nb - 1 : 0);
+  const uint32_t ld_x = (uint32_t)lay.off;
+  uint32_t h[7][4];
+#pragma unroll
+  for (int k = 0; k < 7; ++k) h[k][0] = h[k][1] = h[k][2] = h[k][3] = 0u;
+  const bool edge_strip = sosvo_blur_wide_edge_strip(cols, strip) != 0;
+  const int t_first = ys - 3, t_last = ye + 2;
+  const uint32_t w_lo = 0x36312212u, w_hi = 0x00122231u;
+  uint32_t c_pre[7];
+  auto request = [&](int t0, int k0, int k1) __attribute__((always_inline)) {
+#pragma unroll
+    for (int k = 0; k < 7; ++k)
+      if (k >= k0 && k < k1)
+        c_pre[k] = *reinterpret_cast<const u32_unaligned*>(g + ((uint32_t)(refl101(min(t0 + k, t_last), rows) * cols) + ld_x));
+  };
+  request(t_first, 0, 7);
+  auto step = [&](auto phase_tag, auto edge_tag, const int t) __attribute__((always_inline)) {
+    constexpr int P = decltype(phase_tag)::value;
+    constexpr bool EDGE = decltype(edge_tag)::value;
+    if (t > t_last) return;
+    uint32_t c = c_pre[P];
+    if (EDGE) c = __builtin_amdgcn_perm(c, c, lay.sel);
+    const uint32_t l = (uint32_t)lane_from_left((int)c), r = (uint32_t)lane_from_right((int)c);
+#pragma unroll
+    for (int j = 0; j < 3; ++j)
+      h[P][j] = __builtin_amdgcn_udot4(__builtin_amdgcn_alignbyte(c, l, j + 1), w_lo,
+                                       __builtin_amdgcn_udot4(__builtin_amdgcn_alignbyte(r, c, j + 1), w_hi, 0u, false), false);
+    h[P][3] = __builtin_amdgcn_udot4(c, w_lo, __builtin_amdgcn_udot4(r, w_hi, 0u, false), false);
+    const int y = t - 3;
+    if (y < ys) return;
+    uint32_t s[4];
+#pragma unroll
+    for (int j = 0; j < 4; ++j)
+      s[j] = vmad24(18u, h[(P + 1) % 7][j] + h[P][j], vmad24(34u, h[(P + 2) % 7][j] + h[(P + 6) % 7][j],
+                    vmad24(49u, h[(P + 3) % 7][j] + h[(P + 5) % 7][j], vmad24(54u, h[(P + 4) % 7][j], 32768u))));
+    const uint32_t p01 = __builtin_amdgcn_perm(s[1], s[0], 0x0C0C0602u), p23 = __builtin_amdgcn_perm(s[3], s[2], 0x0C0C0602u);
+    const uint32_t pk = __builtin_amdgcn_perm(p23, p01, 0x05040100u);
+    const uint32_t oy = (uint32_t)(y * cols);
+    if (st_dword) *reinterpret_cast<u32_unaligned*>(o + (oy + st_x)) = pk;
+    if (st_short) *reinterpret_cast<u16_unaligned*>(o + (oy + st_x)) = (uint16_t)(pk >> st_shift);
+    if (st_byte) o[oy + st_xb] = (uint8_t)(pk >> st_shiftb);
+  };
+  auto run = [&](auto edge_tag) __attribute__((always_inline)) {
+    for (int t = t_first; t <= t_last; t += 7) {
+      step(std::integral_constant<int, 0>{}, edge_tag, t);
+      step(std::integral_constant<int, 1>{}, edge_tag, t + 1);
+      step(std::integral_constant<int, 2>{}, edge_tag, t + 2);
+      step(std::integral_constant<int, 3>{}, edge_tag, t + 3);
+      request(t + 7, 0, 4);
+      step(std::integral_constant<int, 4>{}, edge_tag, t + 4);
+      step(std::integral_constant<int, 5>{}, edge_tag, t + 5);
+      step(std::integral_constant<int, 6>{}, edge_tag, t + 6);
+      request(t + 7, 4, 7);
+    }
+  };
+  if (edge_strip) run(std::true_type{}); else run(std::false_type{});
+}
+
 constexpr int kPatchMaxR = 23, kPatchRows = 48, kPatchStride = 64;
 constexpr int kDescRegionBytesGft = 24 * 1024;
-typedef uint32_t __attribute__((aligned(1))) u32_unaligned;
 
 __host__ __device__ __forceinline__ int orb_patch_stride_dw(int R) { return ((2 * R + 1 + 3) >> 2) | 1; }
 struct orb_pattern_table {
@@ -989,12 +1281,31 @@
   *nchunks = cdiv(rows, *chunk_rows);
 }
 
+static void rolling_chunks_wide(int nimg, int rows, int strips, int* nchunks, int* chunk_rows) {
+  int nc = cdiv(6144, nimg * strips);
+  if (nc > rows / 24) nc = rows / 24;
+  if (nc < 1) nc = 1;
+  *chunk_rows = cdiv(rows, nc);
+  *nchunks = cdiv(rows, *chunk_rows);
+}
+
 }
 
 static int32_t launch_gauss7_rows(sosvo_ctx* ctx, const uint8_t* in, long long in_stride, int nimg, int rows, int cols,
                                   uint8_t* out, long long out_stride, const int32_t* row_range, int imgs_per_range) {
+  int nchunks, chunk_rows;
+  if (cols >= SOSVO_BLUR_WIDE_MIN_COLS && !ctx->hint_rolling_narrow) {
+    const int strips = sosvo_blur_wide_strips(cols);
+    rolling_chunks_wide(nimg, rows, strips, &nchunks, &chunk_rows);
+    {
+      SOSVO_PROFILE(ctx, "gauss7_kernel");
+      hipLaunchKernelGGL(gauss7_wide_kernel, dim3(cdiv(nimg * strips * nchunks, kThreads / 64)), dim3(kThreads), 0, ctx->stream, in,
+                         in_stride, nimg, rows, cols, strips, nchunks, chunk_rows, out, out_stride, row_range, imgs_per_range);
+    }
+    SOSVO_LAUNCH_CHECK(ctx);
+    return SOSVO_OK;
+  }
   const int strips = cdiv(cols, kEigStripW);
-  int nchunks, chunk_rows;
   rolling_chunks(nimg, rows, strips, &nchunks, &chunk_rows);
   SOSVO_LAUNCH(ctx, gauss7_kernel, dim3(cdiv(nimg * strips * nchunks, kThreads / 64)), dim3(kThreads), 0, ctx->stream, in,
                in_stride, nimg, rows, cols, strips, nchunks, chunk_rows, out, out_stride, row_range, imgs_per_range);
@@ -1014,7 +1325,89 @@
   return sosvo_launch_gauss7_to(ctx, in, img_stride, nimg, rows, cols, out, img_stride);
 }
 
+struct gft_plan {
+  bool wide;
+  int strip_w, strips, nchunks, chunk_rows, wcap, waves;
+  size_t n_regions, o_cand, o_wcnt, o_stat, end;
+};
+static gft_plan gft_plan_make(const sosvo_ctx* ctx, int nimg, int rows, int cols, int nmask) {
+  gft_plan g;
+  g.wide = cols >= kEigWideMinCols && !ctx->hint_rolling_narrow;
+  g.strip_w = g.wide ? kEigWideStripW : kEigStripW;
+  g.strips = cdiv(cols, g.strip_w);
+  if (g.wide)
+    rolling_chunks_wide(nimg, rows, cdiv(g.strips, 2), &g.nchunks, &g.chunk_rows);
+  else
+    rolling_chunks(nimg, rows, g.strips, &g.nchunks, &g.chunk_rows);
+  g.waves = nimg * g.nchunks * (g.wide ? cdiv(g.strips, 2) : g.strips);
+  g.wcap = (g.chunk_rows * g.strip_w + 63) & ~63;
+  g.n_regions = (size_t)nimg * g.strips * g.nchunks;
+  size_t off = 0;
+  auto carve = [&](size_t bytes) {
+    size_t o = off;
+    off += (bytes + 255) & ~(size_t)255;
+    return o;
+  };
+  g.o_cand = carve(sizeof(uint2) * g.n_regions * g.wcap);
+  g.o_wcnt = carve(sizeof(uint32_t) * g.n_regions);
+  g.o_stat = carve(sizeof(uint32_t) * (size_t)nimg * nmask * 5);
+  g.end = off;
+  return g;
+}
+static int32_t gft_launch_response(sosvo_ctx* ctx, const gft_plan& g, const uint8_t* gray, const uint32_t* mask_bits, int nimg,
+                                   int images_per_maskset, int rows, int cols, int nmask) {
+  char* ws = (char*)ctx->ws;
+  uint2* cand = (uint2*)(ws + g.o_cand);
+  uint32_t* wcnt = (uint32_t*)(ws + g.o_wcnt);
+  uint32_t* mstat = (uint32_t*)(ws + g.o_stat);
+  SOSVO_HIP(ctx, hipMemsetAsync(mstat, 0, sizeof(uint32_t) * (size_t)nimg * nmask * 5, ctx->stream));
+  const int nsets = cdiv(nimg, images_per_maskset);
+  SOSVO_LAUNCH(ctx, mask_bbox_kernel, dim3(rows, nsets), dim3(kThreads), 0, ctx->stream, mask_bits, images_per_maskset, rows,
+               cols, nmask, mstat);
+  SOSVO_LAUNCH_CHECK(ctx);
+  if (g.wide) {
+    SOSVO_PROFILE(ctx, "min_eigen_kernel");
+    hipLaunchKernelGGL(min_eigen_wide_kernel, dim3(cdiv(g.waves, kThreads / 64)), dim3(kThreads), 0, ctx->stream, gray, mask_bits,
+                       nimg, images_per_maskset, rows, cols, nmask, g.strips, g.nchunks, g.chunk_rows, g.wcap, cand, wcnt, mstat);
+  } else {
+    SOSVO_LAUNCH(ctx, min_eigen_kernel, dim3(cdiv(g.waves, kThreads / 64)), dim3(kThreads), 0, ctx->stream, gray, mask_bits, nimg,
+                 images_per_maskset, rows, cols, nmask, g.strips, g.nchunks, g.chunk_rows, g.wcap, cand, wcnt, mstat);
+  }
+  SOSVO_LAUNCH_CHECK(ctx);
+  return SOSVO_OK;
+}
+
 extern "C" {
+
+int32_t sosvo_detect_gft_candidates(sosvo_ctx* ctx, const uint8_t* gray, const uint32_t* mask_bits, int32_t nimg,
+                                    int32_t images_per_maskset, int32_t rows, int32_t cols, int32_t nmask, int32_t* geometry,
+                                    uint32_t* cand_out, uint32_t* wcnt_out, uint32_t* mstat_out) {
+  SOSVO_ENTER(ctx);
+  SOSVO_REQUIRE(ctx, geometry, "null pointer");
+  SOSVO_REQUIRE(ctx, nimg >= 1 && nimg <= 65535 && images_per_maskset > 0, "nimg out of range");
+  SOSVO_REQUIRE(ctx, rows >= 3 && cols >= 3 && rows * (int64_t)cols < (1 << 28), "image sizes out of range");
+  SOSVO_REQUIRE(ctx, rows <= 65535 && cols <= 65535, "image sizes out of range (the candidates are packed as y << 16 | x)");
+  SOSVO_REQUIRE(ctx, nmask >= 1 && nmask <= kMaxMasks, "nmask out of range (1..32)");
+  const gft_plan g = gft_plan_make(ctx, nimg, rows, cols, nmask);
+  SOSVO_REQUIRE(ctx, g.n_regions * (size_t)g.wcap < ((size_t)1 << 31), "too many candidate slots for this entry point");
+  geometry[0] = g.strip_w;
+  geometry[1] = g.strips;
+  geometry[2] = g.nchunks;
+  geometry[3] = g.chunk_rows;
+  geometry[4] = g.wcap;
+  geometry[5] = (int32_t)g.n_regions;
+  if (!cand_out && !wcnt_out && !mstat_out) return SOSVO_OK;
+  SOSVO_REQUIRE(ctx, gray && mask_bits && cand_out && wcnt_out && mstat_out, "null pointer");
+  int32_t rc = sosvo_ws_reserve(ctx, g.end);
+  if (rc != SOSVO_OK) return rc;
+  rc = gft_launch_response(ctx, g, gray, mask_bits, nimg, images_per_maskset, rows, cols, nmask);
+  if (rc != SOSVO_OK) return rc;
+  const char* ws = (const char*)ctx->ws;
+  SOSVO_HIP(ctx, hipMemcpyAsync(cand_out, ws + g.o_cand, sizeof(uint2) * g.n_regions * g.wcap, hipMemcpyDeviceToDevice, ctx->stream));
+  SOSVO_HIP(ctx, hipMemcpyAsync(wcnt_out, ws + g.o_wcnt, sizeof(uint32_t) * g.n_regions, hipMemcpyDeviceToDevice, ctx->stream));
+  SOSVO_HIP(ctx, hipMemcpyAsync(mstat_out, ws + g.o_stat, sizeof(uint32_t) * (size_t)nimg * nmask * 5, hipMemcpyDeviceToDevice, ctx->stream));
+  return SOSVO_OK;
+}
 
 int32_t sosvo_detect_gft(sosvo_ctx* ctx, const uint8_t* gray, const uint32_t* mask_bits, int32_t nimg,
                          int32_t images_per_maskset, int32_t rows, int32_t cols, int32_t nmask, double quality,
@@ -1029,20 +1422,14 @@
   SOSVO_REQUIRE(ctx, cap > 0 && cap <= 4096 && quality > 0 && min_distance >= 0, "bad detector parameters (quality > 0)");
   if (nimg == 0) return SOSVO_OK;
   const size_t P = (size_t)nimg * nmask;
-  size_t off = 0;
+  const gft_plan g = gft_plan_make(ctx, nimg, rows, cols, nmask);
+  size_t off = g.end;
   auto carve = [&](size_t bytes) {
     size_t o = off;
     off += (bytes + 255) & ~(size_t)255;
     return o;
   };
-  const int strips = cdiv(cols, kEigStripW);
-  int nchunks, chunk_rows;
-  rolling_chunks(nimg, rows, strips, &nchunks, &chunk_rows);
-  const int wcap = (chunk_rows * kEigStripW + 63) & ~63;
-  const size_t n_waves = (size_t)nimg * strips * nchunks;
-  const size_t o_cand = carve(sizeof(uint2) * n_waves * wcap);
-  const size_t o_wcnt = carve(sizeof(uint32_t) * n_waves);
-  const size_t o_stat = carve(sizeof(uint32_t) * P * 5);
+  const int strip_w = g.strip_w, strips = g.strips, nchunks = g.nchunks, chunk_rows = g.chunk_rows, wcap = g.wcap;
   const bool large = cap > 1024;
   const int sorted_stride = large ? kCandCapLarge : kCandCap;
   const size_t o_sorted = carve(sizeof(uint32_t) * P * sorted_stride);
@@ -1050,34 +1437,26 @@
   int32_t rc = sosvo_ws_reserve(ctx, off);
   if (rc != SOSVO_OK) return rc;
   char* ws = (char*)ctx->ws;
-  uint2* cand = (uint2*)(ws + o_cand);
-  uint32_t* wcnt = (uint32_t*)(ws + o_wcnt);
-  uint32_t* mstat = (uint32_t*)(ws + o_stat);
+  uint2* cand = (uint2*)(ws + g.o_cand);
+  uint32_t* wcnt = (uint32_t*)(ws + g.o_wcnt);
+  uint32_t* mstat = (uint32_t*)(ws + g.o_stat);
   uint32_t* sorted_g = (uint32_t*)(ws + o_sorted);
-  SOSVO_HIP(ctx, hipMemsetAsync(mstat, 0, sizeof(uint32_t) * P * 5, ctx->stream));
-
-  const int nsets = cdiv(nimg, images_per_maskset);
-  SOSVO_LAUNCH(ctx, mask_bbox_kernel, dim3(rows, nsets), dim3(kThreads), 0, ctx->stream, mask_bits, images_per_maskset, rows,
-               cols, nmask, mstat);
-  SOSVO_LAUNCH_CHECK(ctx);
-  const int waves = nimg * strips * nchunks;
-  SOSVO_LAUNCH(ctx, min_eigen_kernel, dim3(cdiv(waves, kThreads / 64)), dim3(kThreads), 0, ctx->stream, gray, mask_bits, nimg,
-               images_per_maskset, rows, cols, nmask, strips, nchunks, chunk_rows, wcap, cand, wcnt, mstat);
-  SOSVO_LAUNCH_CHECK(ctx);
+  rc = gft_launch_response(ctx, g, gray, mask_bits, nimg, images_per_maskset, rows, cols, nmask);
+  if (rc != SOSVO_OK) return rc;
   const int cell = min_distance >= 1 ? (int)lrint(min_distance) : 1;
   int32_t* redo = (int32_t*)(ws + o_redo);
   if (large) {
     SOSVO_PROFILE(ctx, "gft_select_kernel");
     hipLaunchKernelGGL((gft_select_kernel<kCandCapLarge, 1024>), dim3(xcd_grid(nimg, nmask)), dim3(1024), 0, ctx->stream, cand, wcnt,
-                       strips, nchunks, chunk_rows, wcap, mask_bits, mstat, images_per_maskset, nmask, rows, cols, quality, (float)min_distance, cell,
+                       strip_w, strips, nchunks, chunk_rows, wcap, mask_bits, mstat, images_per_maskset, nmask, rows, cols, quality, (float)min_distance, cell,
                        max_corners, cap, sorted_g, sorted_stride, kp, n, status, nullptr, 0, nimg);
   } else {
     SOSVO_PROFILE(ctx, "gft_select_kernel");
     auto launch = [&](auto small, auto full, int nt) {
-      hipLaunchKernelGGL(small, dim3(xcd_grid(nimg, nmask)), dim3(nt), 0, ctx->stream, cand, wcnt, strips, nchunks, chunk_rows, wcap,
+      hipLaunchKernelGGL(small, dim3(xcd_grid(nimg, nmask)), dim3(nt), 0, ctx->stream, cand, wcnt, strip_w, strips, nchunks, chunk_rows, wcap,
                          mask_bits, mstat, images_per_maskset, nmask, rows, cols, quality, (float)min_distance, cell, max_corners, cap,
                          sorted_g, sorted_stride, kp, n, status, redo, 0, nimg);
-      hipLaunchKernelGGL(full, dim3(xcd_grid(nimg, nmask)), dim3(nt), 0, ctx->stream, cand, wcnt, strips, nchunks, chunk_rows, wcap,
+      hipLaunchKernelGGL(full, dim3(xcd_grid(nimg, nmask)), dim3(nt), 0, ctx->stream, cand, wcnt, strip_w, strips, nchunks, chunk_rows, wcap,
                          mask_bits, mstat, images_per_maskset, nmask, rows, cols, quality, (float)min_distance, cell, max_corners, cap,
                          sorted_g, sorted_stride, kp, n, status, redo, 1, nimg);
     };
@@ -1088,6 +1467,18 @@
   }
   SOSVO_LAUNCH_CHECK(ctx);
   return SOSVO_OK;
+}
+
+int32_t sosvo_gauss7(sosvo_ctx* ctx, const uint8_t* gray, int32_t nimg, int32_t rows, int32_t cols, int64_t img_stride,
+                     uint8_t* out, int64_t out_stride, const int32_t* row_range) {
+  SOSVO_ENTER(ctx);
+  SOSVO_REQUIRE(ctx, gray && out, "null pointer");
+  SOSVO_REQUIRE(ctx, nimg >= 0 && nimg <= 65535, "nimg out of range");
+  SOSVO_REQUIRE(ctx, rows >= 1 && cols >= 1 && rows * (int64_t)cols < (1 << 28), "image sizes out of range");
+  SOSVO_REQUIRE(ctx, img_stride >= rows * (int64_t)cols && out_stride >= rows * (int64_t)cols, "a stride is shorter than an image");
+  SOSVO_REQUIRE(ctx, row_range == nullptr || nimg % 2 == 0, "row_range needs the two views' images (nimg even, view-major)");
+  if (nimg == 0) return SOSVO_OK;
+  return launch_gauss7_rows(ctx, gray, img_stride, nimg, rows, cols, out, out_stride, row_range, nimg > 1 ? nimg / 2 : 1);
 }
 
 int32_t sosvo_describe_orb(sosvo_ctx* ctx, const uint8_t* gray, int32_t nimg, int32_t rows, int32_t cols,
diff --git a/vo_single_camera_sos_amd/csrc/pipeline.hip b/vo_single_camera_sos_amd/csrc/pipeline.hip
--- a/vo_single_camera_sos_amd/csrc/pipeline.hip
+++ b/vo_single_camera_sos_amd/csrc/pipeline.hip
@@ -820,6 +820,7 @@
     }
     ctx->sub[i]->hint_shared_device = 1;
     ctx->sub[i]->hint_score_fp64_only = ctx->hint_score_fp64_only;
+    ctx->sub[i]->hint_rolling_narrow = ctx->hint_rolling_narrow;
     SOSVO_HIP(ctx, hipEventCreateWithFlags(&ctx->sub_done[i], hipEventDisableTiming));
     SOSVO_HIP(ctx, hipEventCreateWithFlags(&ctx->sub_median[i], hipEventDisableTiming));
     ctx->n_sub = i + 1;
diff --git a/vo_single_camera_sos_amd/csrc/rolling_layout.h b/vo_single_camera_sos_amd/csrc/rolling_layout.h
--- /dev/null
+++ b/vo_single_camera_sos_amd/csrc/rolling_layout.h
@@ -0,0 +1,50 @@
+#ifndef SOSVO_ROLLING_LAYOUT_H
+#define SOSVO_ROLLING_LAYOUT_H
+
+#include <stdint.h>
+
+#ifdef __HIPCC__
+#define SOSVO_LAYOUT_FN __host__ __device__ static inline
+#else
+#define SOSVO_LAYOUT_FN static inline
+#endif
+
+#define SOSVO_BLUR_WIDE_SPAN 256
+#define SOSVO_BLUR_WIDE_STRIP_W 250
+#define SOSVO_BLUR_WIDE_MIN_COLS 8
+
+typedef struct sosvo_blur_wide_lane {
+  int32_t off;
+  uint32_t sel;
+  uint32_t own;
+} sosvo_blur_wide_lane;
+
+SOSVO_LAYOUT_FN sosvo_blur_wide_lane sosvo_blur_wide_layout(int cols, int strip, int lane) {
+  sosvo_blur_wide_lane r;
+  const int first = strip * SOSVO_BLUR_WIDE_STRIP_W;
+  const int x0 = first - 3 + 4 * lane;
+  int off = x0;
+  if (off > cols - 4) off = cols - 4;
+  if (off < 0) off = 0;
+  r.off = off;
+  r.sel = 0u;
+  r.own = 0u;
+  for (int j = 0; j < 4; ++j) {
+    const int c = x0 + j;
+    int m = c < 0 ? -c : (c >= cols ? 2 * (cols - 1) - c : c);
+    int b = m - off;
+    if (b < 0) b = 0;
+    if (b > 3) b = 3;
+    r.sel |= (uint32_t)b << (8 * j);
+    if (c >= first && c < first + SOSVO_BLUR_WIDE_STRIP_W && c < cols) r.own |= 1u << j;
+  }
+  return r;
+}
+
+SOSVO_LAYOUT_FN int sosvo_blur_wide_strips(int cols) { return (cols + SOSVO_BLUR_WIDE_STRIP_W - 1) / SOSVO_BLUR_WIDE_STRIP_W; }
+SOSVO_LAYOUT_FN int sosvo_blur_wide_edge_strip(int cols, int strip) {
+  const int xb = strip * SOSVO_BLUR_WIDE_STRIP_W - 3;
+  return xb < 0 || xb + SOSVO_BLUR_WIDE_SPAN > cols;
+}
+
+#endif
diff --git a/vo_single_camera_sos_amd/device.py b/vo_single_camera_sos_amd/device.py
--- a/vo_single_camera_sos_amd/device.py
+++ b/vo_single_camera_sos_amd/device.py
@@ -103,6 +103,9 @@
 
     def set_hint_match_unsplit(self, on=True):
         self._call(self._lib.sosvo_set_hint, _lib.HINT_MATCH_UNSPLIT, 1 if on else 0)
+
+    def set_hint_rolling_narrow(self, on=True):
+        self._call(self._lib.sosvo_set_hint, _lib.HINT_ROLLING_NARROW, 1 if on else 0)
 
     def set_hint_score_fp64_only(self, on=True):
         self._call(self._lib.sosvo_set_hint, _lib.HINT_SCORE_FP64_ONLY, 1 if on else 0)
@@ -288,6 +291,41 @@
         self._call(self._lib.sosvo_describe_orb_rows, _ptr(gray), NI, rows, cols, int(nmask), cap, _ptr(kp), _ptr(n),
                    float(cos_a), float(sin_a), _ptr(pattern), int(edge), _ptr(row_range), _ptr(desc))
         return desc
+
+    def detect_gft_candidates(self, gray, mask_bits, images_per_maskset, nmask):
+        _check(gray, torch.uint8, "gray", ndim=3)
+        NI, rows, cols = gray.shape
+        _check(mask_bits, torch.uint32, "mask_bits", (None, rows, cols))
+        if mask_bits.shape[0] * images_per_maskset < NI:
+            raise SosvoError("mask_bits has too few sets for %d images" % NI)
+        geo = (ctypes.c_int32 * 6)()
+        args = (_ptr(gray), _ptr(mask_bits), NI, int(images_per_maskset), rows, cols, int(nmask), geo)
+        self._call(self._lib.sosvo_detect_gft_candidates, *(args + (NULL, NULL, NULL)))
+        strip_w, strips, nchunks, chunk_rows, wcap, regions = [int(v) for v in geo]
+        cand = torch.zeros((regions, wcap, 2), dtype=torch.uint32, device=gray.device)
+        wcnt = torch.zeros((regions,), dtype=torch.uint32, device=gray.device)
+        mstat = torch.zeros((NI * int(nmask), 5), dtype=torch.uint32, device=gray.device)
+        self._call(self._lib.sosvo_detect_gft_candidates, *(args + (_ptr(cand), _ptr(wcnt), _ptr(mstat))))
+        return dict(strip_w=strip_w, strips=strips, nchunks=nchunks, chunk_rows=chunk_rows, wcap=wcap, regions=regions,
+                    cand=cand, wcnt=wcnt, mstat=mstat)
+
+    def gauss7(self, gray, nimg, rows, cols, out=None, img_stride=None, out_stride=None, row_range=None):
+        nimg, rows, cols = int(nimg), int(rows), int(cols)
+        px = rows * cols
+        img_stride = px if img_stride is None else int(img_stride)
+        out_stride = px if out_stride is None else int(out_stride)
+        _check(gray, torch.uint8, "gray")
+        if out is None:
+            out = torch.zeros(max(nimg - 1, 0) * out_stride + px, dtype=torch.uint8, device=gray.device)
+        _check(out, torch.uint8, "out")
+        if nimg < 0 or rows < 1 or cols < 1 or img_stride < px or out_stride < px:
+            raise SosvoError("gauss7: nimg >= 0, rows, cols >= 1 and strides >= rows * cols")
+        if nimg > 0 and (gray.numel() < (nimg - 1) * img_stride + px or out.numel() < (nimg - 1) * out_stride + px):
+            raise SosvoError("gauss7: a buffer is shorter than (nimg - 1) * stride + rows * cols")
+        if row_range is not None:
+            _check(row_range, torch.int32, "row_range", (2, 2))
+        self._call(self._lib.sosvo_gauss7, _ptr(gray), nimg, rows, cols, img_stride, _ptr(out), out_stride, _ptr(row_range))
+        return out
 
     def refine_subpix(self, gray, kp, n, nmask, half=5, max_iter=_lib.SUBPIX_MAX_ITER, eps=_lib.SUBPIX_EPS, row_range=None):
         _check(gray, torch.uint8, "gray", ndim=3)
```

Measured after the change: 67920, median of 6. +1.7%, better.
